# hall-lab/speedseq

Measured on AMD Instinct MI355X. Metric: paired reads aligned+dup-marked/sec, higher is better.
Workload: dtype int32; 1 GPU; 1000000 synthetic 2x150 bp PE pairs per GPU vs a seeded synthetic GRCh37-shaped reference of 3100 Mbp (25 contigs, order-6 Markov model of the bundled chr20 slice + 63 planted repeat families of 10..10^4 copies at 0-10% divergence = 5% of the bases; GRCh37 itself is not available offline), bwa-mem -t 16 batch boundaries; pairs_per_gpu=1000000, read_len=150, ref_bp=3099999990, records=2058655, dup_pairs=47309, dup_pairs_local_view=47309, seeds=60444408, rescues=632178, chains=9804599, sam_lines=2009191, discordant_stream_lines=29550, splitter_stream_lines=18382, dedup_scope=single GPU = whole input, sorted_merge=single GPU: bin/sambamba sort (device radix sort of the keys)

## Files before the change

### include/ssgpu.h

```cpp
#ifndef SSGPU_H
#define SSGPU_H
#include <stdint.h>
#include <stddef.h>
#include "../speedseq_amd/csrc/ssg_types.h"

#ifdef __cplusplus
extern "C" {
#endif

#define SSG_OK         0
#define SSG_ENODEV   (-19)
#define SSG_ENOMEM   (-12)
#define SSG_EINVAL   (-22)
#define SSG_EIO      (-5)
#define SSG_EOVERFLOW (-75)
#define SSG_EALIGN   (-71)
#define SSG_EHIP     (-1000)

const char *ssg_version(void);
const char *ssg_backend(void);
int ssg_device_count(void);
int ssg_set_device(int dev);
int ssg_set_lane(int lane);
const char *ssg_last_error(void);

void ssg_mem_opt_init(ssg_mem_opt_t *opt);

typedef struct ssg_index ssg_index_t;
int ssg_index_load(const char *prefix, ssg_index_t **out);
int ssg_index_load2(const char *prefix, int defer_dense_sa, ssg_index_t **out);
int ssg_index_densify(ssg_index_t *idx);
int ssg_index_densify_to(ssg_index_t *idx, int intv);
int ssg_index_from_arrays(const uint32_t *bwt, uint64_t bwt_words, uint64_t primary, const uint64_t L2[5],
                          const uint64_t *sa, uint64_t n_sa, int sa_intv,
                          const uint8_t *pac, int64_t l_pac,
                          int n_ctg, const int64_t *ctg_off, const int32_t *ctg_len, ssg_index_t **out);
int ssg_index_build_fasta(const char *fasta, ssg_index_t **out);
int ssg_index_build_dev(const uint8_t *d_fwd, int64_t l_pac, int n_ctg, const int64_t *ctg_off, const int32_t *ctg_len, ssg_index_t **out);
int ssg_index_save(const ssg_index_t *idx, const char *prefix);
void ssg_index_destroy(ssg_index_t *idx);
int64_t ssg_index_l_pac(const ssg_index_t *idx);
int ssg_index_n_ctg(const ssg_index_t *idx);


int ssg_extend_batch(const ssg_mem_opt_t *opt, int n_jobs, const ssg_ext_job_t *jobs,
                     const uint8_t *qbuf, size_t qbytes, const uint8_t *tbuf, size_t tbytes,
                     ssg_ext_res_t *res, uint64_t *cells);

int ssg_align2_batch(const ssg_mem_opt_t *opt, int n_jobs, const ssg_sw_job_t *jobs,
                     const uint8_t *qbuf, size_t qbytes, const uint8_t *tbuf, size_t tbytes, ssg_kswr_t *res);

int ssg_global_batch(const ssg_mem_opt_t *opt, int n_jobs, const ssg_glb_job_t *jobs,
                     const uint8_t *qbuf, size_t qbytes, const uint8_t *tbuf, size_t tbytes,
                     int32_t *score, int32_t *n_cigar, uint32_t *cigar, int cap);

int ssg_smem_batch(const ssg_index_t *idx, const ssg_mem_opt_t *opt, int n_reads, const uint8_t *seq, const int64_t *off,
                   int cap, ssg_intv_t *out_intv, int32_t *out_n);

int ssg_seeds_batch(const ssg_index_t *idx, const ssg_mem_opt_t *opt, int n_reads, const uint8_t *seq, const int64_t *off,
                    int64_t *seed_off, ssg_seed_t **seeds, int32_t **rids);

int ssg_extend_lane_batch(const ssg_index_t *idx, const ssg_mem_opt_t *opt, int n_jobs, const ssg_ext_job_t *jobs, const int64_t *tpos, int dir,
                          const uint8_t *qbuf, size_t qbytes, int qcap, ssg_ext_res_t *res, uint64_t *cells);

int ssg_align2_lane_batch(const ssg_index_t *idx, const ssg_mem_opt_t *opt, int n_jobs, const ssg_sw_job_t *jobs, const int64_t *tpos,
                          const uint8_t *qbuf, size_t qbytes, int lanes, ssg_kswr_t *res, int32_t *from_lane);

int ssg_dbg_chain_sort(const int64_t *keys, int n, int64_t *out_lane, int64_t *out_wave);

#define SSG_CHAIN_FORM_LANE     0
#define SSG_CHAIN_FORM_LDS16    1
#define SSG_CHAIN_FORM_LDS32    2
#define SSG_CHAIN_FORM_LDS64    3
#define SSG_CHAIN_FORM_WAVE256  4
#define SSG_CHAIN_FORM_WAVE512  5
#define SSG_CHAIN_FORM_WAVE1024 6
#define SSG_CHAIN_FORM_WAVE2048 7
#define SSG_CHAIN_FORM_WAVE5120 8
#define SSG_CHAIN_FORM_TREE  0x10
int ssg_dbg_chain(const ssg_mem_opt_t *opt, int64_t l_pac, int n_ctg, int n_reads, const int32_t *read_len, const int64_t *seed_off, const ssg_seed_t *seeds, const int32_t *rids,
                  const int64_t *intv_off, const ssg_intv_t *intv, int64_t *chain_off, ssg_chain_t **chains, int32_t **chain_seeds, int32_t *form);

#define SSG_REG_ROUTE_WAVE  1
#define SSG_REG_ROUTE_PATCH 2
int ssg_dbg_regions(const ssg_mem_opt_t *opt, const uint8_t *pac, int64_t l_pac, int n_ctg, const int64_t *ctg_off, const int32_t *ctg_len, int n_reads, const uint8_t *seq, const int64_t *off,
                    const int64_t *seed_off, const ssg_seed_t *seeds, const int64_t *chain_off, const ssg_chain_t *chains, const int32_t *chain_seeds,
                    int64_t *reg_off, ssg_alnreg_t **regs, int32_t *route);

int ssg_dbg_pestat(const ssg_index_t *idx, const ssg_mem_opt_t *opt, int n_pairs, const int64_t *reg_off, const ssg_alnreg_t *regs,
                   const int32_t *pair_batch, int n_batches, ssg_pestat_t *pes);
void ssg_dbg_matesw_last(uint64_t counts[8]);
int ssg_dbg_matesw(const ssg_index_t *idx, const ssg_mem_opt_t *opt, int n_pairs, const uint8_t *seq, const int64_t *read_off, const int64_t *reg_off, const ssg_alnreg_t *regs,
                   const uint8_t *fixed, const ssg_pestat_t pes[4], int headroom, int64_t *out_off, ssg_alnreg_t **regs_out, int32_t *n_out, int32_t *err, uint64_t counts[8]);
int ssg_dbg_pair_final(const ssg_index_t *idx, const ssg_mem_opt_t *opt, int n_pairs, int64_t id0, const int64_t *reg_off, const ssg_alnreg_t *regs,
                       const ssg_pestat_t pes[4], ssg_alnreg_t *regs_out, int64_t *req_off, ssg_alnreq_t **req);

#define SSG_R2A_ROUTE_LANE 1
#define SSG_R2A_ROUTE_DP0  2
#define SSG_R2A_ROUTE_DP1  4
#define SSG_R2A_ROUTE_DP2  8
#define SSG_R2A_ROUTE_WAVE 16
int ssg_dbg_reg2aln(const ssg_mem_opt_t *opt, const uint8_t *pac, int64_t l_pac, int n_ctg, const int64_t *ctg_off, const int32_t *ctg_len, int n_reads, const uint8_t *seq, const int64_t *off,
                    int64_t n_regs, const ssg_alnreg_t *regs, int64_t n_req, const ssg_alnreq_t *req, ssg_aln_t *alns, int32_t *route, int32_t *dev_err);

int ssg_align1_batch(const ssg_index_t *idx, const ssg_mem_opt_t *opt, int n_reads, const uint8_t *seq, const int64_t *off,
                     int64_t *reg_off, ssg_alnreg_t **regs, uint64_t stats[8]);

typedef struct ssg_pe_result ssg_pe_result_t;
int ssg_mem_process_pairs(const ssg_index_t *idx, const ssg_mem_opt_t *opt, int n_pairs, const uint8_t *seq, const int64_t *off,
                          const int32_t *pair_batch, int n_batches, int64_t id0, const ssg_pestat_t *pes0, ssg_pe_result_t **out);
int ssg_mem_process_reads(const ssg_index_t *idx, const ssg_mem_opt_t *opt, int n_reads, const uint8_t *seq, const int64_t *off, int64_t id0, ssg_pe_result_t **out);
void ssg_pe_result_free(ssg_pe_result_t *r);
int ssg_pe_reserve(int n_pairs, int n_calls);
int64_t ssg_pe_n_req(const ssg_pe_result_t *r);
int ssg_pe_is_se(const ssg_pe_result_t *r);
const int64_t *ssg_pe_req_off(const ssg_pe_result_t *r);
const ssg_alnreq_t *ssg_pe_req(const ssg_pe_result_t *r);
const ssg_aln_t *ssg_pe_alns(const ssg_pe_result_t *r);
const ssg_pestat_t *ssg_pe_pes(const ssg_pe_result_t *r);
const uint64_t *ssg_pe_stats(const ssg_pe_result_t *r);

int ssg_sam_format(const ssg_index_t *idx, const ssg_mem_opt_t *opt, const ssg_pe_result_t *res, int n_pairs,
                   const char *const *names, const uint8_t *seq, const int64_t *off, const char *const *quals, const char *const *comments,
                   const char *rg_id, char **sam, int64_t *sam_off);
int ssg_sam_format_se(const ssg_index_t *idx, const ssg_mem_opt_t *opt, const ssg_pe_result_t *res, int n_reads,
                      const char *const *names, const uint8_t *seq, const int64_t *off, const char *const *quals, const char *const *comments,
                      const char *rg_id, char **sam, int64_t *sam_off);
int ssg_sam_format_sel(const ssg_index_t *idx, const ssg_mem_opt_t *opt, const ssg_pe_result_t *res, const int32_t *sel, int n_sel,
                       const char *const *names, const uint8_t *seq, const int64_t *off, const char *const *quals, const char *const *comments,
                       const char *rg_id, char **sam, int64_t *sam_off);
int ssg_bam_format(const ssg_index_t *idx, const ssg_mem_opt_t *opt, const ssg_pe_result_t *res, int n_pairs,
                   const char *const *names, const uint8_t *seq, const int64_t *off, const char *const *quals,
                   const char *rg_id, uint8_t **bam, int64_t *bam_off);
typedef struct ssg_pe_bam ssg_pe_bam_t;
int ssg_mem_process_fastq_bam(const ssg_index_t *idx, const ssg_mem_opt_t *opt, int n_pairs, const uint8_t *const *parts, const int64_t *part_bytes, int n_parts,
                              const int64_t *rec_off, const int32_t *pair_batch, int n_batches, int64_t id0, const ssg_pestat_t *pes0, const char *rg_id, ssg_pe_bam_t **out);
int ssg_mem_process_pairs_bam(const ssg_index_t *idx, const ssg_mem_opt_t *opt, int n_pairs, const uint8_t *seq, const int64_t *off,
                              const char *const *names, const char *const *quals, const int32_t *pair_batch, int n_batches, int64_t id0,
                              const ssg_pestat_t *pes0, const char *rg_id, ssg_pe_bam_t **out);
void ssg_pe_bam_free(ssg_pe_bam_t *r);
const uint8_t *ssg_pe_bam_data(const ssg_pe_bam_t *r);
int64_t ssg_pe_bam_bytes(const ssg_pe_bam_t *r);
int64_t ssg_pe_bam_n_rec(const ssg_pe_bam_t *r);
int64_t ssg_pe_bam_n_cand(const ssg_pe_bam_t *r);
const ssg_bam_cand_t *ssg_pe_bam_cands(const ssg_pe_bam_t *r);
const ssg_pestat_t *ssg_pe_bam_pes(const ssg_pe_bam_t *r);
const uint64_t *ssg_pe_bam_stats(const ssg_pe_bam_t *r);
int ssg_index_set_names(ssg_index_t *idx, int n, const char *const *names);
const char *ssg_index_name(const ssg_index_t *idx, int i);
int32_t ssg_index_len(const ssg_index_t *idx, int i);

int ssg_sbl_markdup(long n_pairs, const ssg_sbl_end_t *ends, uint8_t *dup);
typedef struct ssg_sbl_state ssg_sbl_state_t;
ssg_sbl_state_t *ssg_sbl_state_new(void);
void ssg_sbl_state_free(ssg_sbl_state_t *st);
int ssg_sbl_markdup_stream(ssg_sbl_state_t *st, long n_pairs, const ssg_sbl_end_t *ends, uint8_t *dup);

#define SSG_SBL_DUP   1
#define SSG_SBL_DISC  2
#define SSG_SBL_SPLIT 4
void ssg_sbl_opt_init(ssg_sbl_opt_t *o);
int ssg_sbl_process(ssg_sbl_state_t *st, const ssg_sbl_opt_t *o, long n_blocks, const int64_t *blk_off, const ssg_sbl_line_t *lines,
                    uint8_t *line_bits, int64_t *mate_line);
int ssg_sbl_ends(long n_blocks, const int64_t *blk_off, const ssg_sbl_line_t *lines, ssg_sbl_end_t *ends);
int ssg_sbl_classify(const ssg_sbl_opt_t *o, long n_blocks, const int64_t *blk_off, const ssg_sbl_line_t *lines, const uint8_t *dup,
                     uint8_t *line_bits, int64_t *mate_line);

int ssg_sort_u64_perm(const uint64_t *keys, int64_t n, uint32_t *perm);

int ssg_hotpath_dev(const ssg_index_t *idx, const ssg_mem_opt_t *opt, int n_pairs, int max_len, const uint8_t *d_seq, const int64_t *d_off,
                    const int32_t *d_pair_batch, int n_batches, int64_t id0, uint64_t summary[8], uint8_t *dup_host);
int ssg_hotpath_dev_sig(const ssg_index_t *idx, const ssg_mem_opt_t *opt, int n_pairs, int max_len, const uint8_t *d_seq, const int64_t *d_off,
                        const int32_t *d_pair_batch, int n_batches, int64_t id0, uint64_t summary[8], uint8_t *dup_host, uint64_t *d_sig_out);

typedef struct ssg_dev_records ssg_dev_records_t;
int ssg_hotpath_dev_ex(const ssg_index_t *idx, const ssg_mem_opt_t *opt, int n_pairs, int max_len, const uint8_t *d_seq, const int64_t *d_off,
                       const int32_t *d_pair_batch, int n_batches, int64_t id0, const ssg_sbl_opt_t *sbl, int local_dedup,
                       uint64_t summary[16], uint8_t *dup_host, uint64_t *d_sig_out, ssg_dev_records_t **keep);
int ssg_dev_records_classify(ssg_dev_records_t *r, const ssg_sbl_opt_t *sbl, const uint8_t *d_dup, uint64_t counts[4]);
int ssg_markdup_sig_dev(long n, const uint64_t *d_sig, const int64_t *d_ordinal, uint8_t *d_dup);
void ssg_dev_records_free(ssg_dev_records_t *r);
int64_t ssg_dev_records_n_lines(const ssg_dev_records_t *r);
size_t ssg_dev_record_bytes(void);
int ssg_dev_records_export(const ssg_dev_records_t *r, uint64_t *d_keys, void *d_recs, uint8_t *d_bits);
int ssg_dev_records_download(const ssg_dev_records_t *r, ssg_pe_result_t **res, uint8_t *line_bits, int64_t *mate_line);
int ssg_dbg_sbl_records(long n_pairs, const int64_t *req_off, const ssg_alnreq_t *req, const ssg_aln_t *alns, const ssg_sbl_opt_t *o, ssg_sbl_state_t *st,
                        int64_t *line_off, int64_t *n_lines, ssg_sbl_line_t *lines, int64_t *line_req, ssg_sbl_end_t *ends, int64_t *prim, uint64_t *sig, uint8_t *dup,
                        uint8_t *bits, int64_t *mate_line, uint64_t counts[4], uint64_t *keys);

int ssg_index_from_device(const uint32_t *d_bwt, uint64_t primary, const uint64_t L2[5], const uint64_t *d_sa, int sa_intv,
                          const uint8_t *d_pac, int64_t l_pac, int n_ctg, const int64_t *ctg_off, const int32_t *ctg_len, ssg_index_t **out);

void ssg_prof_enable(int on);
void ssg_prof_reset(void);
int ssg_prof_get(int cap, const char **name, double *ms, long *launches);

void ssg_free(void *p);

typedef struct ssg_coll ssg_coll_t;
int ssg_coll_available(void);
int ssg_coll_init(int rank, int world, const char *rendezvous_dir, ssg_coll_t **out);
int ssg_coll_alltoallv(ssg_coll_t *c, const void *const *send, const uint64_t *send_bytes, void *const *recv, const uint64_t *recv_bytes);
int ssg_coll_alltoall_u64(ssg_coll_t *c, const uint64_t *send, uint64_t *recv, int k);
void ssg_coll_destroy(ssg_coll_t *c);

int ssg_bgzf_deflate(const uint8_t *payload, const uint64_t *cut, long n_blocks, uint8_t *out, uint64_t out_cap, uint64_t *out_off);
int ssg_bgzf_compress(const uint8_t *payload, const uint64_t *cut, long n_blocks, uint8_t *out, uint64_t out_cap, uint64_t *out_off, uint32_t *crc);
int ssg_bgzf_deflate_level(const uint8_t *payload, const uint64_t *cut, long n_blocks, uint8_t *out, uint64_t out_cap, uint64_t *out_off, int level);
int ssg_bgzf_compress_level(const uint8_t *payload, const uint64_t *cut, long n_blocks, uint8_t *out, uint64_t out_cap, uint64_t *out_off, uint32_t *crc, int level);
uint64_t ssg_bgzf_bound(uint64_t payload_bytes, long n_blocks);
int ssg_crc32_batch(const uint8_t *data, const uint64_t *cut, long n, uint32_t *crc);
int ssg_bgzf_inflate(const uint8_t *members, const uint64_t *moff, long n_blocks, uint8_t *out, uint64_t out_cap, uint64_t *out_off, int32_t *status);
typedef struct ssg_recs ssg_recs_t;
int ssg_recs_create(uint64_t cap_bytes, ssg_recs_t **out);
int ssg_recs_append(ssg_recs_t *r, const uint8_t *bytes, uint64_t len, uint32_t *chunk_id);
int ssg_recs_order(ssg_recs_t *r, const uint64_t *loc, const uint64_t *cum, int64_t n);
int ssg_recs_gather(ssg_recs_t *r, uint64_t v0, uint64_t v1, uint8_t *out);
int ssg_bgzf_compress_recs(ssg_recs_t *r, const uint64_t *cut, long n_blocks, uint8_t *out, uint64_t out_cap, uint64_t *out_off, uint32_t *crc);
int ssg_bgzf_compress_recs_level(ssg_recs_t *r, const uint64_t *cut, long n_blocks, uint8_t *out, uint64_t out_cap, uint64_t *out_off, uint32_t *crc, int level);
void ssg_recs_free(ssg_recs_t *r);
typedef struct { int32_t tid, pos, end; uint32_t flag, len, pad; } ssg_bam_ent_t;
int ssg_recs_append_bgzf(ssg_recs_t *r, const uint8_t *members, const uint64_t *moff, long n_blocks, uint32_t *chunk_id, uint64_t *out_off, int32_t *status);
int ssg_recs_scan(ssg_recs_t *r, uint32_t chunk_id, const uint64_t *hint, int64_t n_hints, uint64_t first, uint64_t cap, uint64_t *n_rec, uint64_t *loc, uint64_t *key, ssg_bam_ent_t *ent);
typedef struct { int32_t tid, beg, end; } ssg_bam_region_t;
typedef struct { uint8_t op, arg; uint16_t pad; int32_t value; } ssg_bam_fop_t;
#define SSG_FOP_MAX 64
enum { SSG_FOP_FLAG = 0, SSG_FOP_AND = 1, SSG_FOP_OR = 2, SSG_FOP_NOT = 3, SSG_FOP_EQ = 4, SSG_FOP_NE = 5, SSG_FOP_LT = 6, SSG_FOP_LE = 7, SSG_FOP_GT = 8, SSG_FOP_GE = 9 };
enum { SSG_FLD_MAPQ = 0, SSG_FLD_REF_ID = 1, SSG_FLD_MATE_REF_ID = 2, SSG_FLD_TLEN = 3, SSG_FLD_SEQ_LEN = 4, SSG_FLD_FLAG = 5 };
int ssg_recs_select(ssg_recs_t *r, uint32_t chunk_id, const uint64_t *hint, int64_t n_hints, uint64_t first, const ssg_bam_region_t *reg, int64_t n_reg, const ssg_bam_fop_t *prog, int n_prog,
                    uint64_t cap, uint64_t *n_rec, uint64_t *n_sel, uint64_t *loc, uint64_t *key, ssg_bam_ent_t *ent);
int ssg_recs_reopen(ssg_recs_t *r);
int ssg_recs_release(ssg_recs_t *r, uint32_t chunk_id);
int ssg_device_memory(uint64_t *free_bytes, uint64_t *total_bytes);
void *ssg_host_alloc(size_t n);
void ssg_host_free(void *p);

#ifdef __cplusplus
}
#endif
#endif
```

### speedseq_amd/capi.py

```python
import ctypes as C
import os

import numpy as np

HERE = os.path.dirname(os.path.abspath(__file__))
DEFAULT_LIB = os.path.join(HERE, "libssgpu.so")

OPT_DT = np.dtype([
    ("a", "i4"), ("b", "i4"), ("o_del", "i4"), ("e_del", "i4"), ("o_ins", "i4"), ("e_ins", "i4"),
    ("pen_unpaired", "i4"), ("pen_clip5", "i4"), ("pen_clip3", "i4"), ("w", "i4"), ("zdrop", "i4"),
    ("T", "i4"), ("min_seed_len", "i4"), ("min_chain_weight", "i4"), ("max_chain_extend", "i4"),
    ("split_width", "i4"), ("max_occ", "i4"), ("max_chain_gap", "i4"), ("max_ins", "i4"), ("max_matesw", "i4"),
    ("max_XA_hits", "i4"), ("max_XA_hits_alt", "i4"), ("mapQ_coef_fac", "i4"), ("chunk_size", "i4"), ("n_threads", "i4"),
    ("_align", "i4"),
    ("max_mem_intv", "u8"),
    ("split_factor", "f4"), ("mask_level", "f4"), ("drop_ratio", "f4"), ("XA_drop_ratio", "f4"),
    ("mask_level_redun", "f4"), ("mapQ_coef_len", "f4"),
    ("mat", "i1", (25,)), ("_pad0", "i1"), ("flag", "u2"), ("_pad", "i1", (4,)),
], align=False)
INTV_DT = np.dtype([("x0", "u8"), ("x1", "u8"), ("x2", "u8"), ("info", "u8")])
SEED_DT = np.dtype([("rbeg", "i8"), ("qbeg", "i4"), ("len", "i4"), ("score", "i4"), ("next", "i4")])
CHAIN_DT = np.dtype([("pos", "i8"), ("first_seed", "i4"), ("last_seed", "i4"), ("n", "i4"), ("rid", "i4"), ("w", "i4"), ("kept", "i4"), ("first", "i4"), ("sec", "i4"),
                     ("left", "i4"), ("right", "i4"), ("frac_rep", "f4"), ("_pad", "i4")])
CHAIN_FORM_LANE, CHAIN_FORM_LDS16, CHAIN_FORM_LDS32, CHAIN_FORM_LDS64 = 0, 1, 2, 3
CHAIN_FORM_WAVE256, CHAIN_FORM_WAVE512, CHAIN_FORM_WAVE1024, CHAIN_FORM_WAVE2048, CHAIN_FORM_WAVE5120 = 4, 5, 6, 7, 8
CHAIN_FORM_TREE = 0x10
REG_ROUTE_WAVE, REG_ROUTE_PATCH = 1, 2
R2A_ROUTE_LANE, R2A_ROUTE_DP0, R2A_ROUTE_DP1, R2A_ROUTE_DP2, R2A_ROUTE_WAVE = 1, 2, 4, 8, 16
EXT_JOB_DT = np.dtype([("qoff", "i4"), ("qlen", "i4"), ("toff", "i4"), ("tlen", "i4"), ("w", "i4"), ("end_bonus", "i4"), ("zdrop", "i4"), ("h0", "i4")])
EXT_RES_DT = np.dtype([("score", "i4"), ("qle", "i4"), ("tle", "i4"), ("gtle", "i4"), ("gscore", "i4"), ("max_off", "i4")])
SW_JOB_DT = np.dtype([("qoff", "i4"), ("qlen", "i4"), ("toff", "i4"), ("tlen", "i4"), ("xtra", "i4"), ("_pad", "i4")])
KSWR_DT = np.dtype([("score", "i4"), ("te", "i4"), ("qe", "i4"), ("score2", "i4"), ("te2", "i4"), ("tb", "i4"), ("qb", "i4")])
GLB_JOB_DT = np.dtype([("qoff", "i4"), ("qlen", "i4"), ("toff", "i4"), ("tlen", "i4"), ("w", "i4"), ("_pad", "i4")])
ALNREG_DT = np.dtype([
    ("rb", "i8"), ("re", "i8"), ("qb", "i4"), ("qe", "i4"), ("rid", "i4"), ("score", "i4"), ("truesc", "i4"), ("sub", "i4"),
    ("alt_sc", "i4"), ("csub", "i4"), ("sub_n", "i4"), ("w", "i4"), ("seedcov", "i4"), ("secondary", "i4"),
    ("secondary_all", "i4"), ("seedlen0", "i4"), ("n_comp", "i4"), ("frac_rep", "f4"), ("hash", "u8"),
])
PESTAT_DT = np.dtype([("low", "i4"), ("high", "i4"), ("failed", "i4"), ("_pad", "i4"), ("avg", "f8"), ("std", "f8")])


class SsgError(RuntimeError):
    pass


def _ptr(a):
    return a.ctypes.data_as(C.c_void_p)


class Lib:
    def __init__(self, path=None):
        path = path or os.environ.get("SSGPU_LIB") or DEFAULT_LIB
        if not os.path.exists(path):
            raise SsgError("%s not found: build it with `make lib` (hipcc --offload-arch=gfx950); there is no CPU fallback" % path)
        self.path = path
        self.l = C.CDLL(path)
        self.l.ssg_version.restype = C.c_char_p
        self.l.ssg_backend.restype = C.c_char_p
        self.l.ssg_last_error.restype = C.c_char_p
        self.l.ssg_index_l_pac.restype = C.c_int64
        assert OPT_DT.itemsize == self.sizeof_opt(), (OPT_DT.itemsize, self.sizeof_opt())

    def sizeof_opt(self):
        return 25 * 4 + 4 + 8 + 6 * 4 + 32

    def _chk(self, rc):
        if rc != 0:
            raise SsgError("libssgpu error %d: %s" % (rc, self.l.ssg_last_error().decode()))

    def backend(self):
        return self.l.ssg_backend().decode()

    def device_count(self):
        return self.l.ssg_device_count()

    def opt_init(self):
        o = np.zeros(1, dtype=OPT_DT)
        self.l.ssg_mem_opt_init(_ptr(o))
        return o

    def index_load(self, prefix):
        h = C.c_void_p()
        self._chk(self.l.ssg_index_load(prefix.encode(), C.byref(h)))
        return h

    def index_build_fasta(self, fasta):
        h = C.c_void_p()
        self._chk(self.l.ssg_index_build_fasta(fasta.encode(), C.byref(h)))
        return h

    def index_build_dev(self, d_fwd, l_pac, ctg_off, ctg_len, names=None):
        h = C.c_void_p()
        co = np.asarray(ctg_off, dtype=np.int64)
        cl = np.asarray(ctg_len, dtype=np.int32)
        self._chk(self.l.ssg_index_build_dev(C.c_void_p(d_fwd), C.c_int64(l_pac), C.c_int(len(co)), _ptr(co), _ptr(cl), C.byref(h)))
        if names is not None:
            arr = (C.c_char_p * len(names))(*[n.encode() for n in names])
            self._chk(self.l.ssg_index_set_names(h, C.c_int(len(names)), arr))
        return h

    def index_save(self, h, prefix):
        self._chk(self.l.ssg_index_save(h, prefix.encode()))

    def index_destroy(self, h):
        self.l.ssg_index_destroy(h)

    def extend_batch(self, opt, jobs, qbuf, tbuf):
        jobs = np.ascontiguousarray(jobs, dtype=EXT_JOB_DT)
        res = np.zeros(len(jobs), dtype=EXT_RES_DT)
        cells = C.c_uint64(0)
        self._chk(self.l.ssg_extend_batch(_ptr(opt), C.c_int(len(jobs)), _ptr(jobs), _ptr(qbuf), C.c_size_t(qbuf.size),
                                          _ptr(tbuf), C.c_size_t(tbuf.size), _ptr(res), C.byref(cells)))
        return res, cells.value

    def align2_batch(self, opt, jobs, qbuf, tbuf):
        jobs = np.ascontiguousarray(jobs, dtype=SW_JOB_DT)
        res = np.zeros(len(jobs), dtype=KSWR_DT)
        self._chk(self.l.ssg_align2_batch(_ptr(opt), C.c_int(len(jobs)), _ptr(jobs), _ptr(qbuf), C.c_size_t(qbuf.size),
                                          _ptr(tbuf), C.c_size_t(tbuf.size), _ptr(res)))
        return res

    def global_batch(self, opt, jobs, qbuf, tbuf, cap=64):
        jobs = np.ascontiguousarray(jobs, dtype=GLB_JOB_DT)
        n = len(jobs)
        score = np.zeros(n, dtype=np.int32)
        ncig = np.zeros(n, dtype=np.int32)
        cig = np.zeros((n, cap), dtype=np.uint32)
        self._chk(self.l.ssg_global_batch(_ptr(opt), C.c_int(n), _ptr(jobs), _ptr(qbuf), C.c_size_t(qbuf.size),
                                          _ptr(tbuf), C.c_size_t(tbuf.size), _ptr(score), _ptr(ncig), _ptr(cig), C.c_int(cap)))
        return score, ncig, cig

    def smem_batch(self, idx, opt, seq, off, cap=64):
        n = len(off) - 1
        intv = np.zeros((n, cap), dtype=INTV_DT)
        cnt = np.zeros(n, dtype=np.int32)
        self._chk(self.l.ssg_smem_batch(idx, _ptr(opt), C.c_int(n), _ptr(seq), _ptr(off), C.c_int(cap), _ptr(intv), _ptr(cnt)))
        return intv, cnt

    def seeds_batch(self, idx, opt, seq, off):
        n = len(off) - 1
        seed_off = np.zeros(n + 1, dtype=np.int64)
        sp, rp = C.c_void_p(), C.c_void_p()
        self._chk(self.l.ssg_seeds_batch(idx, _ptr(opt), C.c_int(n), _ptr(seq), _ptr(off), _ptr(seed_off), C.byref(sp), C.byref(rp)))
        tot = int(seed_off[n])
        seeds = np.frombuffer((C.c_char * (tot * SEED_DT.itemsize)).from_address(sp.value), dtype=SEED_DT, count=tot).copy() if tot else np.zeros(0, SEED_DT)
        rids = np.frombuffer((C.c_char * (tot * 4)).from_address(rp.value), dtype=np.int32, count=tot).copy() if tot else np.zeros(0, np.int32)
        self.l.ssg_free(sp); self.l.ssg_free(rp)
        return seed_off, seeds, rids

    def extend_lane_batch(self, idx, opt, jobs, tpos, direction, qbuf, qcap):
        res = np.zeros(len(jobs), dtype=EXT_RES_DT)
        cells = C.c_uint64(0)
        tpos = np.ascontiguousarray(tpos, dtype=np.int64)
        self._chk(self.l.ssg_extend_lane_batch(idx, _ptr(opt), C.c_int(len(jobs)), _ptr(jobs), _ptr(tpos), C.c_int(direction), _ptr(qbuf), C.c_size_t(qbuf.size), C.c_int(qcap), _ptr(res), C.byref(cells)))
        return res, cells.value

    def align2_lane_batch(self, idx, opt, jobs, tpos, qbuf, lanes):
        jobs = np.ascontiguousarray(jobs, dtype=SW_JOB_DT)
        res = np.zeros(len(jobs), dtype=KSWR_DT)
        from_lane = np.zeros(len(jobs), dtype=np.int32)
        tpos = np.ascontiguousarray(tpos, dtype=np.int64)
        self._chk(self.l.ssg_align2_lane_batch(idx, _ptr(opt), C.c_int(len(jobs)), _ptr(jobs), _ptr(tpos), _ptr(qbuf), C.c_size_t(qbuf.size), C.c_int(lanes), _ptr(res), _ptr(from_lane)))
        return res, from_lane

    def dbg_chain_sort(self, keys):
        keys = np.ascontiguousarray(keys, dtype=np.int64)
        o0, o1 = np.zeros(len(keys), dtype=np.int64), np.zeros(len(keys), dtype=np.int64)
        self._chk(self.l.ssg_dbg_chain_sort(_ptr(keys), C.c_int(len(keys)), _ptr(o0), _ptr(o1)))
        return o0, o1

    def dbg_chain(self, opt, l_pac, n_ctg, read_len, seed_off, seeds, rids, intv_off, intv):
        read_len = np.ascontiguousarray(read_len, dtype=np.int32)
        seed_off = np.ascontiguousarray(seed_off, dtype=np.int64)
        intv_off = np.ascontiguousarray(intv_off, dtype=np.int64)
        seeds = np.ascontiguousarray(seeds, dtype=SEED_DT)
        rids = np.ascontiguousarray(rids, dtype=np.int32)
        intv = np.ascontiguousarray(intv, dtype=INTV_DT)
        n = len(read_len)
        assert len(seed_off) == n + 1 and len(intv_off) == n + 1 and len(seeds) >= seed_off[-1] and len(rids) >= seed_off[-1] and len(intv) >= intv_off[-1]
        chain_off, form = np.zeros(n + 1, dtype=np.int64), np.zeros(n, dtype=np.int32)
        cp, sp = C.c_void_p(), C.c_void_p()
        self._chk(self.l.ssg_dbg_chain(_ptr(opt), C.c_int64(l_pac), C.c_int(n_ctg), C.c_int(n), _ptr(read_len), _ptr(seed_off), _ptr(seeds), _ptr(rids), _ptr(intv_off), _ptr(intv),
                                       _ptr(chain_off), C.byref(cp), C.byref(sp), _ptr(form)))
        nc = int(chain_off[n])
        chains = np.frombuffer((C.c_char * (nc * CHAIN_DT.itemsize)).from_address(cp.value), dtype=CHAIN_DT, count=nc).copy() if nc else np.zeros(0, CHAIN_DT)
        ns = int(chains["n"].sum()) if nc else 0
        cseeds = np.frombuffer((C.c_char * (ns * 4)).from_address(sp.value), dtype=np.int32, count=ns).copy() if ns else np.zeros(0, np.int32)
        self.l.ssg_free(cp); self.l.ssg_free(sp)
        return chain_off, chains, cseeds, form

    def dbg_regions(self, opt, pac, l_pac, ctg_off, ctg_len, seq, off, seed_off, seeds, chain_off, chains, chain_seeds):
        pac = np.ascontiguousarray(pac, dtype=np.uint8)
        ctg_off = np.ascontiguousarray(ctg_off, dtype=np.int64)
        ctg_len = np.ascontiguousarray(ctg_len, dtype=np.int32)
        seq = np.ascontiguousarray(seq, dtype=np.uint8)
        off = np.ascontiguousarray(off, dtype=np.int64)
        seed_off = np.ascontiguousarray(seed_off, dtype=np.int64)
        chain_off = np.ascontiguousarray(chain_off, dtype=np.int64)
        seeds = np.ascontiguousarray(seeds, dtype=SEED_DT)
        chains = np.ascontiguousarray(chains, dtype=CHAIN_DT)
        chain_seeds = np.ascontiguousarray(chain_seeds, dtype=np.int32)
        n = len(off) - 1
        assert len(pac) >= l_pac // 4 + 1 and len(ctg_off) == len(ctg_len) and len(seed_off) == n + 1 and len(chain_off) == n + 1
        assert len(seq) >= off[-1] and len(seeds) >= seed_off[-1] and len(chains) >= chain_off[-1] and len(chain_seeds) >= int(chains["n"][:int(chain_off[-1])].sum())
        reg_off, route = np.zeros(n + 1, dtype=np.int64), np.zeros(n, dtype=np.int32)
        rp = C.c_void_p()
        self._chk(self.l.ssg_dbg_regions(_ptr(opt), _ptr(pac), C.c_int64(l_pac), C.c_int(len(ctg_off)), _ptr(ctg_off), _ptr(ctg_len), C.c_int(n), _ptr(seq), _ptr(off),
                                         _ptr(seed_off), _ptr(seeds), _ptr(chain_off), _ptr(chains), _ptr(chain_seeds), _ptr(reg_off), C.byref(rp), _ptr(route)))
        tot = int(reg_off[n])
        regs = np.frombuffer((C.c_char * (tot * ALNREG_DT.itemsize)).from_address(rp.value), dtype=ALNREG_DT, count=tot).copy() if tot else np.zeros(0, ALNREG_DT)
        self.l.ssg_free(rp)
        return reg_off, regs, route

    def dbg_reg2aln(self, opt, pac, l_pac, ctg_off, ctg_len, seq, off, regs, req):
        pac = np.ascontiguousarray(pac, dtype=np.uint8)
        ctg_off = np.ascontiguousarray(ctg_off, dtype=np.int64)
        ctg_len = np.ascontiguousarray(ctg_len, dtype=np.int32)
        seq = np.ascontiguousarray(seq, dtype=np.uint8)
        off = np.ascontiguousarray(off, dtype=np.int64)
        regs = np.ascontiguousarray(regs, dtype=ALNREG_DT)
        req = np.ascontiguousarray(req, dtype=ALNREQ_DT)
        n = len(off) - 1
        assert len(pac) >= l_pac // 4 + 1 and len(ctg_off) == len(ctg_len) and n >= 0 and (n == 0 or len(seq) >= off[-1])
        alns, route, err = np.zeros(len(req) + 1, dtype=ALN_DT), np.zeros(len(req) + 1, dtype=np.int32), C.c_int32(0)
        rc = self.l.ssg_dbg_reg2aln(_ptr(opt), _ptr(pac), C.c_int64(l_pac), C.c_int(len(ctg_off)), _ptr(ctg_off), _ptr(ctg_len), C.c_int(n), _ptr(seq), _ptr(off),
                                    C.c_int64(len(regs)), _ptr(regs), C.c_int64(len(req)), _ptr(req), _ptr(alns), _ptr(route), C.byref(err))
        if rc != -75:
            self._chk(rc)
        return rc, alns[:len(req)], route[:len(req)], int(err.value)

    def dbg_pestat(self, idx, opt, reg_off, regs, pair_batch, n_batches):
        reg_off = np.ascontiguousarray(reg_off, dtype=np.int64)
        regs = np.ascontiguousarray(regs, dtype=ALNREG_DT)
        pair_batch = np.ascontiguousarray(pair_batch, dtype=np.int32)
        pes = np.zeros(4 * n_batches, dtype=PESTAT_DT)
        self._chk(self.l.ssg_dbg_pestat(idx, _ptr(opt), C.c_int((len(reg_off) - 1) // 2), _ptr(reg_off), _ptr(regs), _ptr(pair_batch), C.c_int(n_batches), _ptr(pes)))
        return pes

    def dbg_pair_final(self, idx, opt, id0, reg_off, regs, pes):
        reg_off = np.ascontiguousarray(reg_off, dtype=np.int64)
        regs = np.ascontiguousarray(regs, dtype=ALNREG_DT)
        pes = np.ascontiguousarray(pes, dtype=PESTAT_DT)
        assert len(pes) == 4 and len(regs) == reg_off[-1]
        n = len(reg_off) - 1
        out = np.zeros(len(regs), dtype=ALNREG_DT)
        req_off = np.zeros(n + 1, dtype=np.int64)
        req_p = C.c_void_p()
        self._chk(self.l.ssg_dbg_pair_final(idx, _ptr(opt), C.c_int(n // 2), C.c_int64(id0), _ptr(reg_off), _ptr(regs), _ptr(pes), _ptr(out), _ptr(req_off), C.byref(req_p)))
        nreq = int(req_off[n])
        req = np.frombuffer((C.c_char * (nreq * ALNREQ_DT.itemsize)).from_address(req_p.value), dtype=ALNREQ_DT, count=nreq).copy() if nreq else np.zeros(0, ALNREQ_DT)
        self.l.ssg_free(req_p)
        return out, req_off, req

    def dbg_matesw(self, idx, opt, seq, read_off, reg_off, regs, pes, fixed=None, headroom=-1):
        seq = np.ascontiguousarray(seq, dtype=np.uint8)
        read_off = np.ascontiguousarray(read_off, dtype=np.int64)
        reg_off = np.ascontiguousarray(reg_off, dtype=np.int64)
        regs = np.ascontiguousarray(regs, dtype=ALNREG_DT)
        pes = np.ascontiguousarray(pes, dtype=PESTAT_DT)
        n = len(reg_off) - 1
        assert len(pes) == 4 and len(regs) == reg_off[-1] and len(read_off) == n + 1 and len(seq) == read_off[-1]
        fx = None if fixed is None else np.ascontiguousarray(fixed, dtype=np.uint8)
        assert fx is None or len(fx) == n
        out_off, n_out, err, counts = np.zeros(n + 1, dtype=np.int64), np.zeros(n, dtype=np.int32), np.zeros(n // 2, dtype=np.int32), np.zeros(8, dtype=np.uint64)
        out_p = C.c_void_p()
        self._chk(self.l.ssg_dbg_matesw(idx, _ptr(opt), C.c_int(n // 2), _ptr(seq), _ptr(read_off), _ptr(reg_off), _ptr(regs), _ptr(fx) if fx is not None else None, _ptr(pes),
                                        C.c_int(headroom), _ptr(out_off), C.byref(out_p), _ptr(n_out), _ptr(err), _ptr(counts)))
        tot = int(out_off[n])
        allr = np.frombuffer((C.c_char * (tot * ALNREG_DT.itemsize)).from_address(out_p.value), dtype=ALNREG_DT, count=tot).copy() if tot and out_p.value else np.zeros(0, ALNREG_DT)
        self.l.ssg_free(out_p)
        lists = [allr[int(out_off[r]):int(out_off[r]) + int(n_out[r])].copy() for r in range(n)]
        return lists, err, counts

    def dbg_matesw_last(self):
        counts = np.zeros(8, dtype=np.uint64)
        self.l.ssg_dbg_matesw_last(_ptr(counts))
        return counts

    def align1_batch(self, idx, opt, seq, off):
        n = len(off) - 1
        reg_off = np.zeros(n + 1, dtype=np.int64)
        regs_p = C.c_void_p()
        stats = np.zeros(8, dtype=np.uint64)
        self._chk(self.l.ssg_align1_batch(idx, _ptr(opt), C.c_int(n), _ptr(seq), _ptr(off), _ptr(reg_off), C.byref(regs_p), _ptr(stats)))
        tot = int(reg_off[n])
        buf = (C.c_char * (tot * ALNREG_DT.itemsize)).from_address(regs_p.value) if tot else b""
        regs = np.frombuffer(buf, dtype=ALNREG_DT, count=tot).copy()
        self.l.ssg_free(regs_p)
        return reg_off, regs, stats


ALNREQ_DT = np.dtype([("read", "i4"), ("reg", "i4"), ("kind", "i4"), ("owner", "i4"), ("flag", "i4"), ("mapq", "i4"), ("_p0", "i4"), ("_p1", "i4")])
ALN_DT = np.dtype([("pos", "i8"), ("rid", "i4"), ("flag", "i4"), ("mapq", "i4"), ("NM", "i4"), ("score", "i4"), ("sub", "i4"), ("n_cigar", "i4"),
                   ("is_rev", "i4"), ("l_md", "i4"), ("reg_idx", "i4"), ("xa_cnt", "i4"), ("_pad", "i4"), ("cigar", "u4", (64,)), ("md", "S320")])


class PeResult:

    def __init__(self, lib, handle, n_pairs, n_batches):
        self.lib, self.h, self.n_pairs, self.n_batches = lib, handle, n_pairs, n_batches
        l = lib.l
        n = l.ssg_pe_n_req(handle)
        self.req_off = np.ctypeslib.as_array(C.cast(l.ssg_pe_req_off(handle), C.POINTER(C.c_int64)), shape=(2 * n_pairs + 1,)).copy()
        self.req = np.frombuffer((C.c_char * (n * ALNREQ_DT.itemsize)).from_address(l.ssg_pe_req(handle)), dtype=ALNREQ_DT, count=n).copy() if n else np.zeros(0, ALNREQ_DT)
        self.alns = np.frombuffer((C.c_char * (n * ALN_DT.itemsize)).from_address(l.ssg_pe_alns(handle)), dtype=ALN_DT, count=n).copy() if n else np.zeros(0, ALN_DT)
        self.pes = np.frombuffer((C.c_char * (n_batches * 4 * PESTAT_DT.itemsize)).from_address(l.ssg_pe_pes(handle)), dtype=PESTAT_DT, count=n_batches * 4).copy() if n_batches else np.zeros(0, PESTAT_DT)
        self.stats = np.ctypeslib.as_array(C.cast(l.ssg_pe_stats(handle), C.POINTER(C.c_uint64)), shape=(8,)).copy()

    def close(self):
        if self.h:
            self.lib.l.ssg_pe_result_free(self.h)
            self.h = None

    def __del__(self):
        self.close()


def _bind_pe(lib):
    l = lib.l
    l.ssg_pe_n_req.restype = C.c_int64
    for f in ("ssg_pe_req_off", "ssg_pe_req", "ssg_pe_alns", "ssg_pe_pes", "ssg_pe_stats"):
        getattr(l, f).restype = C.c_void_p
        getattr(l, f).argtypes = [C.c_void_p]
    l.ssg_pe_n_req.argtypes = [C.c_void_p]
    l.ssg_pe_result_free.argtypes = [C.c_void_p]


def mem_process_pairs(lib, idx, opt, seq, off, pair_batch=None, n_batches=1, id0=0, pes0=None):
    _bind_pe(lib)
    n_pairs = (len(off) - 1) // 2
    if pair_batch is None:
        pair_batch = np.zeros(n_pairs, dtype=np.int32)
    pair_batch = np.ascontiguousarray(pair_batch, dtype=np.int32)
    h = C.c_void_p()
    p0 = _ptr(pes0) if pes0 is not None else None
    lib._chk(lib.l.ssg_mem_process_pairs(idx, _ptr(opt), C.c_int(n_pairs), _ptr(seq), _ptr(off), _ptr(pair_batch), C.c_int(n_batches),
                                         C.c_int64(id0), p0, C.byref(h)))
    return PeResult(lib, h, n_pairs, n_batches)


SBL_END_DT = np.dtype([("seq", "i4"), ("pos", "i4"), ("flag", "i4"), ("lclip", "i4"), ("rclip", "i4"), ("ralen", "i4")])


def sbl_markdup(lib, ends):
    ends = np.ascontiguousarray(ends, dtype=SBL_END_DT)
    n = len(ends) // 2
    dup = np.zeros(n, dtype=np.uint8)
    lib._chk(lib.l.ssg_sbl_markdup(C.c_long(n), _ptr(ends), _ptr(dup)))
    return dup


SBL_LINE_DT = np.dtype([("seq", "i4"), ("pos", "i4"), ("flag", "i4"), ("mapq", "i4"), ("lclip", "i4"), ("rclip", "i4"), ("qalen", "i4"), ("ralen", "i4")])
SBL_OPT_DT = np.dtype([("exclude_dups", "i4"), ("add_mate_tags", "i4"), ("max_split_count", "i4"), ("min_non_overlap", "i4"), ("max_unmapped_bases", "i4"),
                       ("min_indel_size", "i4")])


def sbl_opt_init(lib, **kw):
    o = np.zeros((), dtype=SBL_OPT_DT)
    lib.l.ssg_sbl_opt_init(_ptr(o))
    for k, v in kw.items():
        o[k] = v
    return o


def sbl_state_new(lib):
    lib.l.ssg_sbl_state_new.restype = C.c_void_p
    return C.c_void_p(lib.l.ssg_sbl_state_new())


def sbl_state_free(lib, st):
    lib.l.ssg_sbl_state_free(st)


def sbl_markdup_stream(lib, st, ends):
    ends = np.ascontiguousarray(ends, dtype=SBL_END_DT)
    n = len(ends) // 2
    dup = np.zeros(n, dtype=np.uint8)
    lib._chk(lib.l.ssg_sbl_markdup_stream(st, C.c_long(n), _ptr(ends), _ptr(dup)))
    return dup


def _sbl_chunk(blk_off, lines):
    off = np.ascontiguousarray(blk_off, dtype=np.int64)
    lines = np.ascontiguousarray(lines, dtype=SBL_LINE_DT)
    assert int(off[-1]) == len(lines), (int(off[-1]), len(lines))
    return off, lines, len(off) - 1


def sbl_process(lib, st, opt, blk_off, lines):
    off, lines, nb = _sbl_chunk(blk_off, lines)
    bits, mate = np.zeros(len(lines), dtype=np.uint8), np.zeros(len(lines), dtype=np.int64)
    lib._chk(lib.l.ssg_sbl_process(st, _ptr(opt), C.c_long(nb), _ptr(off), _ptr(lines), _ptr(bits), _ptr(mate)))
    return bits, mate


def sbl_ends(lib, blk_off, lines):
    off, lines, nb = _sbl_chunk(blk_off, lines)
    ends = np.zeros(2 * nb, dtype=SBL_END_DT)
    lib._chk(lib.l.ssg_sbl_ends(C.c_long(nb), _ptr(off), _ptr(lines), _ptr(ends)))
    return ends


def sbl_classify(lib, opt, blk_off, lines, dup):
    off, lines, nb = _sbl_chunk(blk_off, lines)
    dup = np.ascontiguousarray(dup, dtype=np.uint8)
    assert len(dup) == nb
    bits, mate = np.zeros(len(lines), dtype=np.uint8), np.zeros(len(lines), dtype=np.int64)
    lib._chk(lib.l.ssg_sbl_classify(_ptr(opt), C.c_long(nb), _ptr(off), _ptr(lines), _ptr(dup), _ptr(bits), _ptr(mate)))
    return bits, mate


def dbg_sbl_records(lib, req_off, req, alns, opt, st=None):
    req_off = np.ascontiguousarray(req_off, dtype=np.int64)
    req = np.ascontiguousarray(req, dtype=ALNREQ_DT)
    alns = np.ascontiguousarray(alns, dtype=ALN_DT)
    n_pairs, cap = (len(req_off) - 1) // 2, len(req) + 1
    assert len(req_off) == 2 * n_pairs + 1 and len(req) == len(alns)
    o = dict(line_off=np.zeros(n_pairs + 1, np.int64), lines=np.zeros(cap, SBL_LINE_DT), line_req=np.zeros(cap, np.int64), ends=np.zeros(2 * n_pairs + 1, SBL_END_DT),
             prim=np.zeros(2 * n_pairs + 1, np.int64), sig=np.zeros((n_pairs + 1, 3), np.uint64), dup=np.zeros(n_pairs + 1, np.uint8), bits=np.zeros(cap, np.uint8),
             mate=np.zeros(cap, np.int64), counts=np.zeros(4, np.uint64), keys=np.zeros(cap, np.uint64))
    nl = C.c_int64(0)
    rc = lib.l.ssg_dbg_sbl_records(C.c_long(n_pairs), _ptr(req_off), _ptr(req), _ptr(alns), _ptr(opt), st, _ptr(o["line_off"]), C.byref(nl), _ptr(o["lines"]),
                                   _ptr(o["line_req"]), _ptr(o["ends"]), _ptr(o["prim"]), _ptr(o["sig"]), _ptr(o["dup"]), _ptr(o["bits"]), _ptr(o["mate"]),
                                   _ptr(o["counts"]), _ptr(o["keys"]))
    n = int(nl.value)
    for k in ("lines", "line_req", "bits", "mate", "keys"):
        o[k] = o[k][:n]
    for k, m in (("ends", 2 * n_pairs), ("prim", 2 * n_pairs), ("sig", n_pairs), ("dup", n_pairs)):
        o[k] = o[k][:m]
    return rc, o


def index_from_device(lib, d_bwt, primary, L2, d_sa, d_pac, l_pac, ctg_off, ctg_len, sa_intv=32):
    h = C.c_void_p()
    L2a = np.asarray(L2, dtype=np.uint64)
    co = np.asarray(ctg_off, dtype=np.int64)
    cl = np.asarray(ctg_len, dtype=np.int32)
    lib._chk(lib.l.ssg_index_from_device(C.c_void_p(d_bwt), C.c_uint64(primary), _ptr(L2a), C.c_void_p(d_sa), C.c_int(sa_intv),
                                         C.c_void_p(d_pac), C.c_int64(l_pac), C.c_int(len(co)), _ptr(co), _ptr(cl), C.byref(h)))
    return h

# ... 347 lines not shown
```

### speedseq_amd/csrc/k_smem2.h

```cpp
#ifndef SSG_K_SMEM2_H
#define SSG_K_SMEM2_H
#include "ssg_dev.h"

#define SSG_S2_QWORDS 40
enum { S2_FWD = 0, S2_BWD, S2_P3F, S2_READ, S2_P1, S2_P2, S2_P3, S2_OUT, S2_FIN };
enum { S2_PEND_NONE = 0, S2_PEND_FWD, S2_PEND_BWD, S2_PEND_P3 };

struct alignas(16) ssg_pk2_t { uint64_t w0, w1; };
SSG_DEVFN ssg_pk2_t s2_pk(const ssg_intv_t &v)
{ ssg_pk2_t p; p.w0 = v.x0 | (v.x1 & 0xffffffull) << 40; p.w1 = (v.x1 >> 24) | v.x2 << 16 | v.info << 55; return p; }
SSG_DEVFN ssg_intv_t s2_unpk(const ssg_pk2_t &p)
{ ssg_intv_t v; v.x0 = p.w0 & 0xffffffffffull; v.x1 = (p.w0 >> 40) | (p.w1 & 0xffffull) << 24; v.x2 = (p.w1 >> 16) & 0x7fffffffffull; v.info = p.w1 >> 55; return v; }
SSG_DEVFN void s2_set_intv(const ssg_index_view_t &ix, int c, ssg_intv_t &ik)
{
	ik.x0 = ix.L2[c] + 1; ik.x2 = ix.L2[c+1] - ix.L2[c]; ik.x1 = ix.L2[3-c] + 1; ik.info = 0;
}

#ifdef SSG_EMU
static unsigned long long ssg_s2_stat[64];
SSG_DEVFN unsigned long long s2_wall() { return 1; }
#else
__device__ unsigned long long ssg_s2_stat[64];
SSG_DEVFN unsigned long long s2_wall() { return (unsigned long long)wall_clock64(); }
#endif
#define S2_STAT_MIN(i, v) atomicMin(&ssg_s2_stat[i], (unsigned long long)(v))
#define S2_STAT_MAX(i, v) atomicMax(&ssg_s2_stat[i], (unsigned long long)(v))
#define S2_STAT_ADD(i, v) atomicAdd(&ssg_s2_stat[i], (unsigned long long)(v))

#ifndef SSG_S2_WAVES
#define SSG_S2_WAVES 4
#endif
#ifndef SSG_S2_TRIPS
#define SSG_S2_TRIPS 2
#endif

#ifdef SSG_EMU
SSG_DEVFN int wv_uni(int v) { return v; }
SSG_DEVFN uint64_t wv_uni64(uint64_t v) { return v; }
#else
SSG_DEVFN int wv_uni(int v) { return __builtin_amdgcn_readfirstlane(v); }
SSG_DEVFN uint64_t wv_uni64(uint64_t v) { return (uint64_t)(uint32_t)__builtin_amdgcn_readfirstlane((int)(uint32_t)v) | (uint64_t)(uint32_t)__builtin_amdgcn_readfirstlane((int)(uint32_t)(v >> 32)) << 32; }
#endif
SSG_DEVFN ssg_intv_t wv_uni_intv(const ssg_intv_t &v) { ssg_intv_t o; o.x0 = wv_uni64(v.x0); o.x1 = wv_uni64(v.x1); o.x2 = wv_uni64(v.x2); o.info = wv_uni64(v.info); return o; }

SSG_DEVFN unsigned long long s2_wave_read(const ssg_index_view_t &ix, const ssg_mem_opt_t &opt, const int split_len, const int it, const int32_t *read_ids, const uint8_t *seq, const int64_t *off,
                                          ssg_intv_t *out_intv, int32_t *out_n, const int cap, uint8_t *qb, ssg_pk2_t *l0, ssg_pk2_t *l1)
{
	const int lane = wv_lane();
	unsigned long long nx = 0;
	const int r = read_ids ? read_ids[it] : it;
	const uint8_t *q = seq + off[r];
	const int len = (int)(off[r+1] - off[r]);
	ssg_wave_ldssync();
	for (int b = lane; b < len; b += 64) qb[b] = q[b];
	ssg_wave_ldssync();
	ssg_intv_t *const mem = out_intv + (long)it * cap;
	const int left = -2 - out_n[it];
	const bool skip_p3 = left >= 1;
	const int n_p3 = skip_p3 ? left - 1 : 0;
	int mem_n = n_p3, ovf = 0;
	auto smem1 = [&](const int sx, uint64_t min_intv) -> int {
		if (min_intv < 1) min_intv = 1;
		ssg_intv_t ik; s2_set_intv(ix, (int)qb[sx], ik); ik.info = (uint64_t)(sx + 1);
		int n = 0, i = sx + 1;
		bool stop = false;
		while (!stop && i < len) {
			const int cq = wv_uni((int)qb[i]);
			if (cq < 4) {
				const ssg_intv_t ok = wv_uni_intv(ssg_bwt_extend1_lean(ix, ik, 3 - cq, 0)); ++nx;
				if (ok.x2 != ik.x2) { l0[n++] = s2_pk(ik); stop = ok.x2 < min_intv; }
				if (!stop) { ik = ok; ik.info = (uint64_t)(i + 1); ++i; }
			} else { l0[n++] = s2_pk(ik); stop = true; }
		}
		if (!stop) l0[n++] = s2_pk(ik);
		const int ret = (int)ik.info;
		int cur = 0, prev_n = n, rev = 1, m1_n = 0, m1_last_beg = 0;
		bool more = true;
		for (int ib = sx - 1; more && ib >= -1; --ib) {
			const int cb = ib < 0 ? -1 : wv_uni((int)qb[ib]) < 4 ? wv_uni((int)qb[ib]) : -1;
			int curr_n = 0; bool have_last = false; uint64_t last_x2 = 0;
			ssg_wave_ldssync();
			for (int base = 0; base < prev_n; base += 64) {
				const int jj = base + lane; const bool valid = jj < prev_n;
				ssg_intv_t p; p.x0 = p.x1 = p.x2 = p.info = 0;
				if (valid) p = s2_unpk((cur ? l1 : l0)[rev ? prev_n - 1 - jj : jj]);
				ssg_intv_t okc; okc.x0 = okc.x1 = okc.x2 = okc.info = 0;
				if (valid && cb >= 0) okc = ssg_bwt_extend1_lean(ix, p, cb, 1);
				if (cb >= 0) nx += (unsigned long long)(prev_n - base < 64 ? prev_n - base : 64);
				const bool alive = valid && cb >= 0 && okc.x2 >= min_intv;
				if (base == 0 && !wv_get((int)alive, 0)) {
					const int beg = ib + 1;
					if (m1_n == 0 || beg < m1_last_beg) {
						++m1_n; m1_last_beg = beg;
						const int end0 = wv_get((int)(uint32_t)p.info, 0);
						if (end0 - beg >= opt.min_seed_len) {
							if (mem_n < cap) { if (lane == 0) { ssg_intv_t o = p; o.info |= (uint64_t)beg << 32; mem[mem_n] = o; } } else ovf = 1;
							++mem_n;
						}
					}
				}
				const unsigned long long am = wv_ballot(alive);
				if (am) {
					const unsigned long long below = am & ((1ull << lane) - 1ull);
					const int pl = below ? 63 - __clzll(below) : 0;
					const uint64_t px2 = (uint64_t)wv_shfl64_xor((long long)okc.x2, lane ^ pl);
					const bool push = alive && (below ? okc.x2 != px2 : (!have_last || okc.x2 != last_x2));
					const unsigned long long pm = wv_ballot(push);
					if (push) { ssg_intv_t o = okc; o.info = p.info; (cur ? l0 : l1)[curr_n + __popcll(pm & ((1ull << lane) - 1ull))] = s2_pk(o); }
					curr_n += __popcll(pm);
					have_last = true; last_x2 = (uint64_t)wv_get64((long long)okc.x2, 63 - __clzll(am));
				}
			}
			if (curr_n == 0) more = false;
			else { cur ^= 1; rev = 0; prev_n = curr_n; }
		}
		ssg_wave_ldssync();
		return ret;
	};
	if (len >= opt.min_seed_len) {
		int x = 0;
		while (x < len) { if (wv_uni((int)qb[x]) < 4) x = smem1(x, 1); else ++x; }
		const int old_n = mem_n < cap ? mem_n : cap;
		ssg_wave_memsync();
		for (int k = n_p3; k < old_n; ++k) {
			const ssg_intv_t m = wv_uni_intv(mem[k]);
			const int start = (int)(m.info >> 32), end = (int)(uint32_t)m.info;
			if (end - start >= split_len && m.x2 <= (uint64_t)opt.split_width) {
				const int sx = (start + end) >> 1;
				if (wv_uni((int)qb[sx]) < 4) (void)smem1(sx, m.x2 + 1);
			}
		}
		if (opt.max_mem_intv > 0 && !skip_p3) {
			x = 0;
			while (x < len) {
				if (wv_uni((int)qb[x]) > 3) ++x;
				else {
					ssg_intv_t ik; s2_set_intv(ix, (int)qb[x], ik);
					int i = x + 1, nxt = len; bool stop = false;
					while (!stop && i < len) {
						const int cq = wv_uni((int)qb[i]);
						if (cq < 4) {
							const ssg_intv_t ok = wv_uni_intv(ssg_bwt_extend1_lean(ix, ik, 3 - cq, 0)); ++nx;
							if (ok.x2 < (uint64_t)opt.max_mem_intv && i - x >= opt.min_seed_len) {
								if (ok.x2 > 0) {
									if (mem_n < cap) { if (lane == 0) { ssg_intv_t o = ok; o.info = (uint64_t)x << 32 | (uint64_t)(i + 1); mem[mem_n] = o; } } else ovf = 1;
									++mem_n;
								}
								nxt = i + 1; stop = true;
							} else { ik = ok; ++i; }
						} else { nxt = i + 1; stop = true; }
					}
					x = nxt;
				}
			}
		}
	}
	if (lane == 0) out_n[it] = ovf ? -1 : mem_n;
	return nx;
}

SSG_DEVFN long s2_ktab_off(int j) { return (long)(((1ull << (2 * j)) - 4ull) / 3ull); }
__global__ void ssg_k_ktab_level(ssg_index_view_t ix, int j, ssg_pk2_t *tab)
{
	const long p = (long)blockIdx.x * blockDim.x + threadIdx.x;
	if (p >= (1L << (2 * (j - 1)))) return;
	ssg_pk2_t *const out = tab + s2_ktab_off(j) + 4 * p;
	ssg_intv_t ok[4];
	if (j == 1) { for (int c = 0; c < 4; ++c) s2_set_intv(ix, c, ok[c]); }
	else ssg_bwt_extend(ix, s2_unpk(tab[s2_ktab_off(j - 1) + p]), ok, 1);
	for (int c = 0; c < 4; ++c) { ok[c].info = 0; out[c] = s2_pk(ok[c]); }
}
__global__ void ssg_k_ktab_verify(ssg_index_view_t ix, int j, long stride, const ssg_pk2_t *tab, unsigned long long *bad)
{
	const long t = (long)blockIdx.x * blockDim.x + threadIdx.x, code = t * stride;
	if (code >= (1L << (2 * j))) return;
	ssg_intv_t ik;
	s2_set_intv(ix, (int)(code & 3), ik);
	for (int k = 1; k < j; ++k) ik = ssg_bwt_extend1_lean(ix, ik, 3 - (int)((code >> (2 * k)) & 3), 0);
	const ssg_intv_t e = s2_unpk(tab[s2_ktab_off(j) + code]);
	if (ik.x2 != e.x2 || (ik.x2 && (ik.x0 != e.x0 || ik.x1 != e.x1))) atomicAdd(&bad[j], 1ull);
}
SSG_DEVFN uint64_t s2_window(const uint32_t *qw, int stride, int b)
{
	const int w0 = b >> 3, sh = (b & 7) << 2;
	const int w1 = w0 + 1 < SSG_S2_QWORDS ? w0 + 1 : SSG_S2_QWORDS - 1, w2 = w0 + 2 < SSG_S2_QWORDS ? w0 + 2 : SSG_S2_QWORDS - 1;
	uint64_t v = ((uint64_t)qw[w0 * stride] | (uint64_t)qw[w1 * stride] << 32) >> sh;
	if (sh) v |= (uint64_t)qw[w2 * stride] << (64 - sh);
	return v;
}
SSG_DEVFN uint32_t s2_code(const uint32_t *qw, int stride, int b, int n)
{
	uint64_t v = s2_window(qw, stride, b);
	v &= 0x3333333333333333ull; v = (v | v >> 2) & 0x0f0f0f0f0f0f0f0full; v = (v | v >> 4) & 0x00ff00ff00ff00ffull;
	v = (v | v >> 8) & 0x0000ffff0000ffffull; v = (v | v >> 16) & 0xffffffffull;
	return (uint32_t)v & ((1u << (2 * n)) - 1u);
}

template <bool TUNE, bool KT>
__global__ void __launch_bounds__(64, SSG_S2_WAVES) ssg_k_smem2(ssg_index_view_t ix, ssg_mem_opt_t opt, int n_reads, const int32_t *read_ids,
                           const uint8_t *seq, const int64_t *off, ssg_intv_t *out_intv, int32_t *out_n, int cap,
                           ssg_pk2_t *scratch, int scap, unsigned long long *n_extend, unsigned int *next_read, unsigned int max_ext, int max_row, uint32_t *n_ext_read, int32_t *heavy_ids, unsigned int *n_heavy,
                           const ssg_pk2_t *kt_tab, int kt_k )
{
	__shared__ uint32_t qlds[SSG_S2_QWORDS * 64];
	const long gt = (long)blockIdx.x * blockDim.x + threadIdx.x;
	const int lane = (int)(threadIdx.x & 63);
	ssg_pk2_t *const vec0 = scratch + (gt >> 6) * 2 * scap * 64 + lane, *const vec1 = vec0 + (long)scap * 64;
	const uint32_t *const ql_ = qlds + lane;
#define S2Q(i) ((int)((ql_[((i) >> 3) * 64] >> (((i) & 7) << 2)) & 15u))
#define S2V(v, e) ((v)[(long)(e) * 64])
	const int split_len = (int)(opt.min_seed_len * opt.split_factor + .499);
	unsigned long long my_nx = 0;
	unsigned int rd_nx = 0, nx_p3 = 0;
	long it = 0;
	int state = S2_READ, pend = S2_PEND_NONE;
	int len = 0, x = 0, k = 0, old_n = 0, caller = 0, mem_n = 0, ovf = 0, heavy = 0, n_p3 = -1;
	ssg_intv_t *mem = 0;
	int sx = 0, i = 0, j = 0, curr_n = 0, prev_n = 0, prev_rev = 0, flip = 0, m1_n = 0, m1_last_beg = 0, ret = 0, e_c = 0;
	uint64_t min_intv = 1, last_x2 = 0;
	ssg_intv_t ik, p;
	ik.x0 = ik.x1 = ik.x2 = ik.info = 0; p = ik;
	ssg_pk2_t pn, c0, first; pn.w0 = pn.w1 = 0; c0 = first = pn;
	if (TUNE) S2_STAT_MIN(0, s2_wall());
#define S2_FWDEND() do { ret = (int)ik.info; flip ^= 1; prev_n = curr_n < scap ? curr_n : scap; prev_rev = 1; curr_n = 0; i = sx - 1; j = 0; first = s2_pk(ik); state = S2_BWD; if (prev_n > max_row) { heavy = 1; state = S2_OUT; } } while (0)
#define S2_P3END() do { n_p3 = mem_n; nx_p3 = rd_nx; x = 0; state = S2_P1; } while (0)
#define S2_P3START() do { \
		while (x < len && S2Q(x) > 3) ++x; \
		if (x >= len) S2_P3END(); \
		else if (!KT || kt_k < 2) { s2_set_intv(ix, S2Q(x), ik); i = x + 1; state = S2_P3F; } \
		else { \
			const unsigned long long nm_ = s2_window(ql_, 64, x) & 0x4444444444444444ull; \
			int run_ = nm_ ? (int)((__ffsll(nm_) - 1) >> 2) : 16; \
			run_ = run_ > len - x ? len - x : run_; \
			if (run_ >= kt_k) { ik = s2_unpk(kt_tab[s2_ktab_off(kt_k) + (long)s2_code(ql_, 64, x, kt_k)]); i = x + kt_k; my_nx += (unsigned long long)(kt_k - 1); rd_nx += (unsigned int)(kt_k - 1); state = S2_P3F; } \
			else { my_nx += (unsigned long long)(run_ - 1); rd_nx += (unsigned int)(run_ - 1); if (x + run_ >= len) S2_P3END(); else { x += run_ + 1; state = S2_P3; } } \
		} \
	} while (0)
#define S2_RET() do { if (caller == 1) { x = ret; state = S2_P1; } else { ++k; state = S2_P2; } } while (0)
#define S2_EMIT(pp, beg) do { if (m1_n == 0 || (beg) < m1_last_beg) { ++m1_n; m1_last_beg = (beg); \
		if ((int)(uint32_t)(pp).info - (beg) >= opt.min_seed_len) { ssg_intv_t o_ = (pp); o_.info |= (uint64_t)(beg) << 32; if (mem_n < cap) mem[mem_n] = o_; else ovf = 1; ++mem_n; } } } while (0)
	for (;;) {
		SSG_UNROLL for (int trip = 0; trip < SSG_S2_TRIPS; ++trip) if ((trip == 0 || wv_ballot(pend == S2_PEND_NONE && state != S2_FIN)) && pend == S2_PEND_NONE && state != S2_FIN) {
			ssg_pk2_t *const curr = flip ? vec1 : vec0;
			if (state == S2_FWD) {
				if (i < len && S2Q(i) < 4) { pend = S2_PEND_FWD; e_c = 3 - S2Q(i); }
				else { if (curr_n < scap) S2V(curr, curr_n) = s2_pk(ik); else ovf = 1; ++curr_n; S2_FWDEND(); }
			} else if (state == S2_BWD) {
				if (j >= prev_n) {
					bool back_to_caller = curr_n == 0;
					if (!back_to_caller) { flip ^= 1; prev_n = curr_n < scap ? curr_n : scap; prev_rev = 0; curr_n = 0; j = 0; --i; first = c0; back_to_caller = i < -1; }
					if (back_to_caller) S2_RET();
				} else {
					p = s2_unpk(j == 0 ? first : pn);
					const int cb = i < 0 ? -1 : S2Q(i) < 4 ? S2Q(i) : -1;
					if (cb >= 0) { pend = S2_PEND_BWD; e_c = cb; }
					else {
						if (j == 0) S2_EMIT(p, i + 1);
						j = prev_n;
					}
				}
			} else if (state == S2_P3F) {
				if (i >= len) S2_P3END();
				else if (S2Q(i) < 4) { pend = S2_PEND_P3; e_c = 3 - S2Q(i); }
				else { x = i + 1; S2_P3START(); }
			} else if (state == S2_READ) {
				it = (long)atomicAdd(next_read, 1u);
				if (it >= n_reads) { state = S2_FIN; if (TUNE) S2_STAT_MIN(1, s2_wall()); }
				else {
					const int r = read_ids ? read_ids[it] : (int)it;
					const uint8_t *q = seq + off[r];
					len = (int)(off[r+1] - off[r]);
					mem = out_intv + (long)it * cap; mem_n = 0; ovf = 0; rd_nx = 0; nx_p3 = 0; heavy = 0;
					const unsigned al = (unsigned)((uintptr_t)q & 7), sh8 = al << 3;
					const uint64_t *const qa = (const uint64_t*)(q - al);
					const int nw = (len + 7) >> 3, nb = (int)al + len;
					for (int w0 = 0; w0 < nw; w0 += 4) {
						uint64_t t[5];
						SSG_UNROLL for (int jj = 0; jj < 5; ++jj) t[jj] = (w0 + jj) * 8 < nb ? qa[w0 + jj] : 0;
						SSG_UNROLL for (int jj = 0; jj < 4; ++jj) {
							const int w = w0 + jj;
							if (w < nw) {
								uint64_t v = sh8 ? (t[jj] >> sh8) | (t[jj + 1] << (64 - sh8)) : t[jj];
								v &= 0x0f0f0f0f0f0f0f0full;
								v = (v | v >> 4) & 0x00ff00ff00ff00ffull;
								v = (v | v >> 8) & 0x0000ffff0000ffffull;
								uint32_t v32 = (uint32_t)(v | v >> 16);
								const int nv = len - w * 8;
								if (nv < 8) v32 &= (1u << (nv << 2)) - 1u;
								qlds[w * 64 + lane] = v32;
							}
						}
					}
					x = 0;
					n_p3 = opt.max_mem_intv > 0 ? -1 : 0;
					state = len < opt.min_seed_len ? S2_OUT : opt.max_mem_intv > 0 ? S2_P3 : S2_P1;
				}
			} else if (state == S2_P1) {
				if (x >= len) { old_n = mem_n < cap ? mem_n : cap; k = n_p3 > 0 ? n_p3 : 0; state = S2_P2; }
				else if (S2Q(x) > 3) ++x;
				else { sx = x; min_intv = 1; caller = 1; state = S2_FWD; m1_n = 0; curr_n = 0; i = sx + 1; s2_set_intv(ix, S2Q(sx), ik); ik.info = (uint64_t)(sx + 1); }
			} else if (state == S2_P2) {
				if (k >= old_n) state = S2_OUT;
				else {
					const ssg_intv_t m = mem[k];
					const int start = (int)(m.info >> 32), end = (int)(uint32_t)m.info;
					if (end - start < split_len || m.x2 > (uint64_t)opt.split_width) ++k;
					else {
						sx = (start + end) >> 1; min_intv = m.x2 + 1; caller = 2; m1_n = 0; curr_n = 0; i = sx + 1;
						if (S2Q(sx) > 3) S2_RET();
						else { s2_set_intv(ix, S2Q(sx), ik); ik.info = (uint64_t)(sx + 1); state = S2_FWD; }
					}
				}
			} else if (state == S2_P3) {
				S2_P3START();
			} else {
				const bool given_up = heavy != 0;
				out_n[it] = ovf ? -1 : given_up ? (n_p3 < 0 ? -2 : -3 - n_p3) : mem_n;
				if (given_up && !ovf && heavy_ids) heavy_ids[atomicAdd(n_heavy, 1u)] = (int32_t)it;
				if (given_up) my_nx -= n_p3 < 0 ? rd_nx : rd_nx - nx_p3;
				if (n_ext_read) n_ext_read[it] = rd_nx;
				if (TUNE) { S2_STAT_ADD(8 + (64 - __clzll((unsigned long long)(rd_nx | 1u))), 1); if (given_up) S2_STAT_ADD(3, 1); }
				state = S2_READ;
			}
		}
		if (TUNE) { const unsigned long long rdy = wv_ballot(pend != S2_PEND_NONE), alv = wv_ballot(state != S2_FIN); if (lane == 0) { S2_STAT_ADD(48, 1); S2_STAT_ADD(49, __popcll(rdy)); S2_STAT_ADD(50, __popcll(alv)); } }
		if (!wv_ballot(state != S2_FIN)) break;
		const int pat_b = pend == S2_PEND_BWD ? i : pend == S2_PEND_FWD ? sx : x, pat_n = (pend == S2_PEND_BWD ? (int)p.info : i + 1) - pat_b;
		const bool by_table = KT && pend != S2_PEND_NONE && pat_n <= kt_k;
		const bool any_tab = KT && wv_ballot(by_table) != 0, any_ext = !KT || wv_ballot(pend != S2_PEND_NONE && !by_table) != 0;
		if (pend != S2_PEND_NONE) {
			const ssg_pk2_t *const prev = flip ? vec0 : vec1;
			ssg_pk2_t *const curr = flip ? vec1 : vec0;
			const bool back = pend == S2_PEND_BWD;
			const int jn = back && j + 1 < prev_n ? j + 1 : 0;
			ssg_pk2_t pf; pf.w0 = pf.w1 = 0;
			if (jn) pf = S2V(prev, prev_rev ? prev_n - 1 - jn : jn);
			ssg_intv_t okc; okc.x0 = okc.x1 = okc.x2 = okc.info = 0;
			if (any_tab) { if (by_table) okc = s2_unpk(kt_tab[s2_ktab_off(pat_n) + (long)s2_code(ql_, 64, pat_b, pat_n)]); }
			if (any_ext) { if (!by_table) okc = ssg_bwt_extend1_lean(ix, back ? p : ik, e_c, back); }
			++my_nx; ++rd_nx;
			if (pend == S2_PEND_FWD) {
				bool fwd_end = false;
				if (okc.x2 != ik.x2) {
					if (curr_n < scap) S2V(curr, curr_n) = s2_pk(ik); else ovf = 1;
					++curr_n;
					if (okc.x2 < min_intv) { S2_FWDEND(); fwd_end = true; }
				}
				if (!fwd_end) { ik = okc; ik.info = (uint64_t)(i + 1); ++i; }
			} else if (back) {
				pn = pf;
				if (okc.x2 < min_intv) { if (curr_n == 0) S2_EMIT(p, i + 1); }
				else if (curr_n == 0 || okc.x2 != last_x2) {
					ssg_intv_t o = okc; o.info = p.info;
					const ssg_pk2_t po = s2_pk(o);
					if (curr_n == 0) c0 = po;
					if (curr_n < scap) S2V(curr, curr_n) = po; else ovf = 1;
					++curr_n; last_x2 = okc.x2;
				}
				++j;
			} else {
				if (okc.x2 < (uint64_t)opt.max_mem_intv && i - x >= opt.min_seed_len) {
					if (okc.x2 > 0) { ssg_intv_t o = okc; o.info = (uint64_t)x << 32 | (uint64_t)(i + 1); if (mem_n < cap) mem[mem_n] = o; else ovf = 1; ++mem_n; }
					x = i + 1; S2_P3START();
				} else { ik = okc; ++i; }
			}
			pend = S2_PEND_NONE;
			if (rd_nx > max_ext) { heavy = 1; state = S2_OUT; }
		}
	}
	if (TUNE) S2_STAT_MAX(2, s2_wall());
#undef S2Q
#undef S2V
#undef S2_FWDEND
#undef S2_P3START
#undef S2_P3END
#undef S2_RET
#undef S2_EMIT
	if (n_extend && my_nx) atomicAdd(n_extend, my_nx);
}

#ifdef SSG_HEAVY_MIN_WAVES
#define SSG_HEAVY_BOUNDS __launch_bounds__(64, SSG_HEAVY_MIN_WAVES)
#else
#define SSG_HEAVY_BOUNDS __launch_bounds__(64)
#endif
template <int SC>
__global__ void SSG_HEAVY_BOUNDS ssg_k_smem_heavy(ssg_index_view_t ix, ssg_mem_opt_t opt, const int32_t *ids, const unsigned int *n_ids, const int32_t *read_ids,
                           const uint8_t *seq, const int64_t *off, ssg_intv_t *out_intv, int32_t *out_n, int cap, unsigned long long *n_extend, unsigned int *next)
{
	__shared__ uint8_t qb[328];
	__shared__ ssg_pk2_t lst[2][SC];
	const int split_len = (int)(opt.min_seed_len * opt.split_factor + .499);
	const int n_todo = (int)*n_ids;
	unsigned long long nx = 0;
	for (;;) {
		const long t = wv_queue_pop(next);
		if (t >= n_todo) break;
		nx += s2_wave_read(ix, opt, split_len, ids[t], read_ids, seq, off, out_intv, out_n, cap, qb, lst[0], lst[1]);
	}
	if (n_extend && nx && wv_lane() == 0) atomicAdd(n_extend, nx);
}
__global__ void ssg_k_sa_verify(ssg_index_view_t ix, int new_intv, const uint64_t *sa_new, long n_new, long stride, unsigned long long *bad)
{
	const long j = ((long)blockIdx.x * blockDim.x + threadIdx.x) * stride;
	if (j >= n_new) return;
	const uint64_t r = (uint64_t)j * (uint64_t)new_intv;
	const uint64_t want = (r % (uint64_t)ix.sa_intv) == 0 ? ix.sa[r / (uint64_t)ix.sa_intv] : ssg_bwt_sa(ix, r);
	if (sa_new[j] != want) atomicAdd(bad, 1ull);
}
#endif
```

### speedseq_amd/csrc/ssg_dbg.cpp

```cpp
#include <vector>
#include <string>
#include <algorithm>
#include "ssg_rt.h"
#include "../../include/ssgpu.h"
#include "ssg_index_int.h"
#include "ssg_pe_int.h"
#include "ssg_stage_int.h"

SSG_ABI_FP_DEFINE(dbg)

static int dbg_refuse(const char *who, const char *bad, long at)
{
	ssg_err_msg = std::string(who) + ": " + bad + " " + std::to_string(at);
	return SSG_EINVAL;
}
static int dbg_check_contigs(const char *who, int64_t l_pac, int n_ctg, const int64_t *ctg_off, const int32_t *ctg_len)
{
	for (int c = 0; c < n_ctg; ++c)
		if (ctg_len[c] < 1 || ctg_off[c] != (c ? ctg_off[c - 1] + ctg_len[c - 1] : 0) || ctg_off[c] + ctg_len[c] > l_pac || (c == n_ctg - 1 && ctg_off[c] + ctg_len[c] != l_pac)) {
			ssg_err_msg = std::string(who) + ": the contigs must tile [0, l_pac) in order"; return SSG_EINVAL; }
	return 0;
}
static int dbg_read_len(const int64_t *off, int r, const char **bad)
{
// ... 115 lines not shown
	ssg_chain_t *oc = (ssg_chain_t*)calloc((size_t)n_out + 1, sizeof(ssg_chain_t)); int32_t *os = (int32_t*)calloc((size_t)n_sd + 1, sizeof(int32_t));
	if (!oc || !os) { free(oc); free(os); ssg_err_msg = "host allocation failed: chains"; return SSG_ENOMEM; }
	int64_t k = 0, q = 0;
	for (int r = 0; r < n_reads; ++r) {
		chain_off[r] = k;
		for (int i = 0; i < h_nc[r]; ++i) {
			const ssg_chain_t &c = h_ch[seed_off[r] + h_ord[seed_off[r] + i]];
			ssg_chain_t &o = oc[k++];
			o.pos = c.pos; o.rid = c.rid; o.n = c.n; o.w = c.w; o.kept = c.kept; o.frac_rep = c.frac_rep; o.first_seed = (int32_t)q;
			for (int j = 0; j < c.n; ++j) os[q++] = (int32_t)(h_cs[c.first_seed + j] - seed_off[r]);
		}
	}
	chain_off[n_reads] = k;
	*chains = oc; *chain_seeds = os;
	return SSG_OK;
}

int ssg_dbg_regions(const ssg_mem_opt_t *opt, const uint8_t *pac, int64_t l_pac, int n_ctg, const int64_t *ctg_off, const int32_t *ctg_len, int n_reads, const uint8_t *seq, const int64_t *off,
                    const int64_t *seed_off, const ssg_seed_t *seeds, const int64_t *chain_off, const ssg_chain_t *chains, const int32_t *chain_seeds,
                    int64_t *reg_off, ssg_alnreg_t **regs, int32_t *route)
{
	CHK(ssg_need_device());
	*regs = 0;
	if (n_reads < 0 || l_pac < 1 || l_pac >= (int64_t)1 << 33 || n_ctg < 1) { ssg_err_msg = "ssg_dbg_regions: need n_reads >= 0, 1 <= l_pac < 2^33, n_ctg >= 1"; return SSG_EINVAL; }
	CHK(dbg_check_contigs("ssg_dbg_regions", l_pac, n_ctg, ctg_off, ctg_len));
	if (n_reads == 0) { reg_off[0] = 0; return SSG_OK; }
	const char *bad = 0; long at = 0;
	if (off[0] != 0 || seed_off[0] != 0 || chain_off[0] != 0) bad = "offsets start at 0: read";
	int max_len = 0;
	auto ctg_of = [&](int64_t p) { const int64_t f = p < l_pac ? p : 2 * l_pac - 1 - p; int lo = 0, hi = n_ctg - 1; while (lo < hi) { const int mid = (lo + hi + 1) >> 1; if (ctg_off[mid] <= f) lo = mid; else hi = mid - 1; } return lo; };
	std::vector<uint8_t> used;
	for (int r = 0; !bad && r < n_reads; ++r) {
		at = r;
		if (seed_off[r + 1] < seed_off[r] || chain_off[r + 1] < chain_off[r]) { bad = "offsets must not decrease: read"; break; }
		const int len = dbg_read_len(off, r, &bad);
		if (bad) break;
		const int64_t ns = seed_off[r + 1] - seed_off[r], nc = chain_off[r + 1] - chain_off[r];
		if (ns >= (int64_t)1 << 24) { bad = "more than 2^24 seeds: read"; break; }
		if (nc > ns) { bad = "more chains than seeds: read"; break; }
		max_len = std::max(max_len, len);
		dbg_check_codes(seq, off, r, &bad);
		for (int64_t k = seed_off[r]; !bad && k < seed_off[r + 1]; ++k) {
			bad = dbg_check_seed(seeds[k], len, l_pac, "need 0 <= qbeg, 1 <= len, qbeg + len <= read length: seed");
			if (bad) at = (long)k;
		}
		used.assign((size_t)ns, 0);
		for (int64_t k = chain_off[r]; !bad && k < chain_off[r + 1]; ++k) {
			const ssg_chain_t &c = chains[k];
			at = (long)k;
			if (c.n < 1) { bad = "a chain has at least 1 seed: chain"; break; }
			if (c.first_seed < 0 || (k > 0 && c.first_seed != chains[k - 1].first_seed + chains[k - 1].n) || (k == 0 && c.first_seed != 0)) { bad = "first_seed must run on from the chain before: chain"; break; }
			for (int j = 0; j < c.n; ++j) {
				const int32_t id = chain_seeds[c.first_seed + j];
				if (id < 0 || id >= ns) { bad = "a seed index outside the read's seeds: chain"; break; }
				if (used[(size_t)id]) { bad = "a seed in two chains: chain"; break; }
				used[(size_t)id] = 1;
			}
			if (bad) break;
			const int64_t first = seeds[seed_off[r] + chain_seeds[c.first_seed]].rbeg;
			if (c.rid != ctg_of(first)) { bad = "rid must be the contig of the chain's first seed: chain"; break; }
			int64_t cb = ctg_off[c.rid], ce = cb + ctg_len[c.rid];
			if (first >= l_pac) { const int64_t t = cb; cb = 2 * l_pac - ce; ce = 2 * l_pac - t; }
			for (int j = 0; j < c.n; ++j) {
				const ssg_seed_t &sd = seeds[seed_off[r] + chain_seeds[c.first_seed + j]];
				if (sd.rbeg < cb || sd.rbeg + sd.len > ce) { bad = "every seed of a chain must lie inside the contig and strand of its first seed: chain"; break; }
			}
			if (bad) break;
		}
	}
	if (!bad) {
		CHK(check_scores(opt, max_len));
		if (opt->e_del < 1 || opt->e_ins < 1) { ssg_err_msg = "ssg_dbg_regions: gap extension penalties must be positive"; return SSG_EINVAL; }
	}
	if (bad) return dbg_refuse("ssg_dbg_regions", bad, at);
	const int64_t tot = seed_off[n_reads];
	if (tot >= (int64_t)1 << 31) { ssg_err_msg = "ssg_dbg_regions: more than 2^31 seeds"; return SSG_EINVAL; }
	const size_t ts = (size_t)tot + 1;
	const std::vector<ssg_seed_t> h_sd = dbg_stage_seeds(seeds, tot);
	std::vector<ssg_chain_t> h_ch(ts); std::vector<int32_t> h_ord(ts, 0), h_cs(ts, 0);
	const std::vector<int32_t> h_nc = dbg_counts(chain_off, n_reads), h_ns = dbg_counts(seed_off, n_reads);
	memset(h_ch.data(), 0, ts * sizeof(ssg_chain_t));
	for (int r = 0; r < n_reads; ++r) {
		const int64_t s0 = seed_off[r];
		int64_t q = s0;
		for (int i = 0; i < h_nc[r]; ++i) {
			const ssg_chain_t &c = chains[chain_off[r] + i];
			ssg_chain_t &d = h_ch[s0 + i];
			d = c; d.first_seed = (int32_t)q; d.last_seed = -1;
			h_ord[s0 + i] = i;
			for (int j = 0; j < c.n; ++j) h_cs[q++] = (int32_t)(s0 + chain_seeds[c.first_seed + j]);
		}
	}
	dbg_ref_t ref;
	CHK(ref.up(pac, l_pac, n_ctg, ctg_off, ctg_len));
	dbuf<uint8_t> d_seq((size_t)off[n_reads] + 1); dbuf<int64_t> d_off((size_t)n_reads + 1);
	dbuf<ssg_seed_t> d_seeds(ts); dbuf<ssg_chain_t> d_chains(ts); dbuf<int32_t> d_order(ts), d_cseeds(ts), d_nchain(n_reads), d_nseed(n_reads), d_work(n_reads); dbuf<unsigned int> d_queue(8);
	CHKA(d_seq); CHKA(d_off); CHKA(d_seeds); CHKA(d_chains); CHKA(d_order); CHKA(d_cseeds); CHKA(d_nchain); CHKA(d_nseed); CHKA(d_work); CHKA(d_queue);
	CHK(d_seq.up(seq, (size_t)off[n_reads])); CHK(d_off.up(off, (size_t)n_reads + 1));
	CHK(d_seeds.up(h_sd.data(), ts)); CHK(d_chains.up(h_ch.data(), ts)); CHK(d_order.up(h_ord.data(), ts)); CHK(d_cseeds.up(h_cs.data(), ts));
	CHK(d_nchain.up(h_nc.data(), n_reads)); CHK(d_nseed.up(h_ns.data(), n_reads));
	CHK(dbg_work_order(d_nseed.p, n_reads, d_work.p, d_queue));
	align1_dev_t o;
	if (!o.seed_off.alloc((size_t)n_reads + 1) || !o.regs.alloc(ts) || !o.n_reg.alloc(n_reads)) { ssg_err_msg = "device allocation failed: regs"; return SSG_ENOMEM; }
	CHK(o.seed_off.up(seed_off, (size_t)n_reads + 1));
	std::vector<int32_t> todo;
	CHK(run_regions(ref.ix, opt, n_reads, d_seq.p, d_off.p, max_len, ts, d_seeds.p, d_chains.p, d_order.p, d_cseeds.p, d_nchain.p, d_work.p, d_queue.p, o, (uint64_t*)0, (uint64_t*)0, &todo));
	std::vector<int32_t> hn((size_t)n_reads); std::vector<uint8_t> hf((size_t)n_reads); std::vector<ssg_alnreg_t> all(ts);
	CHK(o.n_reg.down(hn.data(), n_reads)); CHK(o.sdp_fixed.down(hf.data(), n_reads)); CHK(o.regs.down(all.data(), (size_t)tot));
	int64_t n_out = 0;
	for (int r = 0; r < n_reads; ++r) {
		if (hn[r] < 0 || hn[r] > h_ns[r]) { ssg_err_msg = "ssg_dbg_regions: a read's region count is outside its slice"; return SSG_EOVERFLOW; }
		reg_off[r] = n_out; n_out += hn[r];
	}
	reg_off[n_reads] = n_out;
	ssg_alnreg_t *out = (ssg_alnreg_t*)malloc(sizeof(ssg_alnreg_t) * (size_t)(n_out + 1));
	if (!out) { ssg_err_msg = "host allocation failed: regions"; return SSG_ENOMEM; }
	for (int r = 0; r < n_reads; ++r) memcpy(out + reg_off[r], all.data() + seed_off[r], sizeof(ssg_alnreg_t) * (size_t)hn[r]);
	if (route) {
		for (int r = 0; r < n_reads; ++r) route[r] = hf[r] == 0 ? SSG_REG_ROUTE_PATCH : 0;
		for (size_t k = 0; k < todo.size(); ++k) if (todo[k] >= 0 && todo[k] < n_reads) route[todo[k]] |= SSG_REG_ROUTE_WAVE;
	}
	*regs = out;
	return SSG_OK;
}

int ssg_dbg_reg2aln(const ssg_mem_opt_t *opt, const uint8_t *pac, int64_t l_pac, int n_ctg, const int64_t *ctg_off, const int32_t *ctg_len, int n_reads, const uint8_t *seq, const int64_t *off,
                    int64_t n_regs, const ssg_alnreg_t *regs, int64_t n_req, const ssg_alnreq_t *req, ssg_aln_t *alns, int32_t *route, int32_t *dev_err)
{
	CHK(ssg_need_device());
	if (dev_err) *dev_err = 0;
	if (n_reads < 0 || n_regs < 0 || n_req < 0 || n_req >= (int64_t)1 << 31 || l_pac < 1 || l_pac >= (int64_t)1 << 33 || n_ctg < 1) {
		ssg_err_msg = "ssg_dbg_reg2aln: need n_reads, n_regs >= 0, 0 <= n_req < 2^31, 1 <= l_pac < 2^33, n_ctg >= 1"; return SSG_EINVAL; }
	CHK(dbg_check_contigs("ssg_dbg_reg2aln", l_pac, n_ctg, ctg_off, ctg_len));
	if (n_req == 0) return SSG_OK;
	const char *bad = 0; long at = 0;
	int max_len = 0;
	if (n_reads < 1) bad = "requests need reads: request";
	else if (off[0] != 0) bad = "offsets start at 0: read";
	for (int r = 0; !bad && r < n_reads; ++r) {
		at = r;
		max_len = std::max(max_len, dbg_read_len(off, r, &bad));
		if (!bad) dbg_check_codes(seq, off, r, &bad);
	}
	for (int64_t k = 0; !bad && k < n_regs; ++k) {
		const ssg_alnreg_t &a = regs[k];
		at = (long)k;
		if (!(0 <= a.rb && a.rb < a.re && a.re <= 2 * l_pac)) bad = "need 0 <= rb < re <= 2 l_pac: region";
		else if (a.rb < l_pac && a.re > l_pac) bad = "a region must not cross the forward / reverse boundary l_pac: region";
		else if (a.re - a.rb > SSG_STAGE_TWIN_GLB) bad = "need re - rb <= 32768: region";
		else if (!(0 <= a.qb && a.qb < a.qe && a.qe <= SSG_MAX_READ_LEN)) bad = "need 0 <= qb < qe <= read length: region";
	}
	for (int64_t k = 0; !bad && k < n_req; ++k) {
		const ssg_alnreq_t &q = req[k];
		at = (long)k;
		if (q.read < 0 || q.read >= n_reads) bad = "read index out of range: request";
		else if (q.reg >= n_regs) bad = "region index out of range: request";
		else if (q.kind != SSG_REQ_MAIN && q.kind != SSG_REQ_XA) bad = "kind is SSG_REQ_MAIN or SSG_REQ_XA: request";
		else if (q.reg >= 0 && regs[q.reg].qe > off[q.read + 1] - off[q.read]) bad = "need 0 <= qb < qe <= read length for the request's region and read: request";
	}
	if (bad) return dbg_refuse("ssg_dbg_reg2aln", bad, at);
	CHK(check_band(opt)); CHK(check_scores(opt, max_len)); CHK(check_gap_penalties(opt));
	dbg_ref_t ref;
	CHK(ref.up(pac, l_pac, n_ctg, ctg_off, ctg_len));
	dbuf<uint8_t> d_seq((size_t)off[n_reads] + 1); dbuf<int64_t> d_off((size_t)n_reads + 1); dbuf<int32_t> d_gerr(1);
	dbuf<ssg_alnreg_t> d_regs((size_t)n_regs + 1); dbuf<ssg_alnreq_t> d_req((size_t)n_req + 1); dbuf<ssg_aln_t> d_alns((size_t)n_req + 1); dbuf<unsigned long long> d_cnt(3);
	CHKA(d_seq); CHKA(d_off); CHKA(d_gerr); CHKA(d_regs); CHKA(d_req); CHKA(d_alns); CHKA(d_cnt);
	CHK(d_seq.up(seq, (size_t)off[n_reads])); CHK(d_off.up(off, (size_t)n_reads + 1));
	if (n_regs) CHK(d_regs.up(regs, (size_t)n_regs));
	CHK(d_req.up(req, (size_t)n_req)); CHK(d_alns.zero()); CHK(d_gerr.zero()); CHK(d_cnt.zero());
	r2a_lists_t lists;
	CHK(run_reg2aln(ref.ix, opt, n_req, d_req.p, d_regs.p, d_seq.p, d_off.p, d_alns.p, d_gerr.p, d_cnt.p, max_len, &lists));
	int32_t ge = 0;
	CHK(d_gerr.down(&ge, 1));
	if (dev_err) *dev_err = ge;
	CHK(d_alns.down(alns, (size_t)n_req));
	if (route) {
		for (int64_t k = 0; k < n_req; ++k) route[k] = req[k].reg >= 0 ? SSG_R2A_ROUTE_LANE : 0;
		for (int c = 0; c < SSG_STAGE_R2D_CLASSES; ++c) for (int32_t g : lists.dp[c]) if (g >= 0 && g < n_req) route[g] = SSG_R2A_ROUTE_DP0 << c;
		for (int32_t g : lists.todo) if (g >= 0 && g < n_req) route[g] = (route[g] & ~SSG_R2A_ROUTE_LANE) | SSG_R2A_ROUTE_WAVE;
	}
	if (ge) { ssg_err_msg = "CIGAR generation exceeded an on-device capacity (code " + std::to_string(ge) + ")"; return SSG_EOVERFLOW; }
	return SSG_OK;
}

static int dbg_check_regs(const ssg_index_t *idx, int n_pairs, const int64_t *reg_off, const ssg_alnreg_t *regs, const char *who)
{
	const int n_reads = 2 * n_pairs;
	const char *bad = 0; long at = -1;
	if (n_pairs < 0 || n_pairs > (1 << 24)) { bad = "n_pairs out of range"; at = n_pairs; }
	else if (reg_off[0] != 0) { bad = "reg_off[0] != 0"; at = 0; }
	for (int r = 0; r < n_reads && !bad; ++r) {
		if (reg_off[r + 1] < reg_off[r] || reg_off[r + 1] - reg_off[r] > 4096) { bad = "reg_off not monotone, or more than 4096 regions in a read: read"; at = r; }
		else if (reg_off[r + 1] > (1LL << 28)) { bad = "too many regions in all: read"; at = r; }
	}
	for (int64_t k = 0; !bad && k < reg_off[n_reads]; ++k) {
		const ssg_alnreg_t &e = regs[k];
		if (e.rid < 0 || e.rid >= idx->v.n_ctg) bad = "rid out of range: region";
		else if (!(0 <= e.qb && e.qb < e.qe && e.qe <= 310)) bad = "need 0 <= qb < qe <= 310: region";
		else if (!(0 <= e.rb && e.rb < e.re && e.re <= 2 * idx->v.l_pac)) bad = "need 0 <= rb < re <= 2 l_pac: region";
		else if (e.score < 0 || e.score > (1 << 20) || e.csub < 0 || e.csub > (1 << 20)) bad = "score / csub out of range: region";
		else if (!(e.frac_rep >= 0 && e.frac_rep <= 1)) bad = "frac_rep outside [0, 1]: region";
		if (bad) at = (long)k;
	}
	return bad ? dbg_refuse(who, bad, at) : 0;
}

int ssg_dbg_pestat(const ssg_index_t *idx, const ssg_mem_opt_t *opt, int n_pairs, const int64_t *reg_off, const ssg_alnreg_t *regs,
                   const int32_t *pair_batch, int n_batches, ssg_pestat_t *pes)
{
	CHK(ssg_need_device());
	CHK(dbg_check_regs(idx, n_pairs, reg_off, regs, "ssg_dbg_pestat"));
	if (n_batches < 1 || n_batches > 64) { ssg_err_msg = "ssg_dbg_pestat: 1 <= n_batches <= 64"; return SSG_EINVAL; }
	for (int p = 0; p < n_pairs; ++p) if (pair_batch[p] < 0 || pair_batch[p] >= n_batches) { ssg_err_msg = "ssg_dbg_pestat: pair_batch out of range"; return SSG_EINVAL; }
	const int n_reads = 2 * n_pairs;
	const int64_t tot = reg_off[n_reads];
	const std::vector<int32_t> hn = dbg_counts(reg_off, n_reads);
	dbuf<int64_t> d_off((size_t)n_reads + 1); dbuf<ssg_alnreg_t> d_regs((size_t)tot + 1); dbuf<int32_t> d_n((size_t)n_reads + 1), d_pb((size_t)n_pairs + 1);
	CHKA(d_off); CHKA(d_regs); CHKA(d_n); CHKA(d_pb);
	CHK(d_off.up(reg_off, (size_t)n_reads + 1)); CHK(d_regs.up(regs, (size_t)tot)); CHK(d_n.up(hn.data(), (size_t)n_reads)); CHK(d_pb.up(pair_batch, (size_t)n_pairs));
	return run_pestat(idx, opt, n_pairs, d_off.p, d_regs.p, d_n.p, d_pb.p, n_batches, pes);
}

int ssg_dbg_pair_final(const ssg_index_t *idx, const ssg_mem_opt_t *opt, int n_pairs, int64_t id0, const int64_t *reg_off, const ssg_alnreg_t *regs,
                       const ssg_pestat_t pes[4], ssg_alnreg_t *regs_out, int64_t *req_off, ssg_alnreq_t **req)
{
	CHK(ssg_need_device());
	CHK(dbg_check_regs(idx, n_pairs, reg_off, regs, "ssg_dbg_pair_final"));
	for (int d = 0; d < 4; ++d) if (!pes[d].failed && !(pes[d].std > 0 && pes[d].low >= 0 && pes[d].low <= pes[d].high)) { ssg_err_msg = "ssg_dbg_pair_final: an orientation that has not failed needs std > 0 and 0 <= low <= high"; return SSG_EINVAL; }
	const int n_reads = 2 * n_pairs;
	const int64_t tot = reg_off[n_reads];
	*req = 0;
	if (n_pairs == 0) { req_off[0] = 0; return SSG_OK; }
	const std::vector<int32_t> hn = dbg_counts(reg_off, n_reads);
	dbuf<int64_t> d_off((size_t)n_reads + 1); dbuf<ssg_alnreg_t> d_regs((size_t)tot + 1); dbuf<int32_t> d_n((size_t)n_reads), d_pb((size_t)n_pairs); dbuf<ssg_pestat_t> d_pes(4);
	CHKA(d_off); CHKA(d_regs); CHKA(d_n); CHKA(d_pb); CHKA(d_pes);
	CHK(d_off.up(reg_off, (size_t)n_reads + 1)); CHK(d_regs.up(regs, (size_t)tot)); CHK(d_n.up(hn.data(), (size_t)n_reads)); CHK(d_pb.zero()); CHK(d_pes.up(pes, 4));
	pair_slices_t s;
	CHK(make_pair_slices(n_reads, d_off.p, d_regs.p, d_n.p, opt->max_matesw, s));
	dbuf<int32_t> d_perr(n_pairs), d_zbuf((size_t)s.t2 + 1), d_nreq(n_reads); dbuf<unsigned int> d_q(1); dbuf<ssg_alnreq_t> d_req((size_t)s.tq + 1);
	CHKA(d_perr); CHKA(d_zbuf); CHKA(d_nreq); CHKA(d_q); CHKA(d_req);
	CHK(d_perr.zero()); CHK(d_nreq.zero());
	CHK(run_pair_final(idx, opt, n_pairs, id0, s.t2, s.d_r2off.p, s.d_regs2.p, d_n.p, d_pb.p, d_pes.p, s.d_pkey.p, s.d_pw.p, d_zbuf.p, s.d_reqoff.p, d_req.p, d_nreq.p, d_perr.p, d_q.p));
	CHK(dev_copy_regs(n_reads, s.d_r2off.p, s.d_regs2.p, d_n.p, d_off.p, d_regs.p));
	pe_dev_t t;
	CHK(run_req_tail(n_reads, s.d_reqoff.p, d_req.p, d_nreq.p, 0, 0, t));
	CHK(rt_sync());
	const int64_t nreq = t.n_req;
	std::vector<int64_t> r2off((size_t)n_reads + 1);
	CHK(s.d_r2off.down(r2off.data(), (size_t)n_reads + 1)); CHK(t.req_off.down(req_off, (size_t)n_reads + 1)); CHK(d_regs.down(regs_out, (size_t)tot));
	ssg_alnreq_t *out = (ssg_alnreq_t*)malloc(sizeof(ssg_alnreq_t) * (size_t)(nreq + 1));
	if (!out) { ssg_err_msg = "host allocation failed: requests"; return SSG_ENOMEM; }
	int rc = t.req.down(out, (size_t)nreq);
	if (rc) { free(out); return rc; }
	for (int64_t k = 0; k < nreq; ++k) if (out[k].reg >= 0) out[k].reg = (int32_t)(out[k].reg - r2off[out[k].read] + reg_off[out[k].read]);
	*req = out;
	return SSG_OK;
}

int ssg_dbg_matesw(const ssg_index_t *idx, const ssg_mem_opt_t *opt, int n_pairs, const uint8_t *seq, const int64_t *read_off, const int64_t *reg_off, const ssg_alnreg_t *regs,
                   const uint8_t *fixed, const ssg_pestat_t pes[4], int headroom, int64_t *out_off, ssg_alnreg_t **regs_out, int32_t *n_out, int32_t *err, uint64_t counts[8])
{
	CHK(ssg_need_device());
	CHK(dbg_check_regs(idx, n_pairs, reg_off, regs, "ssg_dbg_matesw"));
	for (int d = 0; d < 4; ++d) if (!pes[d].failed && !(pes[d].low >= 0 && pes[d].low <= pes[d].high)) { ssg_err_msg = "ssg_dbg_matesw: an orientation that has not failed needs 0 <= low <= high"; return SSG_EINVAL; }
	const int n_reads = 2 * n_pairs;
	*regs_out = 0; memset(counts, 0, 8 * sizeof(uint64_t));
	if (n_pairs == 0) { out_off[0] = 0; return SSG_OK; }
	int max_len = 0;
	for (int r = 0; r < n_reads; ++r) {
		if (read_off[r + 1] <= read_off[r] || (r == 0 && read_off[0] != 0)) { ssg_err_msg = "ssg_dbg_matesw: read_off must start at 0 and increase"; return SSG_EINVAL; }
		max_len = std::max<int>(max_len, (int)std::min<int64_t>(read_off[r + 1] - read_off[r], 1 << 20));
	}
	if (max_len > SSG_MAX_READ_LEN) { ssg_err_msg = "reads longer than " SSG_STR(SSG_MAX_READ_LEN) " bases are outside this build's scope"; return SSG_EINVAL; }
	for (int64_t k = 0; k < read_off[n_reads]; ++k) if (seq[k] > 4) { ssg_err_msg = "ssg_dbg_matesw: bases are codes 0 .. 4"; return SSG_EINVAL; }
	for (int r = 0; r < n_reads; ++r) for (int64_t k = reg_off[r]; k < reg_off[r + 1]; ++k) if (regs[k].qe > (int)(read_off[r + 1] - read_off[r])) { ssg_err_msg = "ssg_dbg_matesw: a region ends beyond its read"; return SSG_EINVAL; }
	const std::vector<int32_t> hn = dbg_counts(reg_off, n_reads);
	std::vector<int32_t> hkey((size_t)n_pairs); std::vector<int64_t> r2off((size_t)n_reads + 1, 0); std::vector<uint8_t> hfix((size_t)n_reads, 0);
	for (int r = 0; r < n_reads; ++r) { const int m = hn[r ^ 1]; r2off[r + 1] = r2off[r] + hn[r] + (headroom >= 0 ? headroom : 4 * std::min(m, opt->max_matesw) + 4); if (fixed) hfix[r] = fixed[r] ? 1 : 0; }
	for (int p = 0; p < n_pairs; ++p) hkey[p] = hn[2 * p] + hn[2 * p + 1];
	const int64_t tot = reg_off[n_reads], t2 = r2off[n_reads];
	dbuf<uint8_t> d_seq((size_t)read_off[n_reads] + 1), d_fixed((size_t)n_reads); dbuf<int64_t> d_roff((size_t)n_reads + 1), d_off((size_t)n_reads + 1), d_r2off((size_t)n_reads + 1);
	dbuf<ssg_alnreg_t> d_regs((size_t)tot + 1), d_regs2((size_t)t2 + 1); dbuf<int32_t> d_n((size_t)n_reads), d_pb((size_t)n_pairs), d_pkey((size_t)n_pairs), d_pw((size_t)n_pairs), d_perr((size_t)n_pairs);
	dbuf<ssg_pestat_t> d_pes(4); dbuf<unsigned long long> d_cnt(3); dbuf<unsigned int> d_q(1);
	CHKA(d_seq); CHKA(d_fixed); CHKA(d_roff); CHKA(d_off); CHKA(d_r2off); CHKA(d_regs); CHKA(d_regs2); CHKA(d_n); CHKA(d_pb); CHKA(d_pkey); CHKA(d_pw); CHKA(d_perr); CHKA(d_pes); CHKA(d_cnt); CHKA(d_q);
	CHK(d_seq.up(seq, (size_t)read_off[n_reads])); CHK(d_fixed.up(hfix.data(), (size_t)n_reads)); CHK(d_roff.up(read_off, (size_t)n_reads + 1)); CHK(d_off.up(reg_off, (size_t)n_reads + 1));
	CHK(d_r2off.up(r2off.data(), (size_t)n_reads + 1)); CHK(d_regs.up(regs, (size_t)tot)); CHK(d_regs2.zero()); CHK(d_n.up(hn.data(), (size_t)n_reads)); CHK(d_pb.zero()); CHK(d_pkey.up(hkey.data(), (size_t)n_pairs));
	CHK(d_perr.zero()); CHK(d_pes.up(pes, 4)); CHK(d_cnt.zero()); CHK(d_q.zero());
	CHK(dev_order_desc(d_pkey.p, d_pw.p, n_pairs)); CHK(rt_sync());
	CHK(dev_copy_regs(n_reads, d_off.p, d_regs.p, d_n.p, d_r2off.p, d_regs2.p));
	msw_stage_t ms;
	CHK(run_matesw(idx, opt, n_pairs, d_seq.p, d_roff.p, max_len, d_r2off.p, d_regs2.p, d_n.p, d_pb.p, d_pes.p, d_pw.p, d_fixed.p, d_perr.p, d_cnt.p, d_q.p, &ms));
	ssg_alnreg_t *out = (ssg_alnreg_t*)malloc(sizeof(ssg_alnreg_t) * (size_t)(t2 + 1));
	if (!out) { ssg_err_msg = "host allocation failed: regions"; return SSG_ENOMEM; }
	int rc = d_regs2.down(out, (size_t)t2);
	if (!rc) rc = d_n.down(n_out, (size_t)n_reads);
	if (!rc) rc = d_perr.down(err, (size_t)n_pairs);
	if (rc) { free(out); return rc; }
	memcpy(out_off, r2off.data(), ((size_t)n_reads + 1) * sizeof(int64_t));
	msw_counts(ms, counts);
	*regs_out = out;
	return SSG_OK;
}

int ssg_dbg_sbl_records(long n_pairs, const int64_t *req_off, const ssg_alnreq_t *req, const ssg_aln_t *alns, const ssg_sbl_opt_t *o, ssg_sbl_state_t *st,
                        int64_t *line_off, int64_t *n_lines, ssg_sbl_line_t *lines, int64_t *line_req, ssg_sbl_end_t *ends, int64_t *prim, uint64_t *sig, uint8_t *dup,
                        uint8_t *bits, int64_t *mate_line, uint64_t counts[4], uint64_t *keys)
{
	const char *who = "ssg_dbg_sbl_records";
	CHK(ssg_need_device());
	*n_lines = 0; memset(counts, 0, 4 * sizeof(uint64_t));
	if (n_pairs < 0 || n_pairs >= (1L << 31)) { ssg_err_msg = "ssg_dbg_sbl_records: need 0 <= n_pairs < 2^31"; return SSG_EINVAL; }
	if (o->max_split_count > SSG_STAGE_SBL_MAX_SPLIT) { ssg_err_msg = "samblaster: --maxSplitCount above 16 is not supported"; return SSG_EINVAL; }
	if (n_pairs == 0) { line_off[0] = 0; return SSG_OK; }
	if (req_off[0] != 0) return dbg_refuse(who, "offsets start at 0: read", 0);
	const long n_reads = 2 * n_pairs;
	for (long r = 0; r < n_reads; ++r) {
		if (req_off[r + 1] < req_off[r]) return dbg_refuse(who, "offsets must not decrease: read", r);
		int n_main = 0;
		for (int64_t g = req_off[r]; g < req_off[r + 1]; ++g) {
			if (req[g].kind != SSG_REQ_MAIN && req[g].kind != SSG_REQ_XA) return dbg_refuse(who, "kind is SSG_REQ_MAIN or SSG_REQ_XA: request", (long)g);
			if (alns[g].n_cigar < 0 || alns[g].n_cigar > SSG_MAX_CIGAR) return dbg_refuse(who, "need 0 <= n_cigar <= " SSG_STR(SSG_MAX_CIGAR) ": record", (long)g);
			n_main += req[g].kind == SSG_REQ_MAIN;
		}
		if (!n_main) return dbg_refuse(who, "a read without a main request: read", r);
		if (req[req_off[r]].kind != SSG_REQ_MAIN) return dbg_refuse(who, "the first request of a read is a main one (its mate's lines print against it): read", r);
	}
	const size_t nreq = (size_t)req_off[n_reads];
	dbuf<int64_t> d_off((size_t)n_reads + 1); dbuf<ssg_alnreq_t> d_req(nreq + 1); dbuf<ssg_aln_t> d_alns(nreq + 1); dbuf<uint64_t> d_sig(3 * (size_t)n_pairs);
	CHKA(d_off); CHKA(d_req); CHKA(d_alns); CHKA(d_sig);
	CHK(d_off.up(req_off, (size_t)n_reads + 1)); CHK(d_req.up(req, nreq)); CHK(d_alns.up(alns, nreq));
	sbl_lines_t L;
	CHK(records_lines(n_pairs, d_off.p, d_req.p, d_alns.p, &L));
	CHK(records_dedup(st, n_pairs, L.ends.p, L.dup.p, d_sig.p));
	CHK(records_classify(n_pairs, &L, o, L.dup.p, counts));
	const size_t nl = (size_t)L.n_lines;
	dbuf<uint64_t> d_keys(nl + 1);
	CHKA(d_keys);
	CHK(records_export(&L, d_alns.p, d_keys.p, 0, 0));
	*n_lines = L.n_lines;
	CHK(L.line_off.down(line_off, (size_t)n_pairs + 1)); CHK(L.lines.down(lines, nl)); CHK(L.line_req.down(line_req, nl)); CHK(L.ends.down(ends, 2 * (size_t)n_pairs));
	CHK(L.prim.down(prim, 2 * (size_t)n_pairs)); CHK(d_sig.down(sig, 3 * (size_t)n_pairs)); CHK(L.dup.down(dup, (size_t)n_pairs)); CHK(L.bits.down(bits, nl));
	CHK(L.mate.down(mate_line, nl));
	return d_keys.down(keys, nl);
}
```

### speedseq_amd/csrc/ssg_dev.h

```cpp
#ifndef SSG_DEV_H
#define SSG_DEV_H
#include "ssg_types.h"

#ifdef SSG_EMU
#include "emu.h"
#define SSG_DEVFN static inline
#define SSG_DEVMEM inline
#define SSG_DEVFN_COLD static
SSG_DEVFN int wv_shfl(int v, int src) { return emu_shfl_i32(v, src); }
SSG_DEVFN unsigned long long wv_ballot(int p) { return emu_ballot(p); }
#define SSG_UNROLL
#else
#include <hip/hip_runtime.h>
#define SSG_DEVFN static __device__ __forceinline__
#define SSG_DEVMEM __device__ __forceinline__
#define SSG_DEVFN_COLD static __device__ __attribute__((noinline))
SSG_DEVFN int wv_shfl(int v, int src) { return __shfl(v, src, 64); }
SSG_DEVFN unsigned long long wv_ballot(int p) { return __ballot(p); }
#define SSG_UNROLL _Pragma("unroll")
#endif

#define SSG_WAVE 64
#ifdef SSG_EMU
static unsigned long long ssg_dbg_cyc[96];
#define SSG_TUNING 0
SSG_DEVFN unsigned long long ssg_clock() { return 0; }
#else
__device__ unsigned long long ssg_dbg_cyc[96];
#ifdef SSG_TUNE
#define SSG_TUNING 1
SSG_DEVFN unsigned long long ssg_clock() { return (unsigned long long)clock64(); }
#else
#define SSG_TUNING 0
SSG_DEVFN unsigned long long ssg_clock() { return 0; }
#endif
#endif
#ifdef SSG_EMU
SSG_DEVFN void ssg_wave_memsync() { (void)emu_ballot(0); }
#else
SSG_DEVFN void ssg_wave_memsync() { __builtin_amdgcn_fence(__ATOMIC_ACQ_REL, "workgroup"); }
#endif
#ifdef SSG_EMU
SSG_DEVFN void ssg_wave_ldssync() { (void)emu_ballot(0); }
#else
SSG_DEVFN void ssg_wave_ldssync() { __builtin_amdgcn_fence(__ATOMIC_ACQ_REL, "wavefront"); }
#endif
#define SSG_LANE0(...) do { ssg_wave_memsync(); if (wv_lane() == 0) { __VA_ARGS__; } ssg_wave_memsync(); } while (0)

SSG_DEVFN int wv_lane() { return (int)(threadIdx.x & 63); }

#ifdef SSG_EMU
SSG_DEVFN int wv_prev(int v, int fill) { int l = wv_lane(); int r = wv_shfl(v, l - 1); return l == 0 ? fill : r; }
SSG_DEVFN int wv_get(int v, int src) { return wv_shfl(v, src); }
SSG_DEVFN int wv_scan_max(int v)
{
	int l = wv_lane();
	for (int d = 1; d < 64; d <<= 1) { int o = wv_shfl(v, l - d); if (l >= d) v = v > o ? v : o; }
	return v;
}
SSG_DEVFN int wv_sum(int v) { for (int d = 1; d < 64; d <<= 1) v += wv_shfl(v, wv_lane() ^ d); return v; }
SSG_DEVFN int wv_scan_add(int v)
{
	int l = wv_lane();
	for (int d = 1; d < 64; d <<= 1) { int o = wv_shfl(v, l - d); if (l >= d) v += o; }
	return v;
}
#else
#define SSG_DPP(old, src, ctrl, rmask) __builtin_amdgcn_update_dpp((old), (src), (ctrl), (rmask), 0xf, false)
SSG_DEVFN int wv_prev(int v, int fill) { return SSG_DPP(fill, v, 0x138 , 0xf); }
SSG_DEVFN int wv_get(int v, int src) { return __builtin_amdgcn_readlane(v, __builtin_amdgcn_readfirstlane(src)); }
SSG_DEVFN int wv_scan_max(int v)
{
	int t;
	const int id = (int)0x80000000;
	t = SSG_DPP(id, v, 0x111, 0xf); v = v > t ? v : t;
	t = SSG_DPP(id, v, 0x112, 0xf); v = v > t ? v : t;
	t = SSG_DPP(id, v, 0x114, 0xf); v = v > t ? v : t;
	t = SSG_DPP(id, v, 0x118, 0xf); v = v > t ? v : t;
	t = SSG_DPP(id, v, 0x142 , 0xa); v = v > t ? v : t;
	t = SSG_DPP(id, v, 0x143 , 0xc); v = v > t ? v : t;
	return v;
}
SSG_DEVFN int wv_sum(int v)
{
	v += SSG_DPP(0, v, 0x111, 0xf); v += SSG_DPP(0, v, 0x112, 0xf); v += SSG_DPP(0, v, 0x114, 0xf); v += SSG_DPP(0, v, 0x118, 0xf);
	v += SSG_DPP(0, v, 0x142, 0xa); v += SSG_DPP(0, v, 0x143, 0xc);
	return __builtin_amdgcn_readlane(v, 63);
}
SSG_DEVFN int wv_scan_add(int v)
{
	v += SSG_DPP(0, v, 0x111, 0xf); v += SSG_DPP(0, v, 0x112, 0xf); v += SSG_DPP(0, v, 0x114, 0xf); v += SSG_DPP(0, v, 0x118, 0xf);
	v += SSG_DPP(0, v, 0x142, 0xa); v += SSG_DPP(0, v, 0x143, 0xc);
	return v;
}
#endif
SSG_DEVFN int wv_last(int v) { return wv_get(v, 63); }
SSG_DEVFN long wv_queue_pop(unsigned int *queue)
{
	int k = 0;
	if (wv_lane() == 0) k = (int)atomicAdd(queue, 1u);
	return (long)(unsigned)wv_get(k, 0);
}
SSG_DEVFN int wv_bcast(int v, int src) { return wv_get(v, src); }
SSG_DEVFN long long wv_bcast64(long long v, int src)
{
	int lo = wv_shfl((int)(unsigned)(unsigned long long)v, src), hi = wv_shfl((int)((unsigned long long)v >> 32), src);
	return (long long)((unsigned long long)(unsigned)lo | (unsigned long long)(unsigned)hi << 32);
}
SSG_DEVFN long long wv_shfl64_xor(long long v, int d)
{
	const int src = wv_lane() ^ d;
	int lo = wv_shfl((int)(unsigned)(unsigned long long)v, src), hi = wv_shfl((int)((unsigned long long)v >> 32), src);
	return (long long)((unsigned long long)(unsigned)lo | (unsigned long long)(unsigned)hi << 32);
}
SSG_DEVFN long long wv_get64(long long v, int src)
{
	int lo = wv_get((int)(unsigned)(unsigned long long)v, src), hi = wv_get((int)((unsigned long long)v >> 32), src);
	return (long long)((unsigned long long)(unsigned)lo | (unsigned long long)(unsigned)hi << 32);
}
SSG_DEVFN int wv_rank_of(unsigned long long ballot) { return __popcll(ballot & ((1ull << wv_lane()) - 1ull)); }
SSG_DEVFN int wv_max(int v) { return wv_last(wv_scan_max(v)); }
SSG_DEVFN int wv_min(int v) { return -wv_max(-v); }
SSG_DEVFN int imax(int a, int b) { return a > b ? a : b; }
SSG_DEVFN int imin(int a, int b) { return a < b ? a : b; }
SSG_DEVFN int iabs(int a) { return a < 0 ? -a : a; }
SSG_DEVFN long long lmax(long long a, long long b) { return a > b ? a : b; }
SSG_DEVFN long long lmin(long long a, long long b) { return a < b ? a : b; }

SSG_DEVFN int ssg_cnt16(uint32_t w, int c, int nsym)
{
	uint32_t m = ~(w ^ ((uint32_t)c * 0x55555555u));
	uint32_t t = m & (m >> 1) & 0x55555555u;
	if (nsym < 16) t &= nsym ? ~((1u << ((16 - nsym) << 1)) - 1) : 0u;
	return __popc(t);
}
SSG_DEVFN void ssg_occ4(const ssg_index_view_t &ix, uint64_t k, uint64_t cnt[4])
{
	if (k == (uint64_t)-1) { cnt[0] = cnt[1] = cnt[2] = cnt[3] = 0; return; }
	k -= (k >= ix.primary);
	const uint32_t *p = ix.bwt + ((k >> 7) << 4);
	struct alignas(16) q16 { uint32_t v[4]; };
	const q16 *pb = (const q16*)p;
	const q16 c0 = pb[0], c1 = pb[1], w0 = pb[2], w1 = pb[3];
	const uint32_t w[8] = { w0.v[0], w0.v[1], w0.v[2], w0.v[3], w1.v[0], w1.v[1], w1.v[2], w1.v[3] };
	const uint64_t pc[4] = { (uint64_t)c0.v[0] | (uint64_t)c0.v[1] << 32, (uint64_t)c0.v[2] | (uint64_t)c0.v[3] << 32,
	                         (uint64_t)c1.v[0] | (uint64_t)c1.v[1] << 32, (uint64_t)c1.v[2] | (uint64_t)c1.v[3] << 32 };
	const int r = (int)(k & 127) + 1;
	uint32_t mk[8];
	SSG_UNROLL for (int i = 0; i < 8; ++i) { int ns = r - i * 16; ns = ns < 0 ? 0 : ns > 16 ? 16 : ns; mk[i] = ns == 16 ? 0x55555555u : ns ? (~((1u << ((16 - ns) << 1)) - 1)) & 0x55555555u : 0u; }
	SSG_UNROLL for (int c = 0; c < 4; ++c) {
		int n = 0;
		SSG_UNROLL for (int i = 0; i < 8; ++i) { const uint32_t m = ~(w[i] ^ ((uint32_t)c * 0x55555555u)); n += __popc(m & (m >> 1) & mk[i]); }
		cnt[c] = pc[c] + (uint64_t)n;
	}
}
SSG_DEVFN uint64_t ssg_occ1(const ssg_index_view_t &ix, uint64_t k, int c)
{
	if (k == ix.seq_len) return ix.L2[c+1] - ix.L2[c];
	if (k == (uint64_t)-1) return 0;
	k -= (k >= ix.primary);
	const uint32_t *p = ix.bwt + ((k >> 7) << 4);
	uint64_t n = ((const uint64_t*)p)[c];
	int r = (int)(k & 127) + 1;
	SSG_UNROLL for (int i = 0; i < 8; ++i) { int ns = r - i * 16; ns = ns < 0 ? 0 : ns > 16 ? 16 : ns; if (ns) n += ssg_cnt16(p[8 + i], c, ns); }
	return n;
}
SSG_DEVFN int ssg_bwt_sym(const ssg_index_view_t &ix, uint64_t k)
{
	const uint32_t *p = ix.bwt + ((k >> 7) << 4) + 8;
	return p[(k & 127) >> 4] >> ((~k & 15) << 1) & 3;
}
SSG_DEVFN uint64_t ssg_lf_step(const ssg_index_view_t &ix, uint64_t k)
{
	const uint64_t x = k - (k > ix.primary);
	struct alignas(16) q16 { uint32_t v[4]; };
	const q16 *pb = (const q16*)(ix.bwt + ((x >> 7) << 4));
	const q16 c01 = pb[0], c23 = pb[1], w0 = pb[2], w1 = pb[3];
	const uint32_t w[8] = { w0.v[0], w0.v[1], w0.v[2], w0.v[3], w1.v[0], w1.v[1], w1.v[2], w1.v[3] };
	const int r = (int)(x & 127), wi = r >> 4;
	uint32_t ww = 0;
	SSG_UNROLL for (int i = 0; i < 8; ++i) if (i == wi) ww = w[i];
	const int c = (int)(ww >> ((~r & 15) << 1)) & 3;
	const uint64_t cnt[4] = { (uint64_t)c01.v[0] | (uint64_t)c01.v[1] << 32, (uint64_t)c01.v[2] | (uint64_t)c01.v[3] << 32, (uint64_t)c23.v[0] | (uint64_t)c23.v[1] << 32, (uint64_t)c23.v[2] | (uint64_t)c23.v[3] << 32 };
	uint64_t n = 0;
	SSG_UNROLL for (int i = 0; i < 4; ++i) if (i == c) n = cnt[i];
	const int upto = r + 1;
	SSG_UNROLL for (int i = 0; i < 8; ++i) { int ns = upto - i * 16; ns = ns < 0 ? 0 : ns > 16 ? 16 : ns; n += (uint64_t)ssg_cnt16(w[i], c, ns); }
	return ix.L2[c] + n;
}
SSG_DEVFN void ssg_bwt_extend(const ssg_index_view_t &ix, const ssg_intv_t &ik, ssg_intv_t ok[4], int is_back)
{
	uint64_t tk[4], tl[4];
	uint64_t kx = is_back ? ik.x0 : ik.x1, ox = is_back ? ik.x1 : ik.x0;
	ssg_occ4(ix, kx - 1, tk);
	ssg_occ4(ix, kx - 1 + ik.x2, tl);
	uint64_t nk[4], ns[4], no[4];
	for (int i = 0; i < 4; ++i) { nk[i] = ix.L2[i] + 1 + tk[i]; ns[i] = tl[i] - tk[i]; }
	no[3] = ox + (kx <= ix.primary && kx + ik.x2 - 1 >= ix.primary);
	no[2] = no[3] + ns[3];
	no[1] = no[2] + ns[2];
	no[0] = no[1] + ns[1];
	for (int i = 0; i < 4; ++i) {
		ok[i].x2 = ns[i];
		if (is_back) { ok[i].x0 = nk[i]; ok[i].x1 = no[i]; } else { ok[i].x1 = nk[i]; ok[i].x0 = no[i]; }
	}
}
SSG_DEVFN ssg_intv_t ssg_bwt_extend1(const ssg_index_view_t &ix, const ssg_intv_t &ik, int c, int is_back)
{
	uint64_t tk[4], tl[4];
	const uint64_t kx = is_back ? ik.x0 : ik.x1, ox = is_back ? ik.x1 : ik.x0;
	ssg_occ4(ix, kx - 1, tk);
	ssg_occ4(ix, kx - 1 + ik.x2, tl);
	uint64_t no = ox + (kx <= ix.primary && kx + ik.x2 - 1 >= ix.primary);
	SSG_UNROLL for (int b = 3; b >= 0; --b) if (b > c) no += tl[b] - tk[b];
	uint64_t tkc = tk[0], tlc = tl[0];
	SSG_UNROLL for (int b = 1; b < 4; ++b) if (b == c) { tkc = tk[b]; tlc = tl[b]; }
	ssg_intv_t o;
	const uint64_t nk = ix.L2[c] + 1 + tkc;
	o.x2 = tlc - tkc; o.info = 0;
	if (is_back) { o.x0 = nk; o.x1 = no; } else { o.x1 = nk; o.x0 = no; }
	return o;
}
struct alignas(16) ssg_q16_t { uint32_t v[4]; };
SSG_DEVFN void ssg_cnt_pair(const ssg_q16_t &w0, const ssg_q16_t &w1, int r, int c, int &na, int &nb)
{
	const uint32_t w[8] = { w0.v[0], w0.v[1], w0.v[2], w0.v[3], w1.v[0], w1.v[1], w1.v[2], w1.v[3] };
	const uint32_t hc = (c & 2) ? 0u : 0xffffffffu;
	const int r2 = r << 1;
	int nt = 0, n1 = 0;
	SSG_UNROLL for (int i = 0; i < 8; ++i) {
		int sh = 32 * (i + 1) - r2; sh = sh < 0 ? 0 : sh > 31 ? 31 : sh;
		const uint32_t hs = (((w[i] >> 1) ^ hc) & 0x55555555u) >> sh;
		nt += __popc(hs); n1 += __popc(hs & (w[i] >> sh));
	}
	na = nt - n1; nb = n1;
}
SSG_DEVFN ssg_intv_t ssg_bwt_extend1_lean(const ssg_index_view_t &ix, const ssg_intv_t &ik, int c, int is_back)
{
	const uint64_t kx = is_back ? ik.x0 : ik.x1, ox = is_back ? ik.x1 : ik.x0;
	const uint64_t k = kx - 1, l = k + ik.x2;
	const bool kneg = k == (uint64_t)-1, lneg = l == (uint64_t)-1;
	const uint64_t k2 = kneg ? 0 : k - (k >= ix.primary), l2 = lneg ? 0 : l - (l >= ix.primary);
	const ssg_q16_t *const pk = (const ssg_q16_t*)(ix.bwt + ((k2 >> 7) << 4)), *const pl = (const ssg_q16_t*)(ix.bwt + ((l2 >> 7) << 4));
	const int rk = (int)(k2 & 127) + 1, rl = (int)(l2 & 127) + 1;
	const bool same = (k2 >> 7) == (l2 >> 7);
	ssg_q16_t z; z.v[0] = z.v[1] = z.v[2] = z.v[3] = 0;
	const ssg_q16_t cql = pl[c >> 1], w0l = pl[2];
	ssg_q16_t w1l = z;
	if (rl > 64) w1l = pl[3];
	ssg_q16_t cqk = z, w0k = z, w1k = z;
	if (!same) { cqk = pk[c >> 1]; w0k = pk[2]; if (rk > 64) w1k = pk[3]; }
	uint32_t sm = same ? 0xffffffffu : 0u;
#if !defined(SSG_EMU) && !defined(SSG_NO_ASM_PINS)
	asm("" : "+v"(sm));
#endif
	SSG_UNROLL for (int i = 0; i < 4; ++i) { cqk.v[i] |= cql.v[i] & sm; w0k.v[i] |= w0l.v[i] & sm; w1k.v[i] |= w1l.v[i] & sm; }
	int nak, nbk, nal, nbl;
	ssg_cnt_pair(w0k, w1k, rk, c, nak, nbk);
	ssg_cnt_pair(w0l, w1l, rl, c, nal, nbl);
	const uint64_t oak = ((uint64_t)cqk.v[0] | (uint64_t)cqk.v[1] << 32) + (uint64_t)nak, obk = ((uint64_t)cqk.v[2] | (uint64_t)cqk.v[3] << 32) + (uint64_t)nbk;
	const uint64_t oal = ((uint64_t)cql.v[0] | (uint64_t)cql.v[1] << 32) + (uint64_t)nal, obl = ((uint64_t)cql.v[2] | (uint64_t)cql.v[3] << 32) + (uint64_t)nbl;
	const uint64_t Tk = k2 + 1, Tl = l2 + 1;
	uint64_t tkc = (c & 1) ? obk : oak, tkg = c == 0 ? Tk - oak : c == 1 ? Tk - oak - obk : c == 2 ? obk : 0;
	uint64_t tlc = (c & 1) ? obl : oal, tlg = c == 0 ? Tl - oal : c == 1 ? Tl - oal - obl : c == 2 ? obl : 0;
	if (kneg) tkc = tkg = 0;
	if (lneg) tlc = tlg = 0;
	const uint64_t no = ox + (kx <= ix.primary && kx + ik.x2 - 1 >= ix.primary) + (tlg - tkg);
	uint64_t L0 = ix.L2[0], L1 = ix.L2[1], L2v = ix.L2[2], L3 = ix.L2[3];
#if !defined(SSG_EMU) && !defined(SSG_NO_ASM_PINS)
	asm("" : "+s"(L0)); asm("" : "+s"(L1)); asm("" : "+s"(L2v)); asm("" : "+s"(L3));
#endif
	const uint64_t l2c = c == 0 ? L0 : c == 1 ? L1 : c == 2 ? L2v : L3;
	ssg_intv_t o;
	const uint64_t nk = l2c + 1 + tkc;
	o.x2 = tlc - tkc; o.info = 0;
	if (is_back) { o.x0 = nk; o.x1 = no; } else { o.x1 = nk; o.x0 = no; }
	return o;
}

SSG_DEVFN uint64_t ssg_bwt_sa(const ssg_index_view_t &ix, uint64_t k)
{
	uint64_t sa = 0, mask = (uint64_t)ix.sa_intv - 1;
	while (k & mask) {
		++sa;
		if (k == ix.primary) { k = 0; continue; }
		k = ssg_lf_step(ix, k);
	}
	return sa + ix.sa[k / (uint64_t)ix.sa_intv];
}

SSG_DEVFN int ssg_ref_base(const ssg_index_view_t &ix, int64_t p)
{
	int64_t q = p < ix.l_pac ? p : (ix.l_pac << 1) - 1 - p;
	int b = ix.pac[q >> 2] >> ((~q & 3) << 1) & 3;
	return p < ix.l_pac ? b : 3 - b;
}
SSG_DEVFN int ssg_pos2rid(const ssg_index_view_t &ix, int64_t pos_f)
{
	if (pos_f >= ix.l_pac) return -1;
	int left = 0, mid = 0, right = ix.n_ctg;
	while (left < right) {
		mid = (left + right) >> 1;
		if (pos_f >= ix.ctg_off[mid]) {
			if (mid == ix.n_ctg - 1) break;
			if (pos_f < ix.ctg_off[mid + 1]) break;
			left = mid + 1;
		} else right = mid;
	}
	return mid;
}
SSG_DEVFN int64_t ssg_depos(const ssg_index_view_t &ix, int64_t pos, int *is_rev)
{
	return (*is_rev = (pos >= ix.l_pac)) ? (ix.l_pac << 1) - 1 - pos : pos;
}
SSG_DEVFN int ssg_intv2rid(const ssg_index_view_t &ix, int64_t rb, int64_t re)
{
	int is_rev;
	if (rb < ix.l_pac && re > ix.l_pac) return -2;
	int rid_b = ssg_pos2rid(ix, ssg_depos(ix, rb, &is_rev));
	int rid_e = rb < re ? ssg_pos2rid(ix, ssg_depos(ix, re - 1, &is_rev)) : rid_b;
	return rid_b == rid_e ? rid_b : -1;
}
SSG_DEVFN int ssg_intv2rid_1(const ssg_index_view_t &ix, int64_t rb, int64_t re)
{
	int is_rev;
	if (rb < ix.l_pac && re > ix.l_pac) return -2;
	const int rid_b = ssg_pos2rid(ix, ssg_depos(ix, rb, &is_rev));
	if (rb >= re || rid_b < 0) return rid_b;
	const int64_t pe = ssg_depos(ix, re - 1, &is_rev);
	const int64_t lo = ix.ctg_off[rid_b], hi = rid_b == ix.n_ctg - 1 ? ix.l_pac : ix.ctg_off[rid_b + 1];
	return pe >= lo && pe < hi ? rid_b : -1;
}
SSG_DEVFN int ssg_score(const ssg_mem_opt_t &o, int t, int q) { return o.mat[t * 5 + q]; }

template <class T, class LT>
SSG_DEVFN void ssg_insertsort(T *s, T *t, LT lt)
{
	for (T *i = s + 1; i < t; ++i)
		for (T *j = i; j > s && lt(*j, *(j - 1)); --j) { T x = *j; *j = *(j - 1); *(j - 1) = x; }
}
template <class T, class LT>
SSG_DEVFN void ssg_combsort(T *a, long n, LT lt)
{
	const double shrink = 1.2473309501039786540366528676643;
	int do_swap; long gap = n;
	do {
		if (gap > 2) { gap = (long)(gap / shrink); if (gap == 9 || gap == 10) gap = 11; }
		do_swap = 0;
		for (T *i = a; i < a + n - gap; ++i) {
			T *j = i + gap;
			if (lt(*j, *i)) { T x = *i; *i = *j; *j = x; do_swap = 1; }
		}
	} while (do_swap || gap > 2);
	if (gap != 1) ssg_insertsort(a, a + n, lt);
}
template <class T, class LT>
SSG_DEVFN void ssg_introsort(T *a, long n, LT lt)
{
	struct { T *l, *r; int d; } stack[40]; int top = 0;
	int d; T rp, *s, *t, *i, *j, *k;
	if (n < 1) return;
	if (n == 2) { if (lt(a[1], a[0])) { T x = a[0]; a[0] = a[1]; a[1] = x; } return; }
	for (d = 2; (1l << d) < n; ++d);
	s = a; t = a + (n - 1); d <<= 1;
	for (;;) {
		if (s < t) {
			if (--d == 0) { ssg_combsort(s, t - s + 1, lt); t = s; continue; }
			i = s; j = t; k = i + ((j - i) >> 1) + 1;
			if (lt(*k, *i)) { if (lt(*k, *j)) k = j; }
			else k = lt(*j, *i) ? i : j;
			rp = *k;
			if (k != t) { T x = *k; *k = *t; *t = x; }
			for (;;) {
				do ++i; while (lt(*i, rp));
				do --j; while (i <= j && lt(rp, *j));
				if (j <= i) break;
				T x = *i; *i = *j; *j = x;
			}
			{ T x = *i; *i = *t; *t = x; }
			if (i - s > t - i) {
				if (i - s > 16) { stack[top].l = s; stack[top].r = i - 1; stack[top].d = d; ++top; }
				s = t - i > 16 ? i + 1 : t;
			} else {
				if (t - i > 16) { stack[top].l = i + 1; stack[top].r = t; stack[top].d = d; ++top; }
				t = i - s > 16 ? i - 1 : s;
			}
		} else {
			if (top == 0) { ssg_insertsort(a, a + n, lt); return; }
			--top; s = stack[top].l; t = stack[top].r; d = stack[top].d;
		}
	}
}
template <class A, class LT>
SSG_DEVFN void ssg_insertsort_ix(A a, int s, int t, LT lt)
{
	for (int i = s + 1; i < t; ++i)
		for (int j = i; j > s; --j) { const auto x = a.get(j), y = a.get(j - 1); if (!lt(x, y)) break; a.set(j, y); a.set(j - 1, x); }
// ... 60 lines not shown
```

### speedseq_amd/csrc/ssg_index_int.h

```cpp
#ifndef SSG_INDEX_INT_H
#define SSG_INDEX_INT_H
#include <vector>
#include <string>
#include <mutex>
#include <string.h>
#include "ssg_types.h"

struct ssg_hole_t { int64_t offset; int32_t len; char amb; };

struct ssg_index {
	ssg_index_view_t v;
	uint32_t *bwt; uint64_t *sa; uint8_t *pac; int64_t *ctg_off; int32_t *ctg_len;
	uint64_t *ktab; int ktab_k;
	uint64_t bwt_words;
	bool raw_alloc;
	std::vector<std::string> names, annos;
	std::vector<int32_t> n_ambs;
	std::vector<ssg_hole_t> holes;
	std::vector<int64_t> h_off; std::vector<int32_t> h_len;
	std::mutex names_mu; char *d_names; int32_t *d_name_off;
	ssg_index() : bwt(0), sa(0), pac(0), ctg_off(0), ctg_len(0), ktab(0), ktab_k(0), bwt_words(0), raw_alloc(false), d_names(0), d_name_off(0) { memset(&v, 0, sizeof(v)); }
};
extern "C" int ssg_index_build_ktab(ssg_index *ix);
extern "C" int ssg_seed_smem2(const ssg_index *idx, const ssg_mem_opt_t *opt, int n_reads, const uint8_t *d_seq, const int64_t *d_off, int max_len, int cap,
                              ssg_intv_t *d_intv, int32_t *d_n, unsigned long long *n_extend, unsigned int max_ext, uint32_t *d_n_ext_read);
extern "C" int ssg_sa_verify(const ssg_index *ix, int new_intv, const uint64_t *d_sa_new, long n_new);
extern "C" int ssg_crc32_ranges_dev(const uint8_t *d_data, const uint64_t *d_cut, long n, uint32_t *d_crc);
extern "C" int ssg_bgzf_frame_dev(const uint8_t *d_tmp, uint32_t tmp_stride, const uint64_t *d_cut, const uint64_t *d_moff, const uint32_t *d_crc, long n_blocks, uint8_t *d_dense);
extern "C" int ssg_bgzf_deep_depth(int level);
extern "C" size_t ssg_bgzf_deep_scratch(long nb);
extern "C" int ssg_bgzf_deflate_deep_dev(const uint8_t *d_pay, const uint64_t *d_cut, long nb, uint8_t *d_tmp, uint32_t *d_sym, uint32_t *d_size, uint16_t *d_prev, int depth);
extern "C" int ssg_bgzf_walk_members(const char *who, const uint8_t *members, const uint64_t *moff, long n_blocks, uint64_t *rng, uint64_t *out_off);
extern "C" int ssg_bgzf_inflate_dev(const uint8_t *d_in, const uint64_t *d_rng, const uint64_t *d_ooff, long nb, uint8_t *d_out, int32_t *d_st, uint32_t *d_crc);
struct ssg_recs;
extern "C" int ssg_recs_gather_dev(const ssg_recs *r, uint64_t v0, uint64_t v1, uint8_t *d_out);

#include <stddef.h>
struct ssg_abi_fp_t { uint32_t v[20]; };
#ifdef __clang__
#pragma clang diagnostic push
#pragma clang diagnostic ignored "-Winvalid-offsetof"
#else
#pragma GCC diagnostic push
#pragma GCC diagnostic ignored "-Winvalid-offsetof"
#endif
static inline ssg_abi_fp_t ssg_abi_fp_make()
{
	ssg_abi_fp_t f = {{ (uint32_t)sizeof(ssg_index_view_t), (uint32_t)sizeof(ssg_mem_opt_t), (uint32_t)sizeof(ssg_index), (uint32_t)sizeof(ssg_intv_t),
		(uint32_t)offsetof(ssg_index_view_t, primary), (uint32_t)offsetof(ssg_index_view_t, L2), (uint32_t)offsetof(ssg_index_view_t, l_pac), (uint32_t)offsetof(ssg_index_view_t, sa_intv),
		(uint32_t)offsetof(ssg_mem_opt_t, min_seed_len), (uint32_t)offsetof(ssg_mem_opt_t, split_width), (uint32_t)offsetof(ssg_mem_opt_t, max_mem_intv), (uint32_t)offsetof(ssg_mem_opt_t, split_factor),
		(uint32_t)offsetof(ssg_mem_opt_t, mat), (uint32_t)offsetof(ssg_index, bwt), (uint32_t)offsetof(ssg_index, ktab), (uint32_t)offsetof(ssg_index, bwt_words),
		(uint32_t)offsetof(ssg_index, names), (uint32_t)sizeof(ssg_seed_t), (uint32_t)sizeof(ssg_alnreg_t), (uint32_t)sizeof(ssg_aln_t) }};
	return f;
}
#ifdef __clang__
#pragma clang diagnostic pop
#else
#pragma GCC diagnostic pop
#endif
#define SSG_ABI_FP_DEFINE(unit) extern "C" void ssg_abi_fp_##unit(ssg_abi_fp_t *out) { *out = ssg_abi_fp_make(); }
extern "C" int ssg_abi_selfcheck(void);
#endif
```

### speedseq_amd/csrc/ssg_seed.cpp

```cpp
#include <algorithm>
#include "ssg_rt.h"
#include "k_smem2.h"
#include "../../include/ssgpu.h"
#include "ssg_index_int.h"

SSG_ABI_FP_DEFINE(seed)
static int env_int(const char *name, int dflt) { const char *e = getenv(name); return e && *e ? atoi(e) : dflt; }
static int budget_row(unsigned int max_ext) { return max_ext < 0x7fffffffu ? env_int("SSG_SMEM_MAX_ROW", 32) : 0x7fffffff; }

static constexpr auto ssg_k_smem2_plain = ssg_k_smem2<false, false>;
static constexpr auto ssg_k_smem2_kt = ssg_k_smem2<false, true>;
static constexpr auto ssg_k_smem2_tune = ssg_k_smem2<true, false>;
static constexpr auto ssg_k_smem2_kt_tune = ssg_k_smem2<true, true>;

extern "C" int ssg_seed_smem2(const ssg_index *idx, const ssg_mem_opt_t *opt, int n_reads, const uint8_t *d_seq, const int64_t *d_off, int max_len, int cap,
                              ssg_intv_t *d_intv, int32_t *d_n, unsigned long long *n_extend, unsigned int max_ext, uint32_t *d_n_ext_read)
{
	const int block = 64;
	const long nthreads = std::min<long>(((long)n_reads + block - 1) / block * block, 256L * env_int("SSG_SMEM_WAVES_PER_CU", 16) * 64)   ;
	const int scap = max_len + 2;
	const int kt_want = idx->ktab ? std::min(idx->ktab_k, opt->min_seed_len - 1) : 0;
	const int kt_k = kt_want >= 2 ? kt_want : 0;
	const ssg_pk2_t *const kt = kt_k ? (const ssg_pk2_t*)idx->ktab : (const ssg_pk2_t*)0;
	dbuf<ssg_pk2_t> scratch((size_t)nthreads * 2 * scap + 64);
	dbuf<unsigned int> d_next(4);
	const int max_row = budget_row(max_ext);
	const bool budget = max_ext < 0x7fffffffu;
	dbuf<int32_t> d_heavy(budget ? (size_t)n_reads : 1);
	if (!scratch.ok() || !d_next.ok() || !d_heavy.ok()) { ssg_err_msg = "device allocation failed: seeding work lists"; return SSG_ENOMEM; }
	CHK(d_next.zero());
	int32_t *const hv = budget ? d_heavy.p : (int32_t*)0;
	if (env_int("SSG_S2_TUNE", 0)) {
		unsigned long long st[64]; memset(st, 0, sizeof(st)); st[0] = st[1] = ~0ull;
#ifdef SSG_EMU
		memcpy(ssg_s2_stat, st, sizeof(st));
#else
		CHK(rt_sync()); CHK(rt_check(hipMemcpyToSymbol(HIP_SYMBOL(ssg_s2_stat), st, sizeof(st)), "hipMemcpyToSymbol"));
#endif
		if (kt) SSG_LAUNCH(ssg_k_smem2_kt_tune, nthreads / block, block, 0, idx->v, *opt, n_reads, (const int32_t*)0, d_seq, d_off, d_intv, d_n, cap, scratch.p, scap, n_extend, d_next.p, max_ext, max_row, d_n_ext_read, hv, d_next.p + 1, kt, kt_k);
		else SSG_LAUNCH(ssg_k_smem2_tune, nthreads / block, block, 0, idx->v, *opt, n_reads, (const int32_t*)0, d_seq, d_off, d_intv, d_n, cap, scratch.p, scap, n_extend, d_next.p, max_ext, max_row, d_n_ext_read, hv, d_next.p + 1, kt, kt_k);
		CHK(rt_sync());
#ifdef SSG_EMU
		memcpy(st, ssg_s2_stat, sizeof(st));
#else
		CHK(rt_check(hipMemcpyFromSymbol(st, HIP_SYMBOL(ssg_s2_stat), sizeof(st)), "hipMemcpyFromSymbol"));
#endif
		fprintf(stderr, "[ssgpu] smem2 timeline (ms): pool of reads empty at %.2f, last lane done at %.2f; %llu reads given up at %u extensions / rows of %d; rounds %llu, lanes ready %.1f, with a read %.1f of 64\n",
		        (double)(st[1] - st[0]) / 1e5, (double)(st[2] - st[0]) / 1e5, st[3], max_ext, max_row, st[48], st[48] ? (double)st[49] / st[48] : 0., st[48] ? (double)st[50] / st[48] : 0.);
		fprintf(stderr, "[ssgpu] smem2 reads by extensions (< 2^b):");
		for (int b = 1; b <= 24; ++b) if (st[8 + b]) fprintf(stderr, " b%d=%llu", b, st[8 + b]);
		fprintf(stderr, "\n");
	} else if (kt) SSG_LAUNCH(ssg_k_smem2_kt, nthreads / block, block, 0, idx->v, *opt, n_reads, (const int32_t*)0, d_seq, d_off, d_intv, d_n, cap, scratch.p, scap, n_extend, d_next.p, max_ext, max_row, d_n_ext_read, hv, d_next.p + 1, kt, kt_k);
	else SSG_LAUNCH(ssg_k_smem2_plain, nthreads / block, block, 0, idx->v, *opt, n_reads, (const int32_t*)0, d_seq, d_off, d_intv, d_n, cap, scratch.p, scap, n_extend, d_next.p, max_ext, max_row, d_n_ext_read, hv, d_next.p + 1, kt, kt_k);
	if (budget) {
		const long n_wg = std::min<long>(n_reads, 256L * env_int("SSG_SMEM_HEAVY_WAVES_PER_CU", 28));
		if (scap <= 160) SSG_LAUNCH(ssg_k_smem_heavy<160>, n_wg, block, 0, idx->v, *opt, (const int32_t*)d_heavy.p, (const unsigned int*)(d_next.p + 1), (const int32_t*)0, d_seq, d_off, d_intv, d_n, cap, n_extend, d_next.p + 2);
		else if (scap <= 264) SSG_LAUNCH(ssg_k_smem_heavy<264>, n_wg, block, 0, idx->v, *opt, (const int32_t*)d_heavy.p, (const unsigned int*)(d_next.p + 1), (const int32_t*)0, d_seq, d_off, d_intv, d_n, cap, n_extend, d_next.p + 2);
		else SSG_LAUNCH(ssg_k_smem_heavy<328>, n_wg, block, 0, idx->v, *opt, (const int32_t*)d_heavy.p, (const unsigned int*)(d_next.p + 1), (const int32_t*)0, d_seq, d_off, d_intv, d_n, cap, n_extend, d_next.p + 2);
	}
	return rt_sync();
}

extern "C" int ssg_index_build_ktab(ssg_index *ix)
{
	int lg = 0; while ((ix->v.seq_len >> (2 * (lg + 1))) != 0) ++lg;
	int K = env_int("SSG_KTAB_K", std::min(13, lg - 2));
	K = std::min(K, std::min(15, lg + 2));
	rt_free(ix->ktab); ix->ktab = 0; ix->ktab_k = 0;
	if (K < 2 || ix->v.seq_len >= (1ull << 40)) return 0;
	const size_t n_ent = (size_t)((((1ull << (2 * (K + 1))) - 4ull) / 3ull));
	ix->ktab = (uint64_t*)rt_malloc(n_ent * 16);
	if (!ix->ktab) { ssg_err_msg = "index allocation failed: table of short-pattern intervals"; return SSG_ENOMEM; }
	for (int j = 1; j <= K; ++j) { const long np = 1L << (2 * (j - 1)); SSG_LAUNCH(ssg_k_ktab_level, (np + 255) / 256, 256, 0, ix->v, j, (ssg_pk2_t*)ix->ktab); }
	CHK(rt_sync());
	if (env_int("SSG_KTAB_VERIFY", 0)) {
		dbuf<unsigned long long> d_bad(16); unsigned long long bad[16];
		if (!d_bad.ok()) { ssg_err_msg = "device allocation failed"; return SSG_ENOMEM; }
		CHK(d_bad.zero());
		for (int j = 1; j <= K; ++j) { const long np = 1L << (2 * j), stride = np > (1L << 22) ? np >> 22 : 1, nt = (np + stride - 1) / stride; SSG_LAUNCH(ssg_k_ktab_verify, (nt + 255) / 256, 256, 0, ix->v, j, stride, (const ssg_pk2_t*)ix->ktab, d_bad.p); }
		CHK(rt_sync()); CHK(d_bad.down(bad, 16));
		fprintf(stderr, "[ssgpu] table of short-pattern intervals, K = %d; entries that differ from forward extension, per level:", K);
		for (int j = 1; j <= K; ++j) fprintf(stderr, " %llu", bad[j]);
		fprintf(stderr, "\n");
	}
	ix->ktab_k = K;
	return 0;
}

extern "C" int ssg_sa_verify(const ssg_index *ix, int new_intv, const uint64_t *d_sa_new, long n_new)
{
	const long stride = n_new > (1L << 24) ? n_new >> 24 : 1, nt = (n_new + stride - 1) / stride;
	dbuf<unsigned long long> d_bad(1); unsigned long long bad = 0;
	if (!d_bad.ok()) { ssg_err_msg = "device allocation failed"; return SSG_ENOMEM; }
	CHK(d_bad.zero());
	SSG_LAUNCH(ssg_k_sa_verify, (nt + 255) / 256, 256, 0, ix->v, new_intv, d_sa_new, n_new, stride, d_bad.p);
	CHK(rt_sync()); CHK(d_bad.down(&bad, 1));
	fprintf(stderr, "[ssgpu] SA samples every %d rows: %llu of %ld checked entries differ from bwt_sa on the file's samples\n", new_intv, bad, nt);
	return 0;
}
```

Before: 5.462 million pairs/s.

## Use cooperative wave BWT extension, k-mer table starts, and resume in heavy SMEM kernel

The wave-per-read heavy SMEM kernel now computes each forward BWT extension with 16 lanes cooperating on the occurrence block. Small backward rows (up to four intervals) use a four-group cooperative variant. Forward searches start from the precomputed short-pattern interval table instead of extending base by base. Reads handed off from the lane kernel now resume from a saved phase and position instead of restarting pass 1, which avoids redoing work at the cost of a per-read resume buffer and extra shuffles. Debug entry points and tuning counters are also added.

```diff
diff --git a/include/ssgpu.h b/include/ssgpu.h
--- a/include/ssgpu.h
+++ b/include/ssgpu.h
@@ -65,6 +65,11 @@
 
 int ssg_align2_lane_batch(const ssg_index_t *idx, const ssg_mem_opt_t *opt, int n_jobs, const ssg_sw_job_t *jobs, const int64_t *tpos,
                           const uint8_t *qbuf, size_t qbytes, int lanes, ssg_kswr_t *res, int32_t *from_lane);
+
+int ssg_dbg_extend_coop(const ssg_index_t *idx, int n, const ssg_intv_t *in, const uint8_t *base, const uint8_t *is_back, ssg_intv_t *out_lean, ssg_intv_t *out_coop,
+                        ssg_intv_t *out_lean4, ssg_intv_t *out_coop4);
+int ssg_dbg_smem_ext(const ssg_index_t *idx, const ssg_mem_opt_t *opt, int n_reads, const uint8_t *seq, const int64_t *off, int cap, ssg_intv_t *out_intv, int32_t *out_n,
+                     uint64_t *n_extend, uint32_t paths[4]);
 
 int ssg_dbg_chain_sort(const int64_t *keys, int n, int64_t *out_lane, int64_t *out_wave);
 
diff --git a/speedseq_amd/capi.py b/speedseq_amd/capi.py
--- a/speedseq_amd/capi.py
+++ b/speedseq_amd/capi.py
@@ -137,6 +137,23 @@
         self._chk(self.l.ssg_smem_batch(idx, _ptr(opt), C.c_int(n), _ptr(seq), _ptr(off), C.c_int(cap), _ptr(intv), _ptr(cnt)))
         return intv, cnt
 
+    def dbg_smem_ext(self, idx, opt, seq, off, cap=64):
+        n = len(off) - 1
+        intv = np.zeros((n, cap), dtype=INTV_DT)
+        cnt = np.zeros(n, dtype=np.int32)
+        nx = C.c_uint64(0)
+        paths = np.zeros(4, dtype=np.uint32)
+        self._chk(self.l.ssg_dbg_smem_ext(idx, _ptr(opt), C.c_int(n), _ptr(seq), _ptr(off), C.c_int(cap), _ptr(intv), _ptr(cnt), C.byref(nx), _ptr(paths)))
+        return intv, cnt, nx.value, [int(x) for x in paths]
+
+    def dbg_extend_coop(self, idx, intv, base, is_back):
+        intv = np.ascontiguousarray(intv, dtype=INTV_DT)
+        base, is_back = np.ascontiguousarray(base, dtype=np.uint8), np.ascontiguousarray(is_back, dtype=np.uint8)
+        n = len(intv)
+        lean, coop, lean4, coop4 = np.zeros(n, dtype=INTV_DT), np.zeros(n, dtype=INTV_DT), np.zeros((n, 4), dtype=INTV_DT), np.zeros((n, 4), dtype=INTV_DT)
+        self._chk(self.l.ssg_dbg_extend_coop(idx, C.c_int(n), _ptr(intv), _ptr(base), _ptr(is_back), _ptr(lean), _ptr(coop), _ptr(lean4), _ptr(coop4)))
+        return lean, coop, lean4, coop4
+
     def seeds_batch(self, idx, opt, seq, off):
         n = len(off) - 1
         seed_off = np.zeros(n + 1, dtype=np.int64)
diff --git a/speedseq_amd/csrc/k_smem2.h b/speedseq_amd/csrc/k_smem2.h
--- a/speedseq_amd/csrc/k_smem2.h
+++ b/speedseq_amd/csrc/k_smem2.h
@@ -43,31 +43,137 @@
 #endif
 SSG_DEVFN ssg_intv_t wv_uni_intv(const ssg_intv_t &v) { ssg_intv_t o; o.x0 = wv_uni64(v.x0); o.x1 = wv_uni64(v.x1); o.x2 = wv_uni64(v.x2); o.info = wv_uni64(v.info); return o; }
 
+SSG_DEVFN ssg_intv_t s2_coop_tail(const ssg_index_view_t &ix, const ssg_intv_t &ik, const int c, const int is_back, const int prk, const int prl, const uint32_t ck[4], const uint32_t cl[4])
+{
+	const uint64_t kx = is_back ? ik.x0 : ik.x1, ox = is_back ? ik.x1 : ik.x0;
+	const uint64_t k = kx - 1, l = k + ik.x2;
+	const bool kneg = k == (uint64_t)-1, lneg = l == (uint64_t)-1;
+	const uint64_t k2 = kneg ? 0 : k - (k >= ix.primary), l2 = lneg ? 0 : l - (l >= ix.primary);
+	const int nbk = prk >> 16, nak = (prk & 0xffff) - nbk, nbl = prl >> 16, nal = (prl & 0xffff) - nbl;
+	const uint64_t oak = ((uint64_t)ck[0] | (uint64_t)ck[1] << 32) + (uint64_t)nak, obk = ((uint64_t)ck[2] | (uint64_t)ck[3] << 32) + (uint64_t)nbk;
+	const uint64_t oal = ((uint64_t)cl[0] | (uint64_t)cl[1] << 32) + (uint64_t)nal, obl = ((uint64_t)cl[2] | (uint64_t)cl[3] << 32) + (uint64_t)nbl;
+	const uint64_t Tk = k2 + 1, Tl = l2 + 1;
+	uint64_t tkc = (c & 1) ? obk : oak, tkg = c == 0 ? Tk - oak : c == 1 ? Tk - oak - obk : c == 2 ? obk : 0;
+	uint64_t tlc = (c & 1) ? obl : oal, tlg = c == 0 ? Tl - oal : c == 1 ? Tl - oal - obl : c == 2 ? obl : 0;
+	if (kneg) tkc = tkg = 0;
+	if (lneg) tlc = tlg = 0;
+	const uint64_t no = ox + (kx <= ix.primary && kx + ik.x2 - 1 >= ix.primary) + (tlg - tkg);
+	const uint64_t nk = ix.L2[c] + 1 + tkc;
+	ssg_intv_t o;
+	o.x2 = tlc - tkc; o.info = 0;
+	if (is_back) { o.x0 = nk; o.x1 = no; } else { o.x1 = nk; o.x0 = no; }
+	return o;
+}
+
+SSG_DEVFN ssg_intv_t s2_extend_coop(const ssg_index_view_t &ix, const ssg_intv_t &ik, const int c, const int is_back)
+{
+	const int l16 = wv_lane() & 15, up = l16 >> 3, wi = l16 & 7;
+	const uint64_t kx = is_back ? ik.x0 : ik.x1, ox = is_back ? ik.x1 : ik.x0;
+	const uint64_t k = kx - 1, l = k + ik.x2;
+	const bool kneg = k == (uint64_t)-1, lneg = l == (uint64_t)-1;
+	const uint64_t k2 = kneg ? 0 : k - (k >= ix.primary), l2 = lneg ? 0 : l - (l >= ix.primary);
+	const uint64_t q2 = up ? l2 : k2;
+	const uint32_t *const blk = ix.bwt + ((q2 >> 7) << 4);
+	const uint32_t w = blk[8 + wi];
+	ssg_q16_t cq; cq.v[0] = cq.v[1] = cq.v[2] = cq.v[3] = 0;
+	if (wi == 0) cq = ((const ssg_q16_t*)blk)[c >> 1];
+	int sh = 32 * (wi + 1) - (((int)(q2 & 127) + 1) << 1); sh = sh < 0 ? 0 : sh > 31 ? 31 : sh;
+	const uint32_t hs = (((w >> 1) ^ ((c & 2) ? 0u : 0xffffffffu)) & 0x55555555u) >> sh;
+	const int pr = wv_seg8_sum(__popc(hs) | __popc(hs & (w >> sh)) << 16);
+	const int prk = wv_get(pr, 7), prl = wv_get(pr, 15);
+	uint32_t ck[4], cl[4];
+	SSG_UNROLL for (int i = 0; i < 4; ++i) { ck[i] = (uint32_t)wv_get((int)cq.v[i], 0); cl[i] = (uint32_t)wv_get((int)cq.v[i], 8); }
+	return s2_coop_tail(ix, ik, c, is_back, prk, prl, ck, cl);
+}
+
+SSG_DEVFN ssg_intv_t s2_extend_coop4(const ssg_index_view_t &ix, const ssg_intv_t &ik, const int c, const int is_back)
+{
+	const int l16 = wv_lane() & 15, up = l16 >> 3, wi = l16 & 7;
+	const uint64_t kx = is_back ? ik.x0 : ik.x1, ox = is_back ? ik.x1 : ik.x0;
+	const uint64_t k = kx - 1, l = k + ik.x2;
+	const bool kneg = k == (uint64_t)-1, lneg = l == (uint64_t)-1;
+	const uint64_t k2 = kneg ? 0 : k - (k >= ix.primary), l2 = lneg ? 0 : l - (l >= ix.primary);
+	const uint64_t q2 = up ? l2 : k2;
+	const uint32_t *const blk = ix.bwt + ((q2 >> 7) << 4);
+	const uint32_t w = blk[8 + wi];
+	const ssg_q16_t cq = ((const ssg_q16_t*)blk)[c >> 1];
+	int sh = 32 * (wi + 1) - (((int)(q2 & 127) + 1) << 1); sh = sh < 0 ? 0 : sh > 31 ? 31 : sh;
+	const uint32_t hs = (((w >> 1) ^ ((c & 2) ? 0u : 0xffffffffu)) & 0x55555555u) >> sh;
+	const int pr = wv_seg8_allsum(__popc(hs) | __popc(hs & (w >> sh)) << 16), po = wv_xor8(pr);
+	const int prk = up ? po : pr, prl = up ? pr : po;
+	uint32_t ck[4], cl[4];
+	SSG_UNROLL for (int i = 0; i < 4; ++i) { const uint32_t o = (uint32_t)wv_xor8((int)cq.v[i]); ck[i] = up ? o : cq.v[i]; cl[i] = up ? cq.v[i] : o; }
+	return s2_coop_tail(ix, ik, c, is_back, prk, prl, ck, cl);
+}
+
+SSG_DEVFN long s2_ktab_off(int j) { return (long)(((1ull << (2 * j)) - 4ull) / 3ull); }
+struct alignas(16) ssg_s2_resume_t { uint32_t w[4]; };
+enum { S2_PATH_RESUME_P1 = 0, S2_PATH_RESUME_P2, S2_PATH_RESTART_P3, S2_PATH_P1_FROM_0, S2_PATH_N };
+enum { S2_WC_READS = 0, S2_WC_FWD, S2_WC_P3, S2_WC_BWD, S2_WC_ROW4, S2_WC_ROW16, S2_WC_ROW64, S2_WC_ROWMORE, S2_WC_EXT, S2_WC_TABSTART, S2_WC_TABEXT, S2_WC_N };
 SSG_DEVFN unsigned long long s2_wave_read(const ssg_index_view_t &ix, const ssg_mem_opt_t &opt, const int split_len, const int it, const int32_t *read_ids, const uint8_t *seq, const int64_t *off,
-                                          ssg_intv_t *out_intv, int32_t *out_n, const int cap, uint8_t *qb, ssg_pk2_t *l0, ssg_pk2_t *l1)
+                                          ssg_intv_t *out_intv, int32_t *out_n, const int cap, uint8_t *qb, ssg_pk2_t *l0, ssg_pk2_t *l1, const ssg_pk2_t *kt_tab, const int kt_k,
+                                          const ssg_s2_resume_t *resume, unsigned int *paths)
 {
 	const int lane = wv_lane();
 	unsigned long long nx = 0;
+	unsigned int wc[S2_WC_N];
+	for (int t = 0; t < S2_WC_N; ++t) wc[t] = 0;
 	const int r = read_ids ? read_ids[it] : it;
 	const uint8_t *q = seq + off[r];
 	const int len = (int)(off[r+1] - off[r]);
 	ssg_wave_ldssync();
 	for (int b = lane; b < len; b += 64) qb[b] = q[b];
 	ssg_wave_ldssync();
+	auto kt_run = [&](const int b, uint32_t &code) -> int {
+		const int qc = lane < kt_k && b + lane < len ? (int)qb[b + lane] : 4;
+		const int run = __ffsll(wv_ballot(qc > 3)) - 1;
+		code = (uint32_t)wv_sum(lane < run ? (qc & 3) << (2 * lane) : 0);
+		return run;
+	};
 	ssg_intv_t *const mem = out_intv + (long)it * cap;
 	const int left = -2 - out_n[it];
 	const bool skip_p3 = left >= 1;
 	const int n_p3 = skip_p3 ? left - 1 : 0;
 	int mem_n = n_p3, ovf = 0;
+	int phase = 1, x0 = 0, k0 = n_p3, old_n_rec = 0;
+	if (skip_p3 && resume) {
+		const ssg_s2_resume_t rec = resume[it];
+		const int w0 = wv_uni((int)rec.w[0]);
+		phase = w0 & 255; mem_n = wv_uni((int)rec.w[1]); old_n_rec = wv_uni((int)rec.w[2]);
+		if (phase == 1) x0 = w0 >> 8; else k0 = w0 >> 8;
+	}
+	if (paths && lane == 0) atomicAdd(&paths[!skip_p3 ? S2_PATH_RESTART_P3 : phase == 2 ? S2_PATH_RESUME_P2 : x0 > 0 ? S2_PATH_RESUME_P1 : S2_PATH_P1_FROM_0], 1u);
 	auto smem1 = [&](const int sx, uint64_t min_intv) -> int {
 		if (min_intv < 1) min_intv = 1;
-		ssg_intv_t ik; s2_set_intv(ix, (int)qb[sx], ik); ik.info = (uint64_t)(sx + 1);
+		ssg_intv_t ik;
 		int n = 0, i = sx + 1;
 		bool stop = false;
+		uint32_t code = 0;
+		const int run = kt_k >= 2 ? kt_run(sx, code) : 0;
+		if (run >= 2) {
+			const bool has = lane >= 1 && lane <= run, ext = lane >= 2 && lane <= run;
+			const int jl = has ? lane : 1;
+			ssg_pk2_t e; e.w0 = e.w1 = 0;
+			if (has) e = kt_tab[s2_ktab_off(jl) + (long)(code & ((1u << (2 * jl)) - 1u))];
+			ssg_intv_t ev = s2_unpk(e);
+			const uint64_t px2 = (uint64_t)(uint32_t)wv_prev((int)(uint32_t)ev.x2, 0) | (uint64_t)(uint32_t)wv_prev((int)(uint32_t)(ev.x2 >> 32), 0) << 32;
+			const unsigned long long stopm = wv_ballot(ext && ev.x2 != px2 && ev.x2 < min_intv);
+			const int jstop = stopm ? __ffsll(stopm) - 1 : run + 1;
+			const unsigned long long pm = wv_ballot(ext && lane <= jstop && ev.x2 != px2) >> 1;
+			if (pm >> lane & 1) { ev.info = (uint64_t)(sx + lane); l0[__popcll(pm & ((1ull << lane) - 1ull))] = s2_pk(ev); }
+			n = __popcll(pm);
+			stop = stopm != 0;
+			const int src = stop ? jstop - 1 : run;
+			nx += (unsigned long long)((stop ? jstop : run) - 1);
+			ssg_pk2_t u; u.w0 = (uint64_t)wv_get64((long long)e.w0, src); u.w1 = (uint64_t)wv_get64((long long)e.w1, src);
+			ik = s2_unpk(u); ik.info = (uint64_t)(sx + src); i = sx + src;
+			if (SSG_TUNING) { ++wc[S2_WC_TABSTART]; wc[S2_WC_TABEXT] += (unsigned int)((stop ? jstop : run) - 1); }
+		} else { s2_set_intv(ix, wv_uni((int)qb[sx]), ik); ik.info = (uint64_t)(sx + 1); }
 		while (!stop && i < len) {
 			const int cq = wv_uni((int)qb[i]);
 			if (cq < 4) {
-				const ssg_intv_t ok = wv_uni_intv(ssg_bwt_extend1_lean(ix, ik, 3 - cq, 0)); ++nx;
+				const ssg_intv_t ok = s2_extend_coop(ix, ik, 3 - cq, 0); ++nx;
+				if (SSG_TUNING) ++wc[S2_WC_FWD];
 				if (ok.x2 != ik.x2) { l0[n++] = s2_pk(ik); stop = ok.x2 < min_intv; }
 				if (!stop) { ik = ok; ik.info = (uint64_t)(i + 1); ++i; }
 			} else { l0[n++] = s2_pk(ik); stop = true; }
@@ -85,8 +191,15 @@
 				ssg_intv_t p; p.x0 = p.x1 = p.x2 = p.info = 0;
 				if (valid) p = s2_unpk((cur ? l1 : l0)[rev ? prev_n - 1 - jj : jj]);
 				ssg_intv_t okc; okc.x0 = okc.x1 = okc.x2 = okc.info = 0;
-				if (valid && cb >= 0) okc = ssg_bwt_extend1_lean(ix, p, cb, 1);
+				if (cb >= 0 && prev_n <= 4) {
+					const int g = lane >> 4, ge = g < prev_n ? g : 0;
+					const ssg_intv_t og = s2_extend_coop4(ix, s2_unpk((cur ? l1 : l0)[rev ? prev_n - 1 - ge : ge]), cb, 1);
+					const int src = (lane & 3) << 4;
+					const uint64_t g0 = (uint64_t)wv_bcast64((long long)og.x0, src), g1 = (uint64_t)wv_bcast64((long long)og.x1, src), g2 = (uint64_t)wv_bcast64((long long)og.x2, src);
+					if (valid) { okc.x0 = g0; okc.x1 = g1; okc.x2 = g2; }
+				} else if (valid && cb >= 0) okc = ssg_bwt_extend1_lean(ix, p, cb, 1);
 				if (cb >= 0) nx += (unsigned long long)(prev_n - base < 64 ? prev_n - base : 64);
+				if (SSG_TUNING && cb >= 0) { ++wc[S2_WC_BWD]; ++wc[prev_n <= 4 ? S2_WC_ROW4 : prev_n <= 16 ? S2_WC_ROW16 : prev_n <= 64 ? S2_WC_ROW64 : S2_WC_ROWMORE]; }
 				const bool alive = valid && cb >= 0 && okc.x2 >= min_intv;
 				if (base == 0 && !wv_get((int)alive, 0)) {
 					const int beg = ib + 1;
@@ -118,11 +231,11 @@
 		return ret;
 	};
 	if (len >= opt.min_seed_len) {
-		int x = 0;
+		int x = phase == 1 ? x0 : len;
 		while (x < len) { if (wv_uni((int)qb[x]) < 4) x = smem1(x, 1); else ++x; }
-		const int old_n = mem_n < cap ? mem_n : cap;
+		const int old_n = phase == 1 ? (mem_n < cap ? mem_n : cap) : old_n_rec;
 		ssg_wave_memsync();
-		for (int k = n_p3; k < old_n; ++k) {
+		for (int k = k0; k < old_n; ++k) {
 			const ssg_intv_t m = wv_uni_intv(mem[k]);
 			const int start = (int)(m.info >> 32), end = (int)(uint32_t)m.info;
 			if (end - start >= split_len && m.x2 <= (uint64_t)opt.split_width) {
@@ -135,12 +248,22 @@
 			while (x < len) {
 				if (wv_uni((int)qb[x]) > 3) ++x;
 				else {
-					ssg_intv_t ik; s2_set_intv(ix, (int)qb[x], ik);
+					ssg_intv_t ik;
 					int i = x + 1, nxt = len; bool stop = false;
+					uint32_t code = 0;
+					const int run = kt_k >= 2 ? kt_run(x, code) : 0;
+					if (kt_k >= 2 && run < kt_k) { nx += (unsigned long long)(run - 1); nxt = x + run >= len ? len : x + run + 1; stop = true; ik.x0 = ik.x1 = ik.x2 = ik.info = 0; }
+					else if (kt_k >= 2) {
+						const ssg_pk2_t e = kt_tab[s2_ktab_off(kt_k) + (long)code];
+						ssg_pk2_t u; u.w0 = wv_uni64(e.w0); u.w1 = wv_uni64(e.w1);
+						ik = s2_unpk(u); i = x + kt_k; nx += (unsigned long long)(kt_k - 1);
+						if (SSG_TUNING) { ++wc[S2_WC_TABSTART]; wc[S2_WC_TABEXT] += (unsigned int)(kt_k - 1); }
+					} else s2_set_intv(ix, wv_uni((int)qb[x]), ik);
 					while (!stop && i < len) {
 						const int cq = wv_uni((int)qb[i]);
 						if (cq < 4) {
-							const ssg_intv_t ok = wv_uni_intv(ssg_bwt_extend1_lean(ix, ik, 3 - cq, 0)); ++nx;
+							const ssg_intv_t ok = s2_extend_coop(ix, ik, 3 - cq, 0); ++nx;
+							if (SSG_TUNING) ++wc[S2_WC_P3];
 							if (ok.x2 < (uint64_t)opt.max_mem_intv && i - x >= opt.min_seed_len) {
 								if (ok.x2 > 0) {
 									if (mem_n < cap) { if (lane == 0) { ssg_intv_t o = ok; o.info = (uint64_t)x << 32 | (uint64_t)(i + 1); mem[mem_n] = o; } } else ovf = 1;
@@ -156,10 +279,14 @@
 		}
 	}
 	if (lane == 0) out_n[it] = ovf ? -1 : mem_n;
+	if (SSG_TUNING && lane == 0) {
+		wc[S2_WC_READS] = 1;
+		for (int t = 0; t < S2_WC_N; ++t) if (t != S2_WC_EXT && wc[t]) S2_STAT_ADD(52 + t, wc[t]);
+		S2_STAT_ADD(52 + S2_WC_EXT, nx);
+	}
 	return nx;
 }
 
-SSG_DEVFN long s2_ktab_off(int j) { return (long)(((1ull << (2 * j)) - 4ull) / 3ull); }
 __global__ void ssg_k_ktab_level(ssg_index_view_t ix, int j, ssg_pk2_t *tab)
 {
 	const long p = (long)blockIdx.x * blockDim.x + threadIdx.x;
@@ -200,7 +327,8 @@
 __global__ void __launch_bounds__(64, SSG_S2_WAVES) ssg_k_smem2(ssg_index_view_t ix, ssg_mem_opt_t opt, int n_reads, const int32_t *read_ids,
                            const uint8_t *seq, const int64_t *off, ssg_intv_t *out_intv, int32_t *out_n, int cap,
                            ssg_pk2_t *scratch, int scap, unsigned long long *n_extend, unsigned int *next_read, unsigned int max_ext, int max_row, uint32_t *n_ext_read, int32_t *heavy_ids, unsigned int *n_heavy,
-                           const ssg_pk2_t *kt_tab, int kt_k )
+                           const ssg_pk2_t *kt_tab, int kt_k ,
+                           ssg_s2_resume_t *resume )
 {
 	__shared__ uint32_t qlds[SSG_S2_QWORDS * 64];
 	const long gt = (long)blockIdx.x * blockDim.x + threadIdx.x;
@@ -212,6 +340,8 @@
 	const int split_len = (int)(opt.min_seed_len * opt.split_factor + .499);
 	unsigned long long my_nx = 0;
 	unsigned int rd_nx = 0, nx_p3 = 0;
+	unsigned int nx_call = 0; int mem_call = 0;
+#define S2_CALL() do { nx_call = rd_nx; mem_call = mem_n; } while (0)
 	long it = 0;
 	int state = S2_READ, pend = S2_PEND_NONE;
 	int len = 0, x = 0, k = 0, old_n = 0, caller = 0, mem_n = 0, ovf = 0, heavy = 0, n_p3 = -1;
@@ -298,7 +428,7 @@
 			} else if (state == S2_P1) {
 				if (x >= len) { old_n = mem_n < cap ? mem_n : cap; k = n_p3 > 0 ? n_p3 : 0; state = S2_P2; }
 				else if (S2Q(x) > 3) ++x;
-				else { sx = x; min_intv = 1; caller = 1; state = S2_FWD; m1_n = 0; curr_n = 0; i = sx + 1; s2_set_intv(ix, S2Q(sx), ik); ik.info = (uint64_t)(sx + 1); }
+				else { S2_CALL(); sx = x; min_intv = 1; caller = 1; state = S2_FWD; m1_n = 0; curr_n = 0; i = sx + 1; s2_set_intv(ix, S2Q(sx), ik); ik.info = (uint64_t)(sx + 1); }
 			} else if (state == S2_P2) {
 				if (k >= old_n) state = S2_OUT;
 				else {
@@ -306,6 +436,7 @@
 					const int start = (int)(m.info >> 32), end = (int)(uint32_t)m.info;
 					if (end - start < split_len || m.x2 > (uint64_t)opt.split_width) ++k;
 					else {
+						S2_CALL();
 						sx = (start + end) >> 1; min_intv = m.x2 + 1; caller = 2; m1_n = 0; curr_n = 0; i = sx + 1;
 						if (S2Q(sx) > 3) S2_RET();
 						else { s2_set_intv(ix, S2Q(sx), ik); ik.info = (uint64_t)(sx + 1); state = S2_FWD; }
@@ -317,9 +448,19 @@
 				const bool given_up = heavy != 0;
 				out_n[it] = ovf ? -1 : given_up ? (n_p3 < 0 ? -2 : -3 - n_p3) : mem_n;
 				if (given_up && !ovf && heavy_ids) heavy_ids[atomicAdd(n_heavy, 1u)] = (int32_t)it;
-				if (given_up) my_nx -= n_p3 < 0 ? rd_nx : rd_nx - nx_p3;
+				const bool fresh = rd_nx == nx_p3;
+				if (given_up && n_p3 >= 0 && resume) {
+					ssg_s2_resume_t rec_;
+					rec_.w[0] = fresh ? 1u : (unsigned int)caller | (unsigned int)(caller == 1 ? sx : k) << 8;
+					rec_.w[1] = (unsigned int)(fresh ? n_p3 : mem_call); rec_.w[2] = (unsigned int)old_n; rec_.w[3] = fresh ? rd_nx : nx_call;
+					resume[it] = rec_;
+				}
+				if (given_up) my_nx -= n_p3 < 0 || !resume ? (n_p3 < 0 ? rd_nx : rd_nx - nx_p3) : fresh ? 0u : rd_nx - nx_call;
 				if (n_ext_read) n_ext_read[it] = rd_nx;
 				if (TUNE) { S2_STAT_ADD(8 + (64 - __clzll((unsigned long long)(rd_nx | 1u))), 1); if (given_up) S2_STAT_ADD(3, 1); }
+#if SSG_TUNING
+				if (TUNE && given_up && n_p3 >= 0) { S2_STAT_ADD(4, nx_call - nx_p3); S2_STAT_ADD(5, rd_nx - nx_p3); }
+#endif
 				state = S2_READ;
 			}
 		}
@@ -376,6 +517,7 @@
 #undef S2_P3END
 #undef S2_RET
 #undef S2_EMIT
+#undef S2_CALL
 	if (n_extend && my_nx) atomicAdd(n_extend, my_nx);
 }
 
@@ -386,7 +528,9 @@
 #endif
 template <int SC>
 __global__ void SSG_HEAVY_BOUNDS ssg_k_smem_heavy(ssg_index_view_t ix, ssg_mem_opt_t opt, const int32_t *ids, const unsigned int *n_ids, const int32_t *read_ids,
-                           const uint8_t *seq, const int64_t *off, ssg_intv_t *out_intv, int32_t *out_n, int cap, unsigned long long *n_extend, unsigned int *next)
+                           const uint8_t *seq, const int64_t *off, ssg_intv_t *out_intv, int32_t *out_n, int cap, unsigned long long *n_extend, unsigned int *next,
+                           const ssg_pk2_t *kt_tab, int kt_k ,
+                           const ssg_s2_resume_t *resume , unsigned int *paths )
 {
 	__shared__ uint8_t qb[328];
 	__shared__ ssg_pk2_t lst[2][SC];
@@ -396,7 +540,7 @@
 	for (;;) {
 		const long t = wv_queue_pop(next);
 		if (t >= n_todo) break;
-		nx += s2_wave_read(ix, opt, split_len, ids[t], read_ids, seq, off, out_intv, out_n, cap, qb, lst[0], lst[1]);
+		nx += s2_wave_read(ix, opt, split_len, ids[t], read_ids, seq, off, out_intv, out_n, cap, qb, lst[0], lst[1], kt_tab, kt_k, resume, paths);
 	}
 	if (n_extend && nx && wv_lane() == 0) atomicAdd(n_extend, nx);
 }
diff --git a/speedseq_amd/csrc/ssg_dbg.cpp b/speedseq_amd/csrc/ssg_dbg.cpp
--- a/speedseq_amd/csrc/ssg_dbg.cpp
+++ b/speedseq_amd/csrc/ssg_dbg.cpp
@@ -441,6 +441,61 @@
 	return SSG_OK;
 }
 
+int ssg_dbg_extend_coop(const ssg_index_t *idx, int n, const ssg_intv_t *in, const uint8_t *base, const uint8_t *is_back, ssg_intv_t *out_lean, ssg_intv_t *out_coop,
+                        ssg_intv_t *out_lean4, ssg_intv_t *out_coop4)
+{
+	CHK(ssg_need_device());
+	if (n < 0 || n > 1 << 24) { ssg_err_msg = "ssg_dbg_extend_coop: need 0 <= n <= 2^24"; return SSG_EINVAL; }
+	if (n == 0) return SSG_OK;
+	const uint64_t seq_len = idx->v.seq_len;
+	std::vector<uint8_t> cd((size_t)n);
+	for (int t = 0; t < n; ++t) {
+		if (base[t] > 3) return dbg_refuse("ssg_dbg_extend_coop", "bases are codes 0 .. 3: item", t);
+		if (is_back[t] > 1) return dbg_refuse("ssg_dbg_extend_coop", "is_back is 0 or 1: item", t);
+		for (int side = 0; side < 2; ++side) {
+			const uint64_t kx = side ? in[t].x0 : in[t].x1;
+			if (kx > seq_len + 1 || in[t].x2 > seq_len + 1 || kx + in[t].x2 > seq_len + 1) return dbg_refuse("ssg_dbg_extend_coop", "need x0 + x2 <= text length + 1 and x1 + x2 <= text length + 1: item", t);
+		}
+		cd[t] = (uint8_t)(base[t] | is_back[t] << 2);
+	}
+	dbuf<ssg_intv_t> d_in((size_t)n), d_lean((size_t)n), d_coop((size_t)n), d_lean4((size_t)n * 4), d_coop4((size_t)n * 4); dbuf<uint8_t> d_cd((size_t)n);
+	CHKA(d_in); CHKA(d_lean); CHKA(d_coop); CHKA(d_lean4); CHKA(d_coop4); CHKA(d_cd);
+	CHK(d_in.up(in, (size_t)n)); CHK(d_cd.up(cd.data(), (size_t)n)); CHK(d_lean.zero()); CHK(d_coop.zero()); CHK(d_lean4.zero()); CHK(d_coop4.zero());
+	CHK(ssg_seed_dbg_extend_coop(idx, n, d_in.p, d_cd.p, d_lean.p, d_coop.p, d_lean4.p, d_coop4.p));
+	CHK(d_lean.down(out_lean, (size_t)n)); CHK(d_coop.down(out_coop, (size_t)n)); CHK(d_lean4.down(out_lean4, (size_t)n * 4));
+	return d_coop4.down(out_coop4, (size_t)n * 4);
+}
+
+int ssg_dbg_smem_ext(const ssg_index_t *idx, const ssg_mem_opt_t *opt, int n_reads, const uint8_t *seq, const int64_t *off, int cap, ssg_intv_t *out_intv, int32_t *out_n, uint64_t *n_extend, uint32_t paths[4])
+{
+	CHK(ssg_need_device());
+	*n_extend = 0; memset(paths, 0, 4 * sizeof(uint32_t));
+	if (n_reads < 0 || cap < 1) { ssg_err_msg = "ssg_dbg_smem_ext: need n_reads >= 0, cap >= 1"; return SSG_EINVAL; }
+	if (n_reads == 0) return SSG_OK;
+	if (off[0] != 0) return dbg_refuse("ssg_dbg_smem_ext", "offsets start at 0: read", 0);
+	int max_len = 0;
+	for (int r = 0; r < n_reads; ++r) {
+		const char *bad = 0;
+		const int64_t len = off[r + 1] - off[r];
+		if (len < 0) bad = "offsets must not decrease: read";
+		else if (len > SSG_MAX_READ_LEN) bad = "need read length <= " SSG_STR(SSG_MAX_READ_LEN) ": read";
+		if (!bad) dbg_check_codes(seq, off, r, &bad);
+		if (bad) return dbg_refuse("ssg_dbg_smem_ext", bad, r);
+		max_len = std::max(max_len, (int)len);
+	}
+	const char *e = getenv("SSG_SMEM_MAX_EXT");
+	const unsigned int max_ext = e && *e ? (unsigned int)atoi(e) : (unsigned int)(13 * max_len + 50);
+	dbuf<uint8_t> d_seq((size_t)off[n_reads] + 1); dbuf<int64_t> d_off((size_t)n_reads + 1); dbuf<ssg_intv_t> d_intv((size_t)n_reads * cap); dbuf<int32_t> d_n((size_t)n_reads); dbuf<unsigned long long> d_nx(1); dbuf<unsigned int> d_paths(4);
+	CHKA(d_seq); CHKA(d_off); CHKA(d_intv); CHKA(d_n); CHKA(d_nx); CHKA(d_paths);
+	CHK(d_seq.up(seq, (size_t)off[n_reads])); CHK(d_off.up(off, (size_t)n_reads + 1)); CHK(d_nx.zero()); CHK(d_paths.zero());
+	CHK(ssg_seed_smem2_paths(idx, opt, n_reads, d_seq.p, d_off.p, max_len, cap, d_intv.p, d_n.p, d_nx.p, max_ext, d_paths.p));
+	unsigned long long nx = 0;
+	CHK(d_nx.down(&nx, 1)); CHK(d_intv.down(out_intv, (size_t)n_reads * cap)); CHK(d_n.down(out_n, (size_t)n_reads));
+	for (int r = 0; r < n_reads; ++r) if (out_n[r] < 0) { ssg_err_msg = "ssg_dbg_smem_ext: a read's list exceeds the per-read capacity"; return SSG_EOVERFLOW; }
+	*n_extend = nx;
+	return d_paths.down(paths, 4);
+}
+
 int ssg_dbg_sbl_records(long n_pairs, const int64_t *req_off, const ssg_alnreq_t *req, const ssg_aln_t *alns, const ssg_sbl_opt_t *o, ssg_sbl_state_t *st,
                         int64_t *line_off, int64_t *n_lines, ssg_sbl_line_t *lines, int64_t *line_req, ssg_sbl_end_t *ends, int64_t *prim, uint64_t *sig, uint8_t *dup,
                         uint8_t *bits, int64_t *mate_line, uint64_t counts[4], uint64_t *keys)
diff --git a/speedseq_amd/csrc/ssg_dev.h b/speedseq_amd/csrc/ssg_dev.h
--- a/speedseq_amd/csrc/ssg_dev.h
+++ b/speedseq_amd/csrc/ssg_dev.h
@@ -93,6 +93,26 @@
 	v += SSG_DPP(0, v, 0x142, 0xa); v += SSG_DPP(0, v, 0x143, 0xc);
 	return v;
 }
+#endif
+#ifdef SSG_EMU
+SSG_DEVFN int wv_seg8_sum(int v) { for (int d = 1; d < 8; d <<= 1) v += wv_shfl(v, wv_lane() ^ d); return v; }
+#else
+SSG_DEVFN int wv_seg8_sum(int v)
+{
+	v += SSG_DPP(0, v, 0x111, 0xf); v += SSG_DPP(0, v, 0x112, 0xf); v += SSG_DPP(0, v, 0x114, 0xf);
+	return v;
+}
+#endif
+#ifdef SSG_EMU
+SSG_DEVFN int wv_seg8_allsum(int v) { return wv_seg8_sum(v); }
+SSG_DEVFN int wv_xor8(int v) { return wv_shfl(v, wv_lane() ^ 8); }
+#else
+SSG_DEVFN int wv_seg8_allsum(int v)
+{
+	v += SSG_DPP(0, v, 0xb1 , 0xf); v += SSG_DPP(0, v, 0x4e , 0xf); v += SSG_DPP(0, v, 0x141 , 0xf);
+	return v;
+}
+SSG_DEVFN int wv_xor8(int v) { return SSG_DPP(0, v, 0x128 , 0xf); }
 #endif
 SSG_DEVFN int wv_last(int v) { return wv_get(v, 63); }
 SSG_DEVFN long wv_queue_pop(unsigned int *queue)
diff --git a/speedseq_amd/csrc/ssg_index_int.h b/speedseq_amd/csrc/ssg_index_int.h
--- a/speedseq_amd/csrc/ssg_index_int.h
+++ b/speedseq_amd/csrc/ssg_index_int.h
@@ -24,6 +24,10 @@
 extern "C" int ssg_index_build_ktab(ssg_index *ix);
 extern "C" int ssg_seed_smem2(const ssg_index *idx, const ssg_mem_opt_t *opt, int n_reads, const uint8_t *d_seq, const int64_t *d_off, int max_len, int cap,
                               ssg_intv_t *d_intv, int32_t *d_n, unsigned long long *n_extend, unsigned int max_ext, uint32_t *d_n_ext_read);
+extern "C" int ssg_seed_smem2_paths(const ssg_index *idx, const ssg_mem_opt_t *opt, int n_reads, const uint8_t *d_seq, const int64_t *d_off, int max_len, int cap,
+                                    ssg_intv_t *d_intv, int32_t *d_n, unsigned long long *n_extend, unsigned int max_ext, unsigned int *d_paths);
+extern "C" int ssg_seed_dbg_extend_coop(const ssg_index *idx, int n, const ssg_intv_t *d_in, const uint8_t *d_cd, ssg_intv_t *d_lean, ssg_intv_t *d_coop,
+                                        ssg_intv_t *d_lean4, ssg_intv_t *d_coop4);
 extern "C" int ssg_sa_verify(const ssg_index *ix, int new_intv, const uint64_t *d_sa_new, long n_new);
 extern "C" int ssg_crc32_ranges_dev(const uint8_t *d_data, const uint64_t *d_cut, long n, uint32_t *d_crc);
 extern "C" int ssg_bgzf_frame_dev(const uint8_t *d_tmp, uint32_t tmp_stride, const uint64_t *d_cut, const uint64_t *d_moff, const uint32_t *d_crc, long n_blocks, uint8_t *d_dense);
diff --git a/speedseq_amd/csrc/ssg_seed.cpp b/speedseq_amd/csrc/ssg_seed.cpp
--- a/speedseq_amd/csrc/ssg_seed.cpp
+++ b/speedseq_amd/csrc/ssg_seed.cpp
@@ -8,13 +8,24 @@
 static int env_int(const char *name, int dflt) { const char *e = getenv(name); return e && *e ? atoi(e) : dflt; }
 static int budget_row(unsigned int max_ext) { return max_ext < 0x7fffffffu ? env_int("SSG_SMEM_MAX_ROW", 32) : 0x7fffffff; }
 
+static int s2_stat_down(unsigned long long st[64])
+{
+	CHK(rt_sync());
+#ifdef SSG_EMU
+	memcpy(st, ssg_s2_stat, 64 * sizeof(st[0]));
+#else
+	CHK(rt_check(hipMemcpyFromSymbol(st, HIP_SYMBOL(ssg_s2_stat), 64 * sizeof(st[0])), "hipMemcpyFromSymbol"));
+#endif
+	return 0;
+}
+
 static constexpr auto ssg_k_smem2_plain = ssg_k_smem2<false, false>;
 static constexpr auto ssg_k_smem2_kt = ssg_k_smem2<false, true>;
 static constexpr auto ssg_k_smem2_tune = ssg_k_smem2<true, false>;
 static constexpr auto ssg_k_smem2_kt_tune = ssg_k_smem2<true, true>;
 
-extern "C" int ssg_seed_smem2(const ssg_index *idx, const ssg_mem_opt_t *opt, int n_reads, const uint8_t *d_seq, const int64_t *d_off, int max_len, int cap,
-                              ssg_intv_t *d_intv, int32_t *d_n, unsigned long long *n_extend, unsigned int max_ext, uint32_t *d_n_ext_read)
+static int seed_smem2(const ssg_index *idx, const ssg_mem_opt_t *opt, int n_reads, const uint8_t *d_seq, const int64_t *d_off, int max_len, int cap,
+                      ssg_intv_t *d_intv, int32_t *d_n, unsigned long long *n_extend, unsigned int max_ext, uint32_t *d_n_ext_read, unsigned int *d_paths)
 {
 	const int block = 64;
 	const long nthreads = std::min<long>(((long)n_reads + block - 1) / block * block, 256L * env_int("SSG_SMEM_WAVES_PER_CU", 16) * 64)   ;
@@ -27,7 +38,9 @@
 	const int max_row = budget_row(max_ext);
 	const bool budget = max_ext < 0x7fffffffu;
 	dbuf<int32_t> d_heavy(budget ? (size_t)n_reads : 1);
-	if (!scratch.ok() || !d_next.ok() || !d_heavy.ok()) { ssg_err_msg = "device allocation failed: seeding work lists"; return SSG_ENOMEM; }
+	dbuf<ssg_s2_resume_t> d_resume(budget ? (size_t)n_reads : 1);
+	ssg_s2_resume_t *const rs = budget ? d_resume.p : (ssg_s2_resume_t*)0;
+	if (!scratch.ok() || !d_next.ok() || !d_heavy.ok() || !d_resume.ok()) { ssg_err_msg = "device allocation failed: seeding work lists"; return SSG_ENOMEM; }
 	CHK(d_next.zero());
 	int32_t *const hv = budget ? d_heavy.p : (int32_t*)0;
 	if (env_int("SSG_S2_TUNE", 0)) {
@@ -37,27 +50,63 @@
 #else
 		CHK(rt_sync()); CHK(rt_check(hipMemcpyToSymbol(HIP_SYMBOL(ssg_s2_stat), st, sizeof(st)), "hipMemcpyToSymbol"));
 #endif
-		if (kt) SSG_LAUNCH(ssg_k_smem2_kt_tune, nthreads / block, block, 0, idx->v, *opt, n_reads, (const int32_t*)0, d_seq, d_off, d_intv, d_n, cap, scratch.p, scap, n_extend, d_next.p, max_ext, max_row, d_n_ext_read, hv, d_next.p + 1, kt, kt_k);
-		else SSG_LAUNCH(ssg_k_smem2_tune, nthreads / block, block, 0, idx->v, *opt, n_reads, (const int32_t*)0, d_seq, d_off, d_intv, d_n, cap, scratch.p, scap, n_extend, d_next.p, max_ext, max_row, d_n_ext_read, hv, d_next.p + 1, kt, kt_k);
-		CHK(rt_sync());
-#ifdef SSG_EMU
-		memcpy(st, ssg_s2_stat, sizeof(st));
-#else
-		CHK(rt_check(hipMemcpyFromSymbol(st, HIP_SYMBOL(ssg_s2_stat), sizeof(st)), "hipMemcpyFromSymbol"));
-#endif
+		if (kt) SSG_LAUNCH(ssg_k_smem2_kt_tune, nthreads / block, block, 0, idx->v, *opt, n_reads, (const int32_t*)0, d_seq, d_off, d_intv, d_n, cap, scratch.p, scap, n_extend, d_next.p, max_ext, max_row, d_n_ext_read, hv, d_next.p + 1, kt, kt_k, rs);
+		else SSG_LAUNCH(ssg_k_smem2_tune, nthreads / block, block, 0, idx->v, *opt, n_reads, (const int32_t*)0, d_seq, d_off, d_intv, d_n, cap, scratch.p, scap, n_extend, d_next.p, max_ext, max_row, d_n_ext_read, hv, d_next.p + 1, kt, kt_k, rs);
+		CHK(s2_stat_down(st));
 		fprintf(stderr, "[ssgpu] smem2 timeline (ms): pool of reads empty at %.2f, last lane done at %.2f; %llu reads given up at %u extensions / rows of %d; rounds %llu, lanes ready %.1f, with a read %.1f of 64\n",
 		        (double)(st[1] - st[0]) / 1e5, (double)(st[2] - st[0]) / 1e5, st[3], max_ext, max_row, st[48], st[48] ? (double)st[49] / st[48] : 0., st[48] ? (double)st[50] / st[48] : 0.);
 		fprintf(stderr, "[ssgpu] smem2 reads by extensions (< 2^b):");
 		for (int b = 1; b <= 24; ++b) if (st[8 + b]) fprintf(stderr, " b%d=%llu", b, st[8 + b]);
 		fprintf(stderr, "\n");
-	} else if (kt) SSG_LAUNCH(ssg_k_smem2_kt, nthreads / block, block, 0, idx->v, *opt, n_reads, (const int32_t*)0, d_seq, d_off, d_intv, d_n, cap, scratch.p, scap, n_extend, d_next.p, max_ext, max_row, d_n_ext_read, hv, d_next.p + 1, kt, kt_k);
-	else SSG_LAUNCH(ssg_k_smem2_plain, nthreads / block, block, 0, idx->v, *opt, n_reads, (const int32_t*)0, d_seq, d_off, d_intv, d_n, cap, scratch.p, scap, n_extend, d_next.p, max_ext, max_row, d_n_ext_read, hv, d_next.p + 1, kt, kt_k);
+	} else if (kt) SSG_LAUNCH(ssg_k_smem2_kt, nthreads / block, block, 0, idx->v, *opt, n_reads, (const int32_t*)0, d_seq, d_off, d_intv, d_n, cap, scratch.p, scap, n_extend, d_next.p, max_ext, max_row, d_n_ext_read, hv, d_next.p + 1, kt, kt_k, rs);
+	else SSG_LAUNCH(ssg_k_smem2_plain, nthreads / block, block, 0, idx->v, *opt, n_reads, (const int32_t*)0, d_seq, d_off, d_intv, d_n, cap, scratch.p, scap, n_extend, d_next.p, max_ext, max_row, d_n_ext_read, hv, d_next.p + 1, kt, kt_k, rs);
 	if (budget) {
 		const long n_wg = std::min<long>(n_reads, 256L * env_int("SSG_SMEM_HEAVY_WAVES_PER_CU", 28));
-		if (scap <= 160) SSG_LAUNCH(ssg_k_smem_heavy<160>, n_wg, block, 0, idx->v, *opt, (const int32_t*)d_heavy.p, (const unsigned int*)(d_next.p + 1), (const int32_t*)0, d_seq, d_off, d_intv, d_n, cap, n_extend, d_next.p + 2);
-		else if (scap <= 264) SSG_LAUNCH(ssg_k_smem_heavy<264>, n_wg, block, 0, idx->v, *opt, (const int32_t*)d_heavy.p, (const unsigned int*)(d_next.p + 1), (const int32_t*)0, d_seq, d_off, d_intv, d_n, cap, n_extend, d_next.p + 2);
-		else SSG_LAUNCH(ssg_k_smem_heavy<328>, n_wg, block, 0, idx->v, *opt, (const int32_t*)d_heavy.p, (const unsigned int*)(d_next.p + 1), (const int32_t*)0, d_seq, d_off, d_intv, d_n, cap, n_extend, d_next.p + 2);
+		if (scap <= 160) SSG_LAUNCH(ssg_k_smem_heavy<160>, n_wg, block, 0, idx->v, *opt, (const int32_t*)d_heavy.p, (const unsigned int*)(d_next.p + 1), (const int32_t*)0, d_seq, d_off, d_intv, d_n, cap, n_extend, d_next.p + 2, kt, kt_k, (const ssg_s2_resume_t*)rs, d_paths);
+		else if (scap <= 264) SSG_LAUNCH(ssg_k_smem_heavy<264>, n_wg, block, 0, idx->v, *opt, (const int32_t*)d_heavy.p, (const unsigned int*)(d_next.p + 1), (const int32_t*)0, d_seq, d_off, d_intv, d_n, cap, n_extend, d_next.p + 2, kt, kt_k, (const ssg_s2_resume_t*)rs, d_paths);
+		else SSG_LAUNCH(ssg_k_smem_heavy<328>, n_wg, block, 0, idx->v, *opt, (const int32_t*)d_heavy.p, (const unsigned int*)(d_next.p + 1), (const int32_t*)0, d_seq, d_off, d_intv, d_n, cap, n_extend, d_next.p + 2, kt, kt_k, (const ssg_s2_resume_t*)rs, d_paths);
+		if (env_int("SSG_S2_TUNE", 0)) {
+			unsigned long long st[64];
+			CHK(s2_stat_down(st));
+			const unsigned long long *const w = st + 52;
+			fprintf(stderr, "[ssgpu] smem_heavy counts: {\"tuning_build\": %d, \"kt_k\": %d, \"max_ext\": %u, \"max_row\": %d, \"given_up\": %llu, \"lane_ext_of_given_up\": %llu, \"lane_ext_in_finished_calls\": %llu, "
+			        "\"reads\": %llu, \"rounds_forward\": %llu, \"rounds_third_pass\": %llu, \"rounds_backward\": %llu, \"rounds_backward_rows_1_4\": %llu, \"rounds_backward_rows_5_16\": %llu, "
+			        "\"rounds_backward_rows_17_64\": %llu, \"rounds_backward_rows_65_up\": %llu, \"extensions\": %llu, \"table_starts\": %llu, \"extensions_from_table\": %llu}\n",
+			        (int)SSG_TUNING, kt_k, max_ext, max_row, st[3], st[5], st[4], w[S2_WC_READS], w[S2_WC_FWD], w[S2_WC_P3], w[S2_WC_BWD], w[S2_WC_ROW4], w[S2_WC_ROW16], w[S2_WC_ROW64], w[S2_WC_ROWMORE],
+			        w[S2_WC_EXT], w[S2_WC_TABSTART], w[S2_WC_TABEXT]);
+		}
 	}
+	return rt_sync();
+}
+
+extern "C" int ssg_seed_smem2(const ssg_index *idx, const ssg_mem_opt_t *opt, int n_reads, const uint8_t *d_seq, const int64_t *d_off, int max_len, int cap,
+                              ssg_intv_t *d_intv, int32_t *d_n, unsigned long long *n_extend, unsigned int max_ext, uint32_t *d_n_ext_read)
+{
+	return seed_smem2(idx, opt, n_reads, d_seq, d_off, max_len, cap, d_intv, d_n, n_extend, max_ext, d_n_ext_read, (unsigned int*)0);
+}
+extern "C" int ssg_seed_smem2_paths(const ssg_index *idx, const ssg_mem_opt_t *opt, int n_reads, const uint8_t *d_seq, const int64_t *d_off, int max_len, int cap,
+                                    ssg_intv_t *d_intv, int32_t *d_n, unsigned long long *n_extend, unsigned int max_ext, unsigned int *d_paths)
+{
+	return seed_smem2(idx, opt, n_reads, d_seq, d_off, max_len, cap, d_intv, d_n, n_extend, max_ext, (uint32_t*)0, d_paths);
+}
+
+__global__ void __launch_bounds__(64) ssg_k_dbg_extend_coop(ssg_index_view_t ix, int n, const ssg_intv_t *in, const uint8_t *cd, ssg_intv_t *out_lean, ssg_intv_t *out_coop,
+                                                            ssg_intv_t *out_lean4, ssg_intv_t *out_coop4)
+{
+	for (int t = (int)blockIdx.x; t < n; t += (int)gridDim.x) {
+		const ssg_intv_t ik = wv_uni_intv(in[t]);
+		const int c = wv_uni((int)cd[t] & 3), back = wv_uni((int)cd[t] >> 2 & 1);
+		const ssg_intv_t a = ssg_bwt_extend1_lean(ix, ik, c, back), b = s2_extend_coop(ix, ik, c, back);
+		if (wv_lane() == 0) { out_lean[t] = a; out_coop[t] = b; }
+		const int g = wv_lane() >> 4;
+		const ssg_intv_t ig = in[(t + g) % n];
+		const ssg_intv_t a4 = ssg_bwt_extend1_lean(ix, ig, c, back), b4 = s2_extend_coop4(ix, ig, c, back);
+		if ((wv_lane() & 15) == 0) { out_lean4[4 * (long)t + g] = a4; out_coop4[4 * (long)t + g] = b4; }
+	}
+}
+extern "C" int ssg_seed_dbg_extend_coop(const ssg_index *idx, int n, const ssg_intv_t *d_in, const uint8_t *d_cd, ssg_intv_t *d_lean, ssg_intv_t *d_coop, ssg_intv_t *d_lean4, ssg_intv_t *d_coop4)
+{
+	SSG_LAUNCH(ssg_k_dbg_extend_coop, std::min(n, 1024), 64, 0, idx->v, n, d_in, d_cd, d_lean, d_coop, d_lean4, d_coop4);
 	return rt_sync();
 }
 
```

After: 5.625 million pairs/s, median of 6. 1.03x the previous value.
